# saifahmadgit/go2-sim2real-locomotion-rl

Measured on AMD Instinct MI355X. Metric: env-steps/sec (all envs) Go2 walk 4096 envs; 1/2/4/8-GPU scaling, higher is better.
Workload: dtype f32

## Files before the change

go2_sim2real_locomotion_rl_amd/csrc/go2sim.hip:

```cpp

#include <hip/hip_runtime.h>

#include <cstdint>
#include <cstdio>
#include <cstdlib>
#include <cstring>
#include <new>
#include <vector>

#include "../../include/go2sim.h"
#include "../../include/go2sim_detmath.h"

#define DEV __device__ __forceinline__
#define DEVN __device__ __noinline__

namespace {

constexpr int NL = GO2SIM_NL, ND = GO2SIM_ND, NQ = GO2SIM_NQ, NG = GO2SIM_NG, NJ = GO2SIM_NJ;
constexpr int NPAIR = GO2SIM_NPAIR_MAX, MAXC = GO2SIM_MAX_CONTACTS, MAXB = GO2SIM_MAX_BROAD, MAXR = GO2SIM_MAX_ROWS;
constexpr int JOINT_FIXED = 0, JOINT_REVOLUTE = 1, JOINT_FREE = 4;
constexpr int GEOM_PLANE = 0, GEOM_SPHERE = 1, GEOM_CYLINDER = 3, GEOM_BOX = 5, GEOM_TERRAIN = 7;
constexpr int TERRAIN_CB = 4;
constexpr int MAX_CONTACTS_PER_PAIR = 5;
constexpr int CTRL_FORCE = 0, CTRL_VELOCITY = 1, CTRL_POSITION = 2;
// ... 1381 lines not shown
  }
  if (legs) {
    const int r = m.leg_root;
    if (tl < 6 * LEG_K) {
      const int l = tl / 6, c = tl % 6;
      const float* src = (c < 3) ? s->cdofd_vel : s->cdofd_ang;
      const int cc = (c < 3) ? c : c - 3;
      const V3 g0 = -m.gravity * (1.0f - 0.0f);
      const int ds = m.links[r].dof_start;
      float vr[6], xr[6], vl[LEG_D], xl[LEG_D]; int lk[LEG_D];
#pragma unroll
      for (int i = 0; i < 6; ++i) { vr[i] = s->vel[ds + i]; xr[i] = src[3 * (ds + i) + cc]; }
#pragma unroll
      for (int d = 0; d < LEG_D; ++d) {
        lk[d] = m.leg_links[LEG_D * l + d];
        const int i_d = m.links[lk[d]].dof_start;
        vl[d] = s->vel[i_d]; xl[d] = src[3 * i_d + cc];
      }
      float* dst = (c < 3) ? s->cdd_vel : s->cdd_ang;
      float a = (c < 3) ? ((cc == 0) ? g0.x : ((cc == 1) ? g0.y : g0.z)) : 0.0f;
#pragma unroll
      for (int i = 0; i < 6; ++i) a = a + xr[i] * vr[i];
      if (l == 0) dst[3 * r + cc] = a;
#pragma unroll
      for (int d = 0; d < LEG_D; ++d) { a = a + xl[d] * vl[d]; dst[3 * lk[d] + cc] = a; }
    }
    for (int i_l = tl; i_l < NL; i_l += T) {
      if (m.links[i_l].parent != -1 || i_l == r) continue;
      st3(s->cdd_vel, i_l, -m.gravity * (1.0f - 0.0f)); st3(s->cdd_ang, i_l, v3(0, 0, 0));
    }
    team_sync();
  }
  for (int lev = 0; lev < (legs ? 0 : m.n_levels); ++lev) {
    for (int k = m.level_start[lev] + tl; k < m.level_start[lev + 1]; k += T) {
      int i_l = m.level_links[k];
      const auto& L = m.links[i_l];
      V3 cv, ca;
      if (L.parent == -1) { cv = -m.gravity * (1.0f - 0.0f); ca = v3(0, 0, 0); }
      else { cv = ld3(s->cdd_vel, L.parent); ca = ld3(s->cdd_ang, L.parent); }
      for (int i_d = L.dof_start; i_d < L.dof_end; ++i_d) {
        float v = s->vel[i_d];
        V3 local_cdd_vel = ld3(s->cdofd_vel, i_d) * v;
        V3 local_cdd_ang = ld3(s->cdofd_ang, i_d) * v;
        cv = cv + local_cdd_vel;
        ca = ca + local_cdd_ang;
      }
      st3(s->cdd_vel, i_l, cv); st3(s->cdd_ang, i_l, ca);
    }
    team_sync();
  }
  for (int i_l = tl; i_l < NL; i_l += T) {
    V3 f1_ang, f1_vel, f2_ang, f2_vel, f3_ang, f3_vel;
    M3 I = ld9(s->cinr_I, i_l); V3 cp = ld3(s->cinr_pos, i_l); float cm = s->cinr_mass[i_l];
    V3 cdv = ld3(s->cd_vel, i_l), cda = ld3(s->cd_ang, i_l);
    inertial_mul(cp, I, cm, ld3(s->cdd_vel, i_l), ld3(s->cdd_ang, i_l), f1_ang, f1_vel);
    inertial_mul(cp, I, cm, cdv, cda, f2_ang, f2_vel);
    motion_cross_force(cda, cdv, f2_ang, f2_vel, f3_ang, f3_vel);
    V3 ext_ang = ld3(s->cfrc_ang, i_l), ext_vel = ld3(s->cfrc_vel, i_l);
    st3(s->cfrc_vel, i_l, f1_vel + f3_vel + ext_vel + v3(0, 0, 0));
    st3(s->cfrc_ang, i_l, f1_ang + f3_ang + ext_ang + v3(0, 0, 0));
  }
  team_sync();
  if (legs) {
    for (int c = tl; c < 6; c += T) {
      auto at = [&](int i_l) -> float* { return (c < 3) ? &s->cfrc_vel[3 * i_l + c] : &s->cfrc_ang[3 * i_l + c - 3]; };
      const int r = m.leg_root;
      float x[LEG_K][LEG_D];
#pragma unroll
      for (int l = 0; l < LEG_K; ++l)
#pragma unroll
        for (int d = 0; d < LEG_D; ++d) x[l][d] = *at(m.leg_links[LEG_D * l + d]);
      float a = *at(r);
#pragma unroll
      for (int l = 0; l < LEG_K; ++l) {
#pragma unroll
        for (int d = LEG_D - 2; d >= 0; --d) { x[l][d] = x[l][d] + x[l][d + 1]; *at(m.leg_links[LEG_D * l + d]) = x[l][d]; }
      }
#pragma unroll
      for (int l = 0; l < LEG_K; ++l) a = a + x[l][0];
      *at(r) = a;
    }
    team_sync();
  }
  for (int lev = (legs ? -1 : m.n_levels - 2); lev >= 0; --lev) {
    int n_par = m.level_start[lev + 1] - m.level_start[lev];
    for (int w = tl; w < n_par * 6; w += T) {
      int i_p = m.level_links[m.level_start[lev] + w / 6], comp = w % 6;
      float* dst = (comp < 3) ? &s->cfrc_vel[3 * i_p + comp] : &s->cfrc_ang[3 * i_p + comp - 3];
      float a = *dst;
      for (int c = m.child_start[i_p]; c < m.child_start[i_p + 1]; ++c) {
        int i_l = m.child_list[c];
        a = a + ((comp < 3) ? s->cfrc_vel[3 * i_l + comp] : s->cfrc_ang[3 * i_l + comp - 3]);
      }
      *dst = a;
    }
    team_sync();
  }
  for (int i_d = tl; i_d < ND; i_d += T) {
    int i_l = m.dof_link[i_d];
    float qf_bias = dot(ld3(s->cdof_ang, i_d), ld3(s->cfrc_ang, i_l)) + dot(ld3(s->cdof_vel, i_d), ld3(s->cfrc_vel, i_l));
    float f = s->qf_passive[i_d] - qf_bias + s->qf_applied[i_d];
    s->force[i_d] = f;
    if (env_valid) { astore(e, AO(force), i_d, f); astore(e, AO(qf_smooth), i_d, f); }
  }
  team_sync();
  PH(24)
  bool solved = false;
#if GO2SIM_FAST_ORDER
  if constexpr (T == 32 || T == 64) {
    if (arrow) {
      const int leg = (tl >> 3) & 3, u = tl & 7, ub = u < 6 ? u : 5;
      const int p0 = dm_arrow_dof(m.arrow_mode, leg, 0), p1 = dm_arrow_dof(m.arrow_mode, leg, 1), p2 = dm_arrow_dof(m.arrow_mode, leg, 2);
      float xb[6], x0, x1, x2;
      arrow_solve<T>(AF, s->force[p0], s->force[p1], s->force[p2], s->force[ub], s->Dinv, tl, xb, x0, x1, x2);
      if (tl == 0) {
#pragma unroll
        for (int k = 0; k < 6; ++k) s->out[k] = xb[k];
      }
      if (tl < 32 && u == 0) { s->out[p0] = x0; s->out[p1] = x1; s->out[p2] = x2; }
      solved = true;
    }
  }
#endif
  if (!solved) {
    float y[ND];
#pragma unroll
    for (int i_d_ = 0; i_d_ < ND; ++i_d_) {
      const int i_d = ND - i_d_ - 1;
      float cur = s->force[i_d];
#pragma unroll
      for (int j_d = i_d + 1; j_d < ND; ++j_d) cur = cur - s->L[j_d * ND + i_d] * y[j_d];
      y[i_d] = cur;
    }
#pragma unroll
    for (int i_d = 0; i_d < ND; ++i_d) y[i_d] = y[i_d] * s->Dinv[i_d];
#pragma unroll
    for (int i_d = 0; i_d < ND; ++i_d) {
      float cur = y[i_d];
#pragma unroll
      for (int j_d = 0; j_d < i_d; ++j_d) cur = cur - s->L[i_d * ND + j_d] * y[j_d];
      y[i_d] = cur;
    }
    if (tl == 0) {
#pragma unroll
      for (int i_d = 0; i_d < ND; ++i_d) s->out[i_d] = y[i_d];
    }
  }
  team_sync();
  if (env_valid) for (int i_d = tl; i_d < ND; i_d += T) { float a = s->out[i_d]; astore(e, AO(acc_smooth), i_d, a); astore(e, AO(acc), i_d, a); }
  if (env_valid) for (int idx = tl; idx < NTRI; idx += T) { int i, j; tri_index(m, idx, i, j); astore(e, AO(mass_mat), idx, s->M[i * ND + j]); }
  PH(25)
}

template <int T>
__global__ __launch_bounds__(64) void k_dynamics_team(Pool P, const ModelS* __restrict__ mp) {
  constexpr int EPW = 64 / T;
  __shared__ DynData lds[EPW];
  __shared__ alignas(16) char ms_raw[MODELS_LDS_BYTES];
  const ModelS& ms = *(const ModelS*)ms_raw;
  wg_dma_to_lds<(int)sizeof(ModelS)>(ms_raw, mp);
  {
    const int b0 = xcd_block() * EPW;
    wg_load<EPW, NL * 3>(P, b0, FO(cd_vel), [&](int ev, int k, float v) { lds[ev].cd_vel[k] = v; });
    wg_load<EPW, NL * 3>(P, b0, FO(cd_ang), [&](int ev, int k, float v) { lds[ev].cd_ang[k] = v; });
    wg_load<EPW, ND>(P, b0, FO(vel), [&](int ev, int k, float v) { lds[ev].vel[k] = v; });
  }
  const int tl = threadIdx.x % T, slot = threadIdx.x / T;
  const int b = xcd_block() * EPW + slot;
  const bool env_valid = b < P.B;
  const ModelView m(&ms, mp);
  E e(P, env_valid ? b : P.B - 1);
  DynData* s = &lds[slot];
  PH_BEGIN
  team_stage<NL * 9, T>(tl, [&](int k) { return aload(e, AO(cinr_inertial), k); }, [&](int k, float v) { s->cinr_I[k] = v; s->crb_I[k] = v; });
  team_stage<NL * 3, T>(tl, [&](int k) { return aload(e, AO(cinr_pos), k); }, [&](int k, float v) { s->cinr_pos[k] = v; s->crb_pos[k] = v; });
  team_stage<NL, T>(tl, [&](int k) { return aload(e, AO(cinr_mass), k); }, [&](int k, float v) { s->cinr_mass[k] = v; s->crb_mass[k] = v; });
  team_stage<ND, T>(tl, [&](int d) { return __int_as_float((int)e.ctrl_mode()[d]); }, [&](int d, float v) { s->ctrl_mode[d] = __float_as_int(v); });
  team_stage<ND * 3, T>(tl, [&](int k) { return aload(e, AO(cdof_ang), k); }, [&](int k, float v) { s->cdof_ang[k] = v; });
  team_stage<ND * 3, T>(tl, [&](int k) { return aload(e, AO(cdof_vel), k); }, [&](int k, float v) { s->cdof_vel[k] = v; });
  team_stage<ND * 3, T>(tl, [&](int k) { return aload(e, AO(cdofd_ang), k); }, [&](int k, float v) { s->cdofd_ang[k] = v; });
  team_stage<ND * 3, T>(tl, [&](int k) { return aload(e, AO(cdofd_vel), k); }, [&](int k, float v) { s->cdofd_vel[k] = v; });
  team_stage<ND, T>(tl, [&](int d) { return gload(e, FO(ctrl_force), d); }, [&](int d, float v) { s->qf_applied[d] = v; });
  team_stage<ND, T>(tl, [&](int d) { return gload(e, FO(ctrl_pos), d); }, [&](int d, float v) { s->qf_passive[d] = v; });
  team_stage<ND, T>(tl, [&](int d) { return gload(e, FO(ctrl_vel), d); }, [&](int d, float v) { s->force[d] = v; });
  team_stage<ND, T>(tl, [&](int d) { return gload(e, FO(dof_pos), d); }, [&](int d, float v) { s->out[d] = v; });
  team_stage<NL * 6, T>(tl, [&](int k) { return gload(e, FO(ext), k); },
                        [&](int k, float v) { int i_l = k / 6, c = k % 6; if (c < 3) s->cfrc_ang[3 * i_l + c] = v; else s->cfrc_vel[3 * i_l + c - 3] = v; });
  team_sync();
  PH(20)
  tk_dynamics<T>(m, e, s, tl, env_valid);
}


template <bool OVERLAY, int EPW> struct KinSeparate { KinData k[EPW]; DEV KinData* at(int slot, void*) { return &k[slot]; } };
template <int EPW> struct KinSeparate<true, EPW> { DEV KinData* at(int, void* overlay) { return (KinData*)overlay; } };
constexpr bool KIN_OVERLAY = sizeof(KinData) <= 2 * sizeof(float) * ND * ND;
template <int T>
DEV void integrate_fk_dynamics_body(const Pool& P, const ModelS* __restrict__ mp, int b, DynData* lds_d, char* ms_raw, KinSeparate<KIN_OVERLAY, 64 / T>& lds_k,
                                    bool pre, float pre_vel, float pre_acc) {
  const ModelS& ms = *(const ModelS*)ms_raw;
  wg_dma_to_lds<(int)sizeof(ModelS)>(ms_raw, mp);
  const int tl = threadIdx.x % T, slot = threadIdx.x / T;
  const ModelView m(&ms, mp);
  E e(P, b < P.B ? b : P.B - 1);
  DynData* d = &lds_d[slot];
  static_assert(offsetof(DynData, L) == offsetof(DynData, M) + sizeof(float) * ND * ND, "KinData overlay");
  KinData* s = lds_k.at(slot, d->M);
  PH_BEGIN
  if (pre) { if (tl < ND) { s->vel[tl] = pre_vel; s->vel_next[tl] = pre_acc; } }
  else {
    team_stage<ND, T>(tl, [&](int i) { return gload(e, FO(vel), i); }, [&](int i, float v) { s->vel[i] = v; });
    team_stage<ND, T>(tl, [&](int i) { return aload(e, AO(acc), i); }, [&](int i, float a) { s->vel_next[i] = a; });
  }
  team_stage<NQ, T>(tl, [&](int q) { return gload(e, FO(qpos), q); }, [&](int q, float v) { s->qpos[q] = v; });
  team_stage<ND, T>(tl, [&](int i) { return __int_as_float((int)e.ctrl_mode()[i]); }, [&](int i, float v) { d->ctrl_mode[i] = __float_as_int(v); });
  team_stage<ND, T>(tl, [&](int i) { return gload(e, FO(ctrl_force), i); }, [&](int i, float v) { d->qf_applied[i] = v; });
  team_stage<ND, T>(tl, [&](int i) { return gload(e, FO(ctrl_pos), i); }, [&](int i, float v) { d->qf_passive[i] = v; });
  team_stage<ND, T>(tl, [&](int i) { return gload(e, FO(ctrl_vel), i); }, [&](int i, float v) { d->force[i] = v; });
  team_stage<NL * 6, T>(tl, [&](int k) { return gload(e, FO(ext), k); },
                        [&](int k, float v) { int i_l = k / 6, c = k % 6; if (c < 3) d->cfrc_ang[3 * i_l + c] = v; else d->cfrc_vel[3 * i_l + c - 3] = v; });
  team_for<ND, T>(tl, [&](int i) { s->vel_next[i] = s->vel[i] + s->vel_next[i] * m.substep_dt; });
  if (tl == 0) s->valid = 1;
  tk_stage_links<T>(e, s, tl);
  team_sync();
  if (b >= P.B) return;
  tk_integrate<T>(m, e, s, tl);
  PH(40)
  tk_kinematics<T>(m, e, s, tl, false, d);
  team_for<ND, T>(tl, [&](int i) { d->vel[i] = s->vel[i]; });
  team_sync();
  PH(41)
  tk_dynamics<T>(m, e, d, tl, true);
}
template <int T>
__global__ __launch_bounds__(64) void k_integrate_fk_dynamics_team(Pool P, const ModelS* __restrict__ mp) {
  STAMP(STK_INT_FK_DYN)
  constexpr int EPW = 64 / T;
  __shared__ DynData lds_d[EPW];
  __shared__ alignas(16) char ms_raw[MODELS_LDS_BYTES];
  __shared__ KinSeparate<KIN_OVERLAY, EPW> lds_k;
  integrate_fk_dynamics_body<T>(P, mp, xcd_block() * EPW + (int)threadIdx.x / T, lds_d, ms_raw, lds_k, false, 0.0f, 0.0f);
}

DEV int wrap180(float x) {
  if (!(x >= 0.0f)) return 0;
  int i = (x >= 180.0f) ? (int)(x - 180.0f) : (int)x;
  return (i > 179) ? 179 : i;
}
DEV int clampidx(float x) {
  if (!(x >= 0.0f)) return 0;
  return (x >= 179.0f) ? 179 : (int)x;
}
DEV V3 support_cylinder_local(const Model& m, const Geom& G, V3 d_mesh, int* vid_out = nullptr) {
  const float PI = 3.14159265358979323846f;
  float theta = dm_atan2(d_mesh.y, d_mesh.x);
  float phi = dm_acos(d_mesh.z);
  const float support_res = 180.0f;
  float ii = (theta + PI) / PI / 2.0f * support_res;
  float jj = phi / PI * support_res;
  const int i_lo = wrap180(dm_floor(ii)), i_hi = wrap180(dm_ceil(ii));
  int j_lo = clampidx(dm_floor(jj)); if (j_lo == 0) j_lo = 1;
  int j_hi = clampidx(dm_ceil(jj)); if (j_hi == 179) j_hi = 178;
  const int k_lo = m.theta_to_ring[i_lo], k_hi = m.theta_to_ring[i_hi];
  const float rx_lo = G.rim[k_lo][0], ry_lo = G.rim[k_lo][1], rx_hi = G.rim[k_hi][0], ry_hi = G.rim[k_hi][1];
  const float half = 0.5f * G.data[1];
  float dot_max = -1e20f;
  V3 v = v3(0, 0, 0);
  int vid = 0;
#pragma unroll
  for (int i4 = 0; i4 < 4; ++i4) {
    const bool hi_i = (i4 % 2) != 0, hi_j = (i4 / 2) > 0;
    const int j = hi_j ? j_hi : j_lo, k = hi_i ? k_hi : k_lo;
    V3 pos = v3(hi_i ? rx_hi : rx_lo, hi_i ? ry_hi : ry_lo, (j <= 90) ? half : -half);
    float d = dot(pos, d_mesh);
    if (d > dot_max) { v = pos; dot_max = d; vid = k + ((j <= 90) ? 0 : 32); }
  }
  if (vid_out) *vid_out = vid;
  return v;
}
template <int T> DEV unsigned long long team_ballot(bool p) {
  const unsigned long long b = __ballot(p);
  if constexpr (T == 64) return b;
  else return (b >> (threadIdx.x & (64 - T))) & ((1ull << T) - 1ull);
}
DEV V3 vsel(bool c, V3 a, V3 b) { return v3(c ? a.x : b.x, c ? a.y : b.y, c ? a.z : b.z); }
DEV V3 support_prism(const V3* prism, V3 d) {
  const bool bottom = d.z < 0;
  const V3 p0 = vsel(bottom, prism[0], prism[3]), p1 = vsel(bottom, prism[1], prism[4]), p2 = vsel(bottom, prism[2], prism[5]);
  float best = dot(p0, d);
  V3 v = p0;
  const float dt1 = dot(p1, d);
  const bool b1 = dt1 > best;
  v = vsel(b1, p1, v); best = b1 ? dt1 : best;
  const float dt2 = dot(p2, d);
  v = vsel(dt2 > best, p2, v);
  return v;
}
struct GeomLite { int type; float d0, d1, d2; };
DEV GeomLite geom_lite(const Model& m, int i_g) { const Geom& G = m.geoms[i_g]; GeomLite r = {G.type, G.data[0], G.data[1], G.data[2]}; return r; }
DEV V3 support_driver(const Model& m, V3 direction, int i_g, const GeomLite& gl, V3 pos, const Rot& rot, const V3* prism = nullptr) {
  if (gl.type == GEOM_TERRAIN) return support_prism(prism, direction);
  if (gl.type == GEOM_SPHERE) {
    return pos + direction * gl.d0;
  } else if (gl.type == GEOM_BOX) {
    V3 d_box = rot_apply_inv(rot, direction);
    V3 v_ = v3((d_box.x < 0.0f ? -1.0f : 1.0f) * gl.d0 * 0.5f, (d_box.y < 0.0f ? -1.0f : 1.0f) * gl.d1 * 0.5f,
               (d_box.z < 0.0f ? -1.0f : 1.0f) * gl.d2 * 0.5f);
    return rot_apply(rot, v_) + pos;
  } else if (gl.type == GEOM_CYLINDER) {
    V3 d_mesh = rot_apply_inv(rot, direction);
    V3 v_ = support_cylinder_local(m, m.geoms[i_g], d_mesh);
    return rot_apply(rot, v_) + pos;
  }
  return pos;
}
struct Pair { int i_ga, i_gb; V3 pos_a; Q4 quat_a; V3 pos_b; Q4 quat_b; const V3* prism; GeomLite ga, gb; Rot ra, rb; };
DEV void pair_set_rots(Pair& pr) { pr.ra = make_rot(pr.quat_a); pr.rb = make_rot(pr.quat_b); }
DEV void compute_support(const Model& m, V3 direction, const Pair& pr, V3& v, V3& v1, V3& v2) {
  v1 = support_driver(m, direction, pr.i_ga, pr.ga, pr.pos_a, pr.ra);
  v2 = support_driver(m, -direction, pr.i_gb, pr.gb, pr.pos_b, pr.rb, pr.prism);
  v = v1 - v2;
}


DEV V3 gjk_support_driver(const Model& m, V3 direction, int i_g, const GeomLite& gl, V3 pos, const Rot& rot, int& vid) {
  if (gl.type == GEOM_SPHERE) {
    vid = -1;
    return pos + direction * gl.d0;
  } else if (gl.type == GEOM_BOX) {
    V3 d_box = rot_apply_inv(rot, direction);
    V3 v_ = v3((d_box.x < 0.0f ? -1.0f : 1.0f) * gl.d0 * 0.5f, (d_box.y < 0.0f ? -1.0f : 1.0f) * gl.d1 * 0.5f,
               (d_box.z < 0.0f ? -1.0f : 1.0f) * gl.d2 * 0.5f);
    vid = (v_.x > 0.0f) * 1 + (v_.y > 0.0f) * 2 + (v_.z > 0.0f) * 4 + 64 * i_g;
    return rot_apply(rot, v_) + pos;
  } else if (gl.type == GEOM_CYLINDER) {
    V3 d_mesh = rot_apply_inv(rot, direction);
    int k = 0;
    V3 v_ = support_cylinder_local(m, m.geoms[i_g], d_mesh, &k);
    vid = k + 64 * i_g;
    return rot_apply(rot, v_) + pos;
  }
  vid = -1;
  return pos;
}
#include "go2sim_gjk_dev.h"

DEVN DgResult gjk_query_global(const DgPair& dp, GjkStoreFull* full, float eps) { return dg_contact(dp, *full, eps); }
DEV DgResult gjk_query(const DgPair& dp, GjkStoreLds* slots, unsigned* slot_mask, GjkStoreFull* full, float eps) {
  int slot = -1;
  if (slots) {
    for (int i = 0; i < GJK_SLOTS_MAX && slot < 0; ++i) {
      const unsigned bit = 1u << i;
      if (!(atomicOr(slot_mask, bit) & bit)) slot = i;
    }
  }
  DgResult r; r.is_col = false; r.overflow = true; r.penetration = 0.0f; r.normal = v3(0, 0, 0); r.pos = v3(0, 0, 0);
  if (slot >= 0) {
    r = dg_contact(dp, slots[slot], eps);
    atomicAnd(slot_mask, ~(1u << slot));
  }
  if (r.overflow) r = gjk_query_global(dp, full, eps);
  return r;
}

struct Simplex { V3 v[4], v1[4], v2[4]; };
DEV V3 mpr_portal_dir(const Simplex& s) { return normalized(cross(s.v[2] - s.v[1], s.v[3] - s.v[1])); }
DEV bool mpr_portal_reach_tolerance(const Model& m, const Simplex& s, V3 v, V3 direction) {
  float dv1 = dot(s.v[1], direction), dv2 = dot(s.v[2], direction), dv3 = dot(s.v[3], direction), dv4 = dot(v, direction);
  float dot1 = fmn(fmn(dv4 - dv1, dv4 - dv2), dv4 - dv3);
  return dot1 < m.ccd_tolerance + m.ccd_eps * fmx(1.0f, dot1);
}
DEV void simplex_set(Simplex& s, int i, V3 v, V3 v1, V3 v2) {
  const bool c1 = i == 1, c2 = i == 2, c3 = !(c1 || c2);
  s.v[1] = vsel(c1, v, s.v[1]); s.v1[1] = vsel(c1, v1, s.v1[1]); s.v2[1] = vsel(c1, v2, s.v2[1]);
  s.v[2] = vsel(c2, v, s.v[2]); s.v1[2] = vsel(c2, v1, s.v1[2]); s.v2[2] = vsel(c2, v2, s.v2[2]);
  s.v[3] = vsel(c3, v, s.v[3]); s.v1[3] = vsel(c3, v1, s.v1[3]); s.v2[3] = vsel(c3, v2, s.v2[3]);
}
DEV void mpr_expand_portal(Simplex& s, V3 v, V3 v1, V3 v2) {
  V3 v4v0 = cross(v, s.v[0]);
  float d = dot(s.v[1], v4v0);
  int i_s;
  if (d > 0) { d = dot(s.v[2], v4v0); i_s = (d > 0) ? 1 : 3; }
  else { d = dot(s.v[3], v4v0); i_s = (d > 0) ? 2 : 1; }
  simplex_set(s, i_s, v, v1, v2);
}
DEV bool mpr_first_support_separates(const Model& m, const Pair& pr, V3 center_a, V3 center_b) {
  const float EPSC = m.ccd_eps;
  V3 v0 = center_a - center_b;
  if (dm_abs(v0.x) < EPSC && dm_abs(v0.y) < EPSC && dm_abs(v0.z) < EPSC) v0.x += 10.0f * EPSC;
  const V3 direction = -normalized(v0);
  V3 v, v1, v2;
  compute_support(m, direction, pr, v, v1, v2);
  return dot(v, direction) < EPSC;
}
DEV int mpr_discover_portal(const Model& m, Simplex& s, const Pair& pr, V3 center_a, V3 center_b) {
  const float EPSC = m.ccd_eps;
  s.v1[0] = center_a; s.v2[0] = center_b; s.v[0] = center_a - center_b;
  int simplex_size = 1;
  if (dm_abs(s.v[0].x) < EPSC && dm_abs(s.v[0].y) < EPSC && dm_abs(s.v[0].z) < EPSC) s.v[0].x += 10.0f * EPSC;
  V3 direction = -normalized(s.v[0]);
  V3 v, v1, v2;
  compute_support(m, direction, pr, v, v1, v2);
  s.v1[1] = v1; s.v2[1] = v2; s.v[1] = v;
  simplex_size = 2;
  float d = dot(v, direction);
  int ret = 0;
  if (d < EPSC) {
    ret = -1;
  } else {
    direction = cross(s.v[0], s.v[1]);
    if (dot(direction, direction) < EPSC) {
      if (dm_abs(s.v[1].x) < EPSC && dm_abs(s.v[1].y) < EPSC && dm_abs(s.v[1].z) < EPSC) ret = 1; else ret = 2;
    } else {
      direction = normalized(direction);
      compute_support(m, direction, pr, v, v1, v2);
      d = dot(v, direction);
      if (d < EPSC) {
        ret = -1;
      } else {
        s.v1[2] = v1; s.v2[2] = v2; s.v[2] = v;
        simplex_size = 3;
        V3 va = s.v[1] - s.v[0], vb = s.v[2] - s.v[0];
        direction = normalized(cross(va, vb));
        d = dot(direction, s.v[0]);
        if (d > 0) {
          V3 t;
          t = s.v[1]; s.v[1] = s.v[2]; s.v[2] = t; t = s.v1[1]; s.v1[1] = s.v1[2]; s.v1[2] = t; t = s.v2[1]; s.v2[1] = s.v2[2]; s.v2[2] = t;
          direction = -direction;
        }
        int num_trials = 0;
        while (simplex_size < 4) {
          compute_support(m, direction, pr, v, v1, v2);
          d = dot(v, direction);
          if (d < EPSC) { ret = -1; break; }
          bool cont = false;
          va = cross(s.v[1], v);
// ... 4 lines not shown
            d = dot(va, s.v[0]);
            if (d < -EPSC) { s.v1[1] = v1; s.v2[1] = v2; s.v[1] = v; cont = true; }
          }
          if (cont) {
            va = s.v[1] - s.v[0]; vb = s.v[2] - s.v[0];
            direction = normalized(cross(va, vb));
            num_trials++;
            if (num_trials == 15) { ret = -1; break; }
          } else {
            s.v1[3] = v1; s.v2[3] = v2; s.v[3] = v;
            simplex_size = 4;
          }
        }
      }
    }
  }
  return ret;
}
DEV int mpr_refine_portal(const Model& m, Simplex& s, const Pair& pr) {
  int ret = 1;
  while (true) {
    V3 direction = mpr_portal_dir(s);
    if (dot(s.v[1], direction) > -m.ccd_eps) { ret = 0; break; }
    V3 v, v1, v2;
    compute_support(m, direction, pr, v, v1, v2);
    if (!(dot(v, direction) > -m.ccd_eps) || mpr_portal_reach_tolerance(m, s, v, direction)) { ret = -1; break; }
    mpr_expand_portal(s, v, v1, v2);
  }
  return ret;
}
DEV V3 mpr_find_pos(const Model& m, const Simplex& s) {
  float b0 = 0.0f, b1 = 0.0f, b2 = 0.0f, b3 = 0.0f;
  float sum_ = ((b0 + b1) + b2) + b3;
  if (sum_ < m.ccd_eps) {
    V3 direction = mpr_portal_dir(s);
    b0 = 0.0f;
    b1 = dot(cross(s.v[2], s.v[3]), direction);
    b2 = dot(cross(s.v[3], s.v[1]), direction);
    b3 = dot(cross(s.v[1], s.v[2]), direction);
    sum_ = ((b0 + b1) + b2) + b3;
  }
  V3 p1 = v3(0, 0, 0), p2 = v3(0, 0, 0);
  p1 = p1 + b0 * s.v1[0]; p2 = p2 + b0 * s.v2[0];
  p1 = p1 + b1 * s.v1[1]; p2 = p2 + b1 * s.v2[1];
  p1 = p1 + b2 * s.v1[2]; p2 = p2 + b2 * s.v2[2];
  p1 = p1 + b3 * s.v1[3]; p2 = p2 + b3 * s.v2[3];
  return (0.5f / sum_) * (p1 + p2);
}
DEV void mpr_find_penetration(const Model& m, Simplex& s, const Pair& pr, bool& is_col, V3& normal, float& penetration, V3& pos) {
  int iterations = 0;
  while (true) {
    V3 direction = mpr_portal_dir(s);
    V3 v, v1, v2;
    compute_support(m, direction, pr, v, v1, v2);
    if (mpr_portal_reach_tolerance(m, s, v, direction) || iterations > m.ccd_iterations) {
      penetration = dot(direction, s.v[1]);
      normal = -direction;
      is_col = true;
      pos = mpr_find_pos(m, s);
      break;
    }
    mpr_expand_portal(s, v, v1, v2);
    iterations++;
  }
}
DEV void guess_geoms_center(const Model& m, const Pair& pr, V3 normal_ws, V3& center_a, V3& center_b) {
  const Geom& A = m.geoms[pr.i_ga]; const Geom& Bg = m.geoms[pr.i_gb];
  center_a = transform_by_trans_quat(A.center, pr.pos_a, pr.quat_a);
  center_b = transform_by_trans_quat(Bg.center, pr.pos_b, pr.quat_b);
  if (dm_abs(normal_ws.x) > m.ccd_eps || dm_abs(normal_ws.y) > m.ccd_eps || dm_abs(normal_ws.z) > m.ccd_eps) {
    V3 center_a_local = 0.5f * (A.aabb[7] + A.aabb[0]);
    center_a = transform_by_trans_quat(center_a_local, pr.pos_a, pr.quat_a);
    V3 center_b_local = 0.5f * (Bg.aabb[7] + Bg.aabb[0]);
    center_b = transform_by_trans_quat(center_b_local, pr.pos_b, pr.quat_b);
    V3 delta = center_a - center_b;
    V3 normal = normalized(delta);
    if (norm(cross(normal_ws, normal)) > 0.01f) {
      V3 offset = dot(delta, normal_ws) * normal_ws - delta;
      float offset_norm = norm(offset);
      if (offset_norm > m.eps) {
        V3 dir_offset = offset / offset_norm;
        V3 dla = inv_transform_by_quat(dir_offset, pr.quat_a), dlb = inv_transform_by_quat(dir_offset, pr.quat_b);
        V3 box_size_a = A.aabb[7] - A.aabb[0], box_size_b = Bg.aabb[7] - Bg.aabb[0];
        float length_a = dot(box_size_a, v3(dm_abs(dla.x), dm_abs(dla.y), dm_abs(dla.z)));
        float length_b = dot(box_size_b, v3(dm_abs(dlb.x), dm_abs(dlb.y), dm_abs(dlb.z)));
        float offset_ratio = fmn(offset_norm / (length_a + length_b), 0.5f);
        center_a = center_a + dir_offset * length_a * offset_ratio;
        center_b = center_b - dir_offset * length_b * offset_ratio;
      }
    }
  }
}
DEV void mpr_contact_from_centers(const Model& m, const Pair& pr, V3 center_a, V3 center_b, bool& is_col, V3& normal, float& penetration, V3& pos) {
  Simplex s;
  int res = mpr_discover_portal(m, s, pr, center_a, center_b);
  is_col = false; pos = v3(0, 0, 0); normal = v3(0, 0, 0); penetration = 0.0f;
  if (res == 1) {
    is_col = true; penetration = 0.0f; normal = -normalized(s.v[0]); pos = (s.v1[1] + s.v2[1]) * 0.5f;
  } else if (res == 2) {
    is_col = true; penetration = norm(s.v[1]); normal = -normalized(s.v[1]); pos = (s.v1[1] + s.v2[1]) * 0.5f;
  } else if (res == 0) {
    res = mpr_refine_portal(m, s, pr);
    if (res >= 0) mpr_find_penetration(m, s, pr, is_col, normal, penetration, pos);
  }
}
DEV void mpr_contact(const Model& m, const Pair& pr, V3 normal_ws, bool& is_col, V3& normal, float& penetration, V3& pos) {
  V3 center_a, center_b;
  guess_geoms_center(m, pr, normal_ws, center_a, center_b);
  mpr_contact_from_centers(m, pr, center_a, center_b, is_col, normal, penetration, pos);
}

DEV float compute_tolerance(const Model& m, int i_ga, int i_gb, float tolerance) {
  float size_b = norm(m.geoms[i_gb].aabb[7] - m.geoms[i_gb].aabb[0]);
  if (m.geoms[i_ga].type == GEOM_PLANE) return 0.5f * tolerance * size_b;
  float size_a = norm(m.geoms[i_ga].aabb[7] - m.geoms[i_ga].aabb[0]);
  return 0.5f * tolerance * fmn(size_a, size_b);
}
DEV void contact_orthogonals(const Model& m, const E& e, int i_ga, int i_gb, V3 normal, V3& axis_0, V3& axis_1) {
  V3 size_ga = m.geoms[i_ga].aabb[7], size_gb = m.geoms[i_gb].aabb[7];
  float volume_ga = size_ga.x * size_ga.y * size_ga.z, volume_gb = size_gb.x * size_gb.y * size_gb.z;
  int i_g = (volume_ga < volume_gb && m.geoms[i_ga].type != GEOM_PLANE) ? i_ga : i_gb;
  int i_l = m.geoms[i_g].link;
  M3 rot = quat_to_R(e.i_quat()[i_l], m.eps);
  int axis_idx = 0; float axis_angle_max = 0.0f;
#pragma unroll
  for (int i = 0; i < 3; ++i) {
    float axis_angle = dm_abs(dot(mcol(rot, i), normal));
    if (axis_angle > axis_angle_max) { axis_angle_max = axis_angle; axis_idx = i; }
  }
  axis_idx = (axis_idx + 1) % 3;
  axis_0 = mcol(rot, axis_idx);
  axis_0 = normalized(axis_0 - dot(normal, axis_0) * normal);
  axis_1 = cross(normal, axis_0);
}
DEV void rotate_frame(V3 pos, Q4 quat, V3 contact_pos, Q4 qrot, V3& new_pos, Q4& new_quat) {
  new_quat = transform_quat_by_quat(quat, qrot);
  V3 rel = contact_pos - pos;
  V3 vec = transform_by_quat(rel, qrot);
  vec = vec - rel;
  new_pos = pos - vec;
}

DEV void plane_contact(const Model& m, const Pair& pr, bool& is_col, V3& normal, float& penetration, V3& pos) {
  const V3 plane_dir = transform_by_quat(v3(pr.ga.d0, pr.ga.d1, pr.ga.d2), pr.quat_a);
  normal = -normalized(plane_dir);
  const V3 v1 = support_driver(m, normal, pr.i_gb, pr.gb, pr.pos_b, pr.rb);
  penetration = dot(normal, v1 - pr.pos_a);
  pos = v1 - 0.5f * penetration * normal;
  is_col = penetration > 0.0f;
}
constexpr int GJK_SLOTS = GJK_SLOTS_MAX;
template <int T>
struct CollideData {
  struct Broad {
    alignas(16) float amin[NG * 4], amax[NG * 4];
    float sval[2 * NG], sval_sorted[2 * NG];
    alignas(16) unsigned long long skey[2 * NG];
    int sig[2 * NG], sig_sorted[2 * NG];
    alignas(8) int rank_mm[NG * 2];
    int cand_key[MAXB], cand_pair[MAXB];
  };
  struct TPair { int i_ga, r_min, r_max, c_min, c_max, n_items, item_off; float zmin, tol; V3 pos_a; Q4 quat_a; V3 center_a; };
  struct Terrain {
    TPair tp[NG];
  };
  union alignas(16) {
    Broad bp;
    GjkStoreLds gjk[GJK_SLOTS];
    Terrain tr;
  };
  unsigned short pair_sorted[MAXB];
  float stage[T][5][7];
  int cnt[T];
  unsigned gjk_slot_mask;
  float gjk_res[T][8];
  unsigned ncv[NCV];
};
struct ContactStage { float* st; int n; };

DEV void stage_contact(ContactStage& cs, V3 normal, V3 pos, float pen) {
  float* p = cs.st + 7 * cs.n;
  p[0] = normal.x; p[1] = normal.y; p[2] = normal.z; p[3] = pos.x; p[4] = pos.y; p[5] = pos.z; p[6] = pen;
  cs.n++;
}

DEV void plane_box_contact_staged(const Model& m, const E& e, int i_ga, int i_gb, ContactStage& cs) {
  const V3 ga_pos = e.g_pos()[i_ga], gb_pos = e.g_pos()[i_gb];
  const Q4 ga_quat = e.g_quat()[i_ga], gb_quat = e.g_quat()[i_gb];
  const Geom& A = m.geoms[i_ga]; const Geom& Bg = m.geoms[i_gb];
  const V3 normal = -normalized(transform_by_quat(v3(A.data[0], A.data[1], A.data[2]), ga_quat));
  const V3 d_box = inv_transform_by_quat(normal, gb_quat);
  const V3 v_ = v3((d_box.x < 0.0f ? -1.0f : 1.0f) * Bg.data[0] * 0.5f, (d_box.y < 0.0f ? -1.0f : 1.0f) * Bg.data[1] * 0.5f,
                   (d_box.z < 0.0f ? -1.0f : 1.0f) * Bg.data[2] * 0.5f);
  const V3 v1 = transform_by_trans_quat(v_, gb_pos, gb_quat);
  const float pen0 = dot(normal, v1 - ga_pos);
  if (!(pen0 > 0.0f)) return;
  const V3 contact_pos_0 = v1 - 0.5f * pen0 * normal;
  stage_contact(cs, normal, contact_pos_0, pen0);
  const float tolerance = compute_tolerance(m, i_ga, i_gb, m.mc_tolerance);
  const int n_max = imn(m.n_contacts_per_pair, 5);
  for (int c = 0; c < 8; ++c) {
    if (cs.n >= n_max) break;
    const V3 corner = transform_by_trans_quat(Bg.aabb[c], gb_pos, gb_quat);
    const float pen = dot(normal, corner - ga_pos);
    if (pen > 0.0f) {
      const V3 cpos = corner - 0.5f * pen * normal;
      if (norm(cpos - contact_pos_0) > tolerance) stage_contact(cs, normal, cpos, pen);
    }
  }
}

struct CcState {
  Pair pr; V3 ga_pos_o, gb_pos_o; Q4 ga_quat_o, gb_quat_o;
  int i_pair, type_a, type_b; bool multi_contact, want_gjk; float tolerance;
  bool is_col; float penetration; V3 normal, contact_pos;
};
DEV void cc_mpr_with_retry(const Model& m, CcState& c, int i_detection, unsigned* ncv, const Arr3& normal_cache, bool& guess_available) {
  const float EPS = m.eps;
  bool is_mpr_updated = false;
  V3 normal_ws = ((ncv[c.i_pair >> 5] >> (c.i_pair & 31)) & 1u) ? (V3)normal_cache[c.i_pair] : v3(0, 0, 0);
  guess_available = (dm_abs(normal_ws.x) > EPS) || (dm_abs(normal_ws.y) > EPS) || (dm_abs(normal_ws.z) > EPS);
  for (int i_mpr = 0; i_mpr < 2; ++i_mpr) {
    if (i_mpr == 1) {
      if ((i_detection == 0) && !c.is_col && guess_available) { normal_ws = v3(0, 0, 0); guess_available = false; is_mpr_updated = false; }
    }
    if (!is_mpr_updated) {
      PHD_BEGIN
      mpr_contact(m, c.pr, normal_ws, c.is_col, c.normal, c.penetration, c.contact_pos);
      PHD(36)
      is_mpr_updated = true;
    }
  }
}
DEV bool cc_prefer_gjk(const Model& m, const CcState& c, bool guess_available) {
  if (c.penetration > c.tolerance) return !guess_available || (m.mc_tolerance * c.penetration >= m.mpr_to_gjk_ratio * c.tolerance);
  return false;
}
DEV void cc_detect0(const Model& m, const E& e, int i_ga, int i_gb, unsigned* ncv, CcState& c) {
  c.type_a = m.geoms[i_ga].type; c.type_b = m.geoms[i_gb].type;
  c.multi_contact = (c.type_a != GEOM_SPHERE) && (c.type_b != GEOM_SPHERE);
  c.tolerance = compute_tolerance(m, i_ga, i_gb, m.mc_tolerance);
  c.ga_pos_o = e.g_pos()[i_ga]; c.gb_pos_o = e.g_pos()[i_gb]; c.ga_quat_o = e.g_quat()[i_ga]; c.gb_quat_o = e.g_quat()[i_gb];
  Pair& pr = c.pr;
  pr.i_ga = i_ga; pr.i_gb = i_gb; pr.pos_a = c.ga_pos_o; pr.quat_a = c.ga_quat_o; pr.pos_b = c.gb_pos_o; pr.quat_b = c.gb_quat_o; pr.prism = nullptr; pr.ga = geom_lite(m, i_ga); pr.gb = geom_lite(m, i_gb);
  pair_set_rots(pr);
  c.is_col = false; c.penetration = 0.0f; c.normal = v3(0, 0, 0); c.contact_pos = v3(0, 0, 0);
  c.i_pair = (i_ga > i_gb) ? m.pair_idx[i_gb][i_ga] : m.pair_idx[i_ga][i_gb];
  if (c.type_a == GEOM_PLANE) {
    plane_contact(m, pr, c.is_col, c.normal, c.penetration, c.contact_pos);
    c.want_gjk = false;
    return;
  }
  bool guess_available;
  cc_mpr_with_retry(m, c, 0, ncv, e.normal_cache(), guess_available);
  c.want_gjk = cc_prefer_gjk(m, c, guess_available);
}
DEV void cc_gjk_lane(const Model& m, const E& e, CcState& c, GjkStoreLds* gjk_slots, unsigned* gjk_slot_mask, GjkStoreFull* gjk_full) {
  atomicAdd(&e.gjk_fallback()[0], 1);
  const Pair& pr = c.pr;
  DgPair dp;
  dp.m = &m; dp.i_ga = pr.i_ga; dp.i_gb = pr.i_gb; dp.pos_a = pr.pos_a; dp.quat_a = pr.quat_a; dp.pos_b = pr.pos_b; dp.quat_b = pr.quat_b;
  dp.ga = pr.ga; dp.gb = pr.gb; dp.ra = pr.ra; dp.rb = pr.rb;
  dp.discrete = c.type_a == GEOM_BOX && c.type_b == GEOM_BOX;
  PHD_BEGIN
  const DgResult gr = gjk_query(dp, gjk_slots, gjk_slot_mask, gjk_full, m.eps);
  PHD(34)
  c.is_col = gr.is_col;
  c.penetration = gr.penetration;
  if (c.is_col) { c.contact_pos = gr.pos; c.normal = gr.normal; }
}
DEV void cc_rest(const Model& m, const E& e, CcState& c, ContactStage& cs, GjkStoreLds* gjk_slots, unsigned* gjk_slot_mask, GjkStoreFull* gjk_full, unsigned* ncv) {
  const float EPS = m.eps;
  const int i_ga = c.pr.i_ga, i_gb = c.pr.i_gb, i_pair = c.i_pair;
  const bool multi_contact = c.multi_contact;
  const float tolerance = c.tolerance;
  Pair& pr = c.pr;
  bool is_col_0 = false; V3 normal_0 = v3(0, 0, 0), contact_pos_0 = v3(0, 0, 0);
  bool& is_col = c.is_col; float& penetration = c.penetration; V3& normal = c.normal; V3& contact_pos = c.contact_pos;
  V3 axis_0 = v3(0, 0, 0), axis_1 = v3(0, 0, 0); Q4 qrot = q4(0, 0, 0, 0);
  auto normal_cache = e.normal_cache();
  PHD_BEGIN
  for (int i_detection = 0; i_detection < 5; ++i_detection) {
    if (i_detection == 1) { PHD(44) }
    if (i_detection > 0 && multi_contact && is_col_0) {
      V3 axis = (float)(2 * (i_detection % 2) - 1) * axis_0 + (float)(1 - 2 * ((i_detection / 2) % 2)) * axis_1;
      qrot = rotvec_to_quat(m.mc_perturbation * axis, EPS);
      rotate_frame(c.ga_pos_o, c.ga_quat_o, contact_pos_0, qrot, pr.pos_a, pr.quat_a);
      rotate_frame(c.gb_pos_o, c.gb_quat_o, contact_pos_0, inv_quat(qrot), pr.pos_b, pr.quat_b);
      pair_set_rots(pr);
      if (c.type_a == GEOM_PLANE) {
        plane_contact(m, pr, is_col, normal, penetration, contact_pos);
      } else {
        bool guess_available;
        cc_mpr_with_retry(m, c, i_detection, ncv, normal_cache, guess_available);
        if (cc_prefer_gjk(m, c, guess_available)) cc_gjk_lane(m, e, c, gjk_slots, gjk_slot_mask, gjk_full);
      }
    }
    if (i_detection == 0) {
      is_col_0 = is_col; normal_0 = normal; contact_pos_0 = contact_pos;
      if (is_col_0) {
        stage_contact(cs, normal, contact_pos, penetration);
        if (multi_contact) contact_orthogonals(m, e, i_ga, i_gb, normal, axis_0, axis_1);
        normal_cache[i_pair] = normal; atomicOr(&ncv[i_pair >> 5], 1u << (i_pair & 31));
      } else {
        atomicAnd(&ncv[i_pair >> 5], ~(1u << (i_pair & 31)));
      }
    } else if (multi_contact && is_col) {
      V3 contact_point_a = transform_by_quat((contact_pos - 0.5f * penetration * normal) - contact_pos_0, inv_quat(qrot)) + contact_pos_0;
      V3 contact_point_b = transform_by_quat((contact_pos + 0.5f * penetration * normal) - contact_pos_0, qrot) + contact_pos_0;
      contact_pos = 0.5f * (contact_point_a + contact_point_b);
      V3 tw = cross(normal, normal_0);
      V3 twist_rotvec = v3(clampf(tw.x, -m.mc_perturbation, m.mc_perturbation), clampf(tw.y, -m.mc_perturbation, m.mc_perturbation),
                           clampf(tw.z, -m.mc_perturbation, m.mc_perturbation));
      normal = normal + cross(twist_rotvec, normal);
      penetration = dot(normal, contact_point_b - contact_point_a);
      bool repeated = false;
      for (int i_c = 0; i_c < cs.n; ++i_c)
        if (!repeated) {
          const float* prev = cs.st + 7 * (cs.n - 1 - i_c);
          if (norm(contact_pos - v3(prev[3], prev[4], prev[5])) < tolerance) repeated = true;
        }
      if (!repeated && penetration > -tolerance) {
        penetration = fmx(penetration, 0.0f);
        stage_contact(cs, normal, contact_pos, penetration);
      }
    }
  }
  PHD(46)
}
DEV void convex_convex_contact_staged(const Model& m, const E& e, int i_ga, int i_gb, ContactStage& cs, GjkStoreLds* gjk_slots, unsigned* gjk_slot_mask, GjkStoreFull* gjk_full, unsigned* ncv) {
  CcState c;
  cc_detect0(m, e, i_ga, i_gb, ncv, c);
  if (c.want_gjk) cc_gjk_lane(m, e, c, gjk_slots, gjk_slot_mask, gjk_full);
  cc_rest(m, e, c, cs, gjk_slots, gjk_slot_mask, gjk_full, ncv);
}

DEV bool terrain_pair_out_of_reach(const Model& m, const GeomLite& gl, V3 pos) {
  float R;
  if (gl.type == GEOM_SPHERE) R = gl.d0;
  else if (gl.type == GEOM_BOX) R = 0.5f * dm_sqrt(gl.d0 * gl.d0 + gl.d1 * gl.d1 + gl.d2 * gl.d2);
  else if (gl.type == GEOM_CYLINDER) R = dm_sqrt(gl.d0 * gl.d0 + 0.25f * (gl.d1 * gl.d1));
  else return false;
  R = R * 1.001f + 1e-3f;
  const float* tmm = m.terrain_xyz_maxmin;
  const float sh = m.terrain_hs;
  int r_lo = (int)dm_floor((pos.x - R - tmm[3]) / sh) - 1, r_hi = (int)dm_ceil((pos.x + R - tmm[3]) / sh) + 1;
  int c_lo = (int)dm_floor((pos.y - R - tmm[4]) / sh) - 1, c_hi = (int)dm_ceil((pos.y + R - tmm[4]) / sh) + 1;
  r_lo = imx(0, r_lo); c_lo = imx(0, c_lo); r_hi = imn(m.terrain_rows - 1, r_hi); c_hi = imn(m.terrain_cols - 1, c_hi);
  if (!(r_lo <= r_hi && c_lo <= c_hi)) return false;
  const int I0 = r_lo / TERRAIN_CB, J0 = c_lo / TERRAIN_CB;
  if (r_hi / TERRAIN_CB > I0 + 2 || c_hi / TERRAIN_CB > J0 + 2) return false;
  float mx = -1e30f;
#pragma unroll
  for (int a = 0; a < 3; ++a)
#pragma unroll
    for (int q = 0; q < 3; ++q) mx = fmx(mx, m.terrain_cmax[(size_t)imn(I0 + a, m.terrain_crows - 1) * m.terrain_ccols + imn(J0 + q, m.terrain_ccols - 1)]);
  return mx < pos.z - R;
}
template <class TP>
DEV bool terrain_pair_setup(const Model& m, const E& e, int i_ga, int i_gb, TP& t) {
  V3 ga_pos = e.g_pos()[i_ga], gb_pos = e.g_pos()[i_gb]; Q4 ga_quat = e.g_quat()[i_ga], gb_quat = e.g_quat()[i_gb];
  const float margin = 0.0f;
  transform_pos_quat_by_trans_quat(ga_pos - gb_pos, ga_quat, v3(0, 0, 0), inv_quat(gb_quat), t.pos_a, t.quat_a);
  t.center_a = transform_by_trans_quat(m.geoms[i_ga].center, t.pos_a, t.quat_a);
  t.i_ga = i_ga;
  GeomLite gl = geom_lite(m, i_ga);
  const Rot t_rot = make_rot(t.quat_a);
  float xyz_max_min[6];
#pragma unroll
  for (int i_axis = 0; i_axis < 3; ++i_axis)
#pragma unroll
    for (int i_m = 0; i_m < 2; ++i_m) {
      V3 direction = v3(0, 0, 0);
      vset(direction, i_axis, (i_m == 0) ? 1.0f : -1.0f);
      V3 v1 = support_driver(m, direction, i_ga, gl, t.pos_a, t_rot);
      xyz_max_min[3 * i_m + i_axis] = vget(v1, i_axis);
    }
  const float* tmm = m.terrain_xyz_maxmin;
  bool is_return = false;
#pragma unroll
  for (int i = 0; i < 3; ++i)
    if (tmm[i] < xyz_max_min[i + 3] - margin || tmm[i + 3] > xyz_max_min[i] + margin) is_return = true;
  const float sh = m.terrain_hs;
  int r_min = (int)dm_floor((xyz_max_min[3] - tmm[3]) / sh);
  int r_max = (int)dm_ceil((xyz_max_min[0] - tmm[3]) / sh);
  int c_min = (int)dm_floor((xyz_max_min[4] - tmm[4]) / sh);
  int c_max = (int)dm_ceil((xyz_max_min[1] - tmm[4]) / sh);
  t.r_min = imx(0, r_min); t.c_min = imx(0, c_min);
  t.r_max = imn(m.terrain_rows - 1, r_max); t.c_max = imn(m.terrain_cols - 1, c_max);
  t.zmin = xyz_max_min[5];
  if (is_return) { t.r_max = t.r_min; }
  return !is_return;
}
DEV float terrain_strip_z(const Model& m, int r, int c_min, int k) { return m.terrain_hf[(size_t)(r + (k & 1)) * m.terrain_cols + c_min + (k >> 1)]; }
static_assert(NG - 1 <= 32, "five bits of pair slot: at most 32 geoms besides the heightfield");
inline bool terrain_cells_fit(const Model& m, float hs) {
  for (int i = 0; i < NG; ++i) {
    const double dx = m.geoms[i].aabb[7].x - m.geoms[i].aabb[0].x, dy = m.geoms[i].aabb[7].y - m.geoms[i].aabb[0].y, dz = m.geoms[i].aabb[7].z - m.geoms[i].aabb[0].z;
    const double n = std::sqrt(dx * dx + dy * dy + dz * dz) / (double)hs + 2.0;
    if (i > 0 && 2.0 * n * n >= (double)(1 << 26)) return false;
  }
  return true;
}
DEV int terrain_desc(int p, int local) { return p | (local << 5); }
template <class TP>
DEV void terrain_desc_cell(const TP& t, int local, int& r, int& k) {
  const int nkk = 2 * (t.c_max - t.c_min + 1) - 2;
  r = t.r_min + local / nkk; k = 2 + local % nkk;
}
template <class TP>
DEV void terrain_prism_pair(const Model& m, const TP& t, int i_gb, int r, int k, V3 (&prism)[6], Pair& pr, V3& center_b) {
  const float* tmm = m.terrain_xyz_maxmin;
  const float sh = m.terrain_hs;
#pragma unroll
  for (int j = 0; j < 3; ++j) {
    int kk = k - 2 + j;
    float x = sh * (float)(r + (kk & 1)) + tmm[3], y = sh * (float)(t.c_min + (kk >> 1)) + tmm[4];
    prism[j] = v3(x, y, tmm[5]);
    prism[3 + j] = v3(x, y, terrain_strip_z(m, r, t.c_min, kk) + 0.0f);
  }
  pr.i_ga = t.i_ga; pr.i_gb = i_gb; pr.prism = prism; pr.pos_a = t.pos_a; pr.quat_a = t.quat_a; pr.pos_b = v3(0, 0, 0); pr.quat_b = qident();
  pr.ga = geom_lite(m, t.i_ga); pr.gb = geom_lite(m, i_gb);
  pair_set_rots(pr);
  center_b = v3(0, 0, 0);
  for (int i_p = 0; i_p < 6; ++i_p) center_b = center_b + prism[i_p];
  center_b = center_b / 6.0f;
}
template <class TP>
DEV bool terrain_prism_separated_at_once(const Model& m, const TP& t, int i_gb, int r, int k) {
  V3 prism[6]; Pair pr; V3 center_b;
  terrain_prism_pair(m, t, i_gb, r, k, prism, pr, center_b);
  return mpr_first_support_separates(m, pr, t.center_a, center_b);
}
template <class TP>
DEV bool terrain_prism_contact(const Model& m, const E& e, const TP& t, int i_gb, int r, int k, V3& normal, V3& contact_pos, float& penetration) {
  V3 prism[6]; Pair pr; V3 center_b;
  terrain_prism_pair(m, t, i_gb, r, k, prism, pr, center_b);
  bool is_col;
  mpr_contact_from_centers(m, pr, t.center_a, center_b, is_col, normal, penetration, contact_pos);
  if (is_col) {
    V3 gb_pos = e.g_pos()[i_gb]; Q4 gb_quat = e.g_quat()[i_gb];
    normal = transform_by_quat(normal, gb_quat);
    contact_pos = transform_by_quat(contact_pos, gb_quat);
    contact_pos = contact_pos + gb_pos;
  }
  return is_col;
}

template <int T>
__global__ __launch_bounds__(64) void k_collide_team(Pool P, const Model* __restrict__ mp, GjkStoreFull* __restrict__ gjk_scratch, int* __restrict__ lpt_rec, int lpt_cap, int solver_epw) {
  STAMP(STK_COLLIDE)
  constexpr int EPW = 64 / T;
  __shared__ CollideData<T> lds[EPW];
  const int tl = threadIdx.x % T, slot = threadIdx.x / T;
  const int b = xcd_block() * EPW + slot;
  if (slot >= EPW || b >= P.B) return;
  const Model& m = *mp;
  E e(P, b);
  CollideData<T>* s = &lds[slot];
  const float inf = dm_bits2f(0x7f800000u);
  if (tl == 0) s->gjk_slot_mask = 0u;
  for (int i = tl; i < NCV; i += T) s->ncv[i] = (unsigned)e.ncache_valid()[i];
  PH_BEGIN
  const int nc_old = e.n_contacts()[0];
  const bool first = e.first_time()[0] != 0;
  const int n2 = 2 * NG;
  team_stage<2 * NG, T>(tl, [&](int i) { return __int_as_float(e.sort_ig()[i]); }, [&](int i, float v) { s->bp.sig[i] = __float_as_int(v); });
  constexpr int NPI = (NPAIR + T - 1) / T;
  int packed_[NPI];
  {
    const int n_pairs = m.n_pairs;
#pragma unroll
    for (int it = 0; it < NPI; ++it) { int pidx = it * T + tl; int v = m.pair_list[pidx < NPAIR ? pidx : NPAIR - 1]; packed_[it] = (pidx < n_pairs) ? v : -1; }
  }
#pragma unroll
  for (int g0 = 0; g0 < NG; g0 += T) {
    const int i_g = (g0 + tl < NG) ? g0 + tl : NG - 1;
    V3 lower = v3(inf, inf, inf), upper = v3(-inf, -inf, -inf);
    V3 gp = e.g_pos()[i_g]; Q4 gq = e.g_quat()[i_g];
#pragma unroll
    for (int c = 0; c < 8; ++c) {
      V3 corner = transform_by_trans_quat(m.geoms[i_g].aabb[c], gp, gq);
      lower = vmin(lower, corner); upper = vmax(upper, corner);
    }
    *(float4*)&s->bp.amin[4 * i_g] = make_float4(lower.x, lower.y, lower.z, 0.0f);
    *(float4*)&s->bp.amax[4 * i_g] = make_float4(upper.x, upper.y, upper.z, 0.0f);
  }
  for (int i_c = tl; i_c < nc_old; i_c += T) {
    e.c_link()[i_c] = -1; e.c_link()[MAXC + i_c] = -1; e.c_geom()[i_c] = -1; e.c_geom()[MAXC + i_c] = -1;
    e.c_pen()[i_c] = 0.0f; e.c_pos()[i_c] = v3(0, 0, 0); e.c_normal()[i_c] = v3(0, 0, 0); e.c_force()[i_c] = v3(0, 0, 0);
  }
  team_sync();
  PH(30)
  for (int i = tl; i < n2; i += T) {
    int sg = first ? ((i >> 1) | ((i & 1) ? 0x100 : 0)) : s->bp.sig[i];
    int g = sg & 0xff;
    s->bp.sig[i] = sg;
    const float v = (sg & 0x100) ? s->bp.amax[4 * g] : s->bp.amin[4 * g];
    s->bp.sval[i] = v;
    unsigned u = (unsigned)__float_as_int(v + 0.0f);
    u = (u & 0x80000000u) ? ~u : (u | 0x80000000u);
    s->bp.skey[i] = ((unsigned long long)u << 8) | (unsigned long long)i;
  }
  team_sync();
  {
    constexpr int NK = (2 * NG + T - 1) / T;
    unsigned long long key[NK]; int r[NK];
#pragma unroll
    for (int q = 0; q < NK; ++q) { const int i = tl + q * T; key[q] = s->bp.skey[i < n2 ? i : n2 - 1]; r[q] = 0; }
#pragma unroll
    for (int j = 0; j < 2 * NG; ++j) {
      const unsigned long long kj = s->bp.skey[j];
#pragma unroll
      for (int q = 0; q < NK; ++q) r[q] += (kj < key[q]) ? 1 : 0;
    }
#pragma unroll
    for (int q = 0; q < NK; ++q) {
      const int i = tl + q * T;
      if (i < n2) {
        const float v = s->bp.sval[i];
        const int sg = s->bp.sig[i];
        s->bp.sval_sorted[r[q]] = v; s->bp.sig_sorted[r[q]] = sg;
        s->bp.rank_mm[2 * (sg & 0xff) + ((sg & 0x100) ? 1 : 0)] = r[q];
        e.sort_value()[r[q]] = v; e.sort_ig()[r[q]] = sg;
      }
    }
  }
  if (tl == 0 && first) e.first_time()[0] = 0;
  team_sync();
  PH(31)
  int n_cand = 0;
  unsigned cmask = 0; int key_[NPI];
  unsigned ncv_clear = 0u;
  static_assert(NCV <= T, "one lane per word of the normal-cache mask");
#pragma unroll
  for (int it = 0; it < NPI; ++it) {
    const int pidx = it * T + tl;
    const int packed = packed_[it];
    const int a = (packed < 0) ? 0 : (packed & 0xff), bg = (packed < 0) ? 0 : (packed >> 8);
    const int2 rka = *(const int2*)&s->bp.rank_mm[2 * a], rkb = *(const int2*)&s->bp.rank_mm[2 * bg];
    const float4 amn = *(const float4*)&s->bp.amin[4 * a], amx = *(const float4*)&s->bp.amax[4 * a], bmn = *(const float4*)&s->bp.amin[4 * bg], bmx = *(const float4*)&s->bp.amax[4 * bg];
    const int ra = rka.x, rb = rkb.x;
    const int rs = (ra < rb) ? rb : ra, rf = (ra < rb) ? ra : rb;
    const int rmax_first = (ra < rb) ? rka.y : rkb.y;
    key_[it] = rs * 64 + rf;
    const bool swept = packed >= 0 && rs < rmax_first;
    const bool any1 = (amx.x <= bmn.x) || (amx.y <= bmn.y) || (amx.z <= bmn.z);
    const bool any2 = (amn.x >= bmx.x) || (amn.y >= bmx.y) || (amn.z >= bmx.z);
    if (swept && !(any1 || any2)) cmask |= 1u << it;
    const unsigned long long sep = team_ballot<T>(swept && (any1 || any2));
    (void)pidx;
    if constexpr (T < 32) { if (tl == ((it * T) >> 5)) ncv_clear |= (unsigned)(sep << ((it * T) & 31)); }
    else if constexpr (T == 32) { if (tl == it) ncv_clear |= (unsigned)sep; }
    else { if (tl == 2 * it) ncv_clear |= (unsigned)sep; if (tl == 2 * it + 1) ncv_clear |= (unsigned)(sep >> 32); }
  }
  if (tl < NCV) s->ncv[tl] &= ~ncv_clear;
  {
    const int mine = __popc(cmask);
    s->cnt[tl] = mine;
    team_sync();
    int pos = 0, tot = 0;
    for (int l = 0; l < T; ++l) { int c = s->cnt[l]; pos += (l < tl) ? c : 0; tot += c; }
    team_sync();
#pragma unroll
    for (int it = 0; it < NPI; ++it)
      if (cmask & (1u << it)) { if (pos < MAXB) { s->bp.cand_key[pos] = key_[it]; s->bp.cand_pair[pos] = packed_[it]; } pos++; }
    n_cand = tot;
  }
  if (n_cand > m.max_broad_pairs && tl == 0) atomicOr(&e.err()[0], GO2SIM_ERR_OVERFLOW_CANDIDATE_CONTACTS);
  n_cand = imn(n_cand, MAXB);
  team_sync();
  for (int c = tl; c < n_cand; c += T) {
    int key = s->bp.cand_key[c], r = 0;
    for (int j = 0; j < n_cand; ++j) r += s->bp.cand_key[j] < key;
    s->pair_sorted[r] = (unsigned short)s->bp.cand_pair[c];
  }
  const int n_broad = imn(n_cand, m.max_broad_pairs);
  team_sync();
  for (int c = tl; c < n_broad; c += T) { int pk = s->pair_sorted[c]; e.broad()[2 * c] = pk & 0xff; e.broad()[2 * c + 1] = pk >> 8; }
  PH(32)
  int nc_run = 0;
  const int n_np_iter = (n_broad + T - 1) / T;
  auto append_staged = [&](const ContactStage& cs, int i_ga, int i_gb) {
    s->cnt[tl] = cs.n;
    team_sync();
    int off = 0, tot = 0;
    for (int l = 0; l < T; ++l) { int c = s->cnt[l]; off += (l < tl) ? c : 0; tot += c; }
    for (int k = 0; k < cs.n; ++k) {
      int i_c = nc_run + off + k;
      if (i_c < m.max_contact_pairs) {
        const float* p = cs.st + 7 * k;
        float friction_a = e.geom_friction()[i_ga] * e.friction_ratio()[i_ga];
        float friction_b = e.geom_friction()[i_gb] * e.friction_ratio()[i_gb];
        e.c_geom()[i_c] = i_ga; e.c_geom()[MAXC + i_c] = i_gb;
        e.c_normal()[i_c] = v3(p[0], p[1], p[2]); e.c_pos()[i_c] = v3(p[3], p[4], p[5]); e.c_pen()[i_c] = p[6];
        e.c_friction()[i_c] = fmx(fmx(friction_a, friction_b), 1e-2f);
        auto sol = e.c_sol()[i_c];
        for (int q = 0; q < 7; ++q) sol[q] = 0.5f * (m.geoms[i_ga].sol_params[q] + m.geoms[i_gb].sol_params[q]);
        e.c_link()[i_c] = m.geoms[i_ga].link; e.c_link()[MAXC + i_c] = m.geoms[i_gb].link;
      } else {
        atomicOr(&e.err()[0], GO2SIM_ERR_OVERFLOW_COLLISION_PAIRS);
      }
    }
    nc_run += tot;
    team_sync();
  };
  bool any_plane_box = false;
  for (int it = 0; it < n_np_iter; ++it) {
    int ip = it * T + tl;
    ContactStage cs; cs.st = &s->stage[tl][0][0]; cs.n = 0;
    int i_ga = 0, i_gb = 0;
    bool convex_pair = false, plane_box = false;
    if (ip < n_broad) {
      int pk = s->pair_sorted[ip];
      i_ga = pk & 0xff; i_gb = pk >> 8;
      if (m.geoms[i_ga].type > m.geoms[i_gb].type) { int t = i_ga; i_ga = i_gb; i_gb = t; }
      plane_box = m.geoms[i_ga].type == GEOM_PLANE && m.geoms[i_gb].type == GEOM_BOX;
      convex_pair = m.geoms[i_gb].type != GEOM_TERRAIN && !plane_box;
    }
    any_plane_box |= team_ballot<T>(plane_box) != 0ull;
    if constexpr (T == 16) {
      static_assert(GJK_SLOTS >= 4, "one LDS polytope slot per quad");
      CcState cst;
      cst.want_gjk = false;
      if (convex_pair) cc_detect0(m, e, i_ga, i_gb, s->ncv, cst);
      const bool wants = convex_pair && cst.want_gjk;
      const unsigned want = dgc_ballot<16>(wants);
      const int n_want = __popc(want), quad = tl >> 2, ql = tl & 3;
      for (int r0 = 0; r0 < n_want; r0 += 4) {
        unsigned rest = want;
        for (int k = 0; k < r0 + quad; ++k) rest &= rest - 1u;
        const int L = rest ? __ffs((int)rest) - 1 : -1;
        const int Ls = L < 0 ? tl : L;
        DgPair dp;
        dp.m = mp; dp.i_ga = __shfl(i_ga, Ls, 16); dp.i_gb = __shfl(i_gb, Ls, 16);
        dp.pos_a = v3(__shfl(cst.pr.pos_a.x, Ls, 16), __shfl(cst.pr.pos_a.y, Ls, 16), __shfl(cst.pr.pos_a.z, Ls, 16));
        dp.quat_a = q4(__shfl(cst.pr.quat_a.w, Ls, 16), __shfl(cst.pr.quat_a.x, Ls, 16), __shfl(cst.pr.quat_a.y, Ls, 16), __shfl(cst.pr.quat_a.z, Ls, 16));
        dp.pos_b = v3(__shfl(cst.pr.pos_b.x, Ls, 16), __shfl(cst.pr.pos_b.y, Ls, 16), __shfl(cst.pr.pos_b.z, Ls, 16));
        dp.quat_b = q4(__shfl(cst.pr.quat_b.w, Ls, 16), __shfl(cst.pr.quat_b.x, Ls, 16), __shfl(cst.pr.quat_b.y, Ls, 16), __shfl(cst.pr.quat_b.z, Ls, 16));
        if (L >= 0) {
          dp.ga = geom_lite(m, dp.i_ga); dp.gb = geom_lite(m, dp.i_gb); dp.ra = make_rot(dp.quat_a); dp.rb = make_rot(dp.quat_b);
          dp.discrete = dp.ga.type == GEOM_BOX && dp.gb.type == GEOM_BOX;
          PHD_BEGIN
          DgResult gr = dgc_contact<4>(dp, s->gjk[quad], m.eps, ql);
          if (gr.overflow) gr = dgc_contact<4>(dp, gjk_scratch[(size_t)b * T + L], m.eps, ql);
          PHD(34)
          if (ql == 0) {
            float* o = s->gjk_res[L];
            o[0] = gr.is_col ? 1.0f : 0.0f; o[1] = gr.penetration; o[2] = gr.normal.x; o[3] = gr.normal.y; o[4] = gr.normal.z; o[5] = gr.pos.x; o[6] = gr.pos.y; o[7] = gr.pos.z;
          }
        }
      }
      team_sync();
      if (wants) {
        atomicAdd(&e.gjk_fallback()[0], 1);
        const float* o = s->gjk_res[tl];
        cst.is_col = o[0] != 0.0f;
        cst.penetration = o[1];
        if (cst.is_col) { cst.normal = v3(o[2], o[3], o[4]); cst.contact_pos = v3(o[5], o[6], o[7]); }
      }
      if (convex_pair) cc_rest(m, e, cst, cs, nullptr, &s->gjk_slot_mask, &gjk_scratch[(size_t)b * T + tl], s->ncv);
    } else if (convex_pair) convex_convex_contact_staged(m, e, i_ga, i_gb, cs, s->gjk, &s->gjk_slot_mask, &gjk_scratch[(size_t)b * T + tl], s->ncv);
    append_staged(cs, i_ga, i_gb);
  }
  if (any_plane_box) {
    for (int it = 0; it < n_np_iter; ++it) {
      int ip = it * T + tl;
      ContactStage cs; cs.st = &s->stage[tl][0][0]; cs.n = 0;
      int i_ga = 0, i_gb = 0;
      if (ip < n_broad) {
        int pk = s->pair_sorted[ip];
        i_ga = pk & 0xff; i_gb = pk >> 8;
        if (m.geoms[i_ga].type > m.geoms[i_gb].type) { int t = i_ga; i_ga = i_gb; i_gb = t; }
        if (m.geoms[i_ga].type == GEOM_PLANE && m.geoms[i_gb].type == GEOM_BOX) plane_box_contact_staged(m, e, i_ga, i_gb, cs);
      }
      append_staged(cs, i_ga, i_gb);
    }
  }
  if (m.terrain_enabled) {
    PH(33)
    int n_list = 0, i_terrain = 0;
    for (int ip = 0; ip < n_broad; ++ip) {
      int pk = s->pair_sorted[ip];
      int i_ga = pk & 0xff, i_gb = pk >> 8;
      if (m.geoms[i_ga].type == GEOM_TERRAIN) { int t = i_ga; i_ga = i_gb; i_gb = t; }
      if (m.geoms[i_gb].type != GEOM_TERRAIN) continue;
      if (n_list < NG) { if (tl == 0) s->tr.tp[n_list].i_ga = i_ga; i_terrain = i_gb; n_list++; }
    }
    team_sync();
    int n_tp = 0;
    for (int base = 0; base < n_list; base += T) {
      const int p = base + tl;
      int i_ga = 0; bool keep = false;
      if (p < n_list) {
        i_ga = s->tr.tp[p].i_ga;
        V3 pos_t; Q4 quat_t;
        transform_pos_quat_by_trans_quat((V3)e.g_pos()[i_ga] - (V3)e.g_pos()[i_terrain], e.g_quat()[i_ga], v3(0, 0, 0), inv_quat(e.g_quat()[i_terrain]), pos_t, quat_t);
        keep = m.terrain_cmax == nullptr || !terrain_pair_out_of_reach(m, geom_lite(m, i_ga), pos_t);
      }
      const unsigned long long mk = team_ballot<T>(keep);
      team_sync();
      if (keep) s->tr.tp[n_tp + __popcll(mk & ((1ull << tl) - 1ull))].i_ga = i_ga;
      n_tp += __popcll(mk);
      team_sync();
    }
    for (int p = tl; p < n_tp; p += T) {
      auto& t = s->tr.tp[p];
      terrain_pair_setup(m, e, t.i_ga, i_terrain, t);
      t.n_items = imx(0, t.r_max - t.r_min) * imx(0, 2 * (t.c_max - t.c_min + 1) - 2);
      t.tol = compute_tolerance(m, t.i_ga, i_terrain, m.mc_tolerance);
    }
    team_sync();
    PH(26)
    int* items = (int*)&gjk_scratch[(size_t)b * T];
    constexpr int TU = 4;
    const int items_cap = (int)(sizeof(GjkStoreFull) * T / sizeof(int));
    static_assert(sizeof(GjkStoreFull) / sizeof(int) >= TU, "a chunk of descriptors holds a batch of cells");
    static_assert(sizeof(GjkStoreFull) * 16 / sizeof(int) <= 100000, "test_terrain_gpu.py::test_descriptors_beyond_one_chunk sizes its field for > 1 chunk");
    int n_cells = 0;
    for (int p = 0; p < n_tp; ++p) n_cells += s->tr.tp[p].n_items;
    team_sync();
    { int off = 0; for (int p = 0; p < n_tp; ++p) { int c = s->tr.tp[p].n_items; if (tl == 0) s->tr.tp[p].item_off = off; off += c; } }
    team_sync();
    int cur_p = -1, n_con = 0;
    float tolerance = 0.0f;
    V3 acc[5];
#pragma unroll
    for (int j = 0; j < 5; ++j) acc[j] = v3(0, 0, 0);
    int p_cur = 0, p_end = n_tp > 0 ? s->tr.tp[0].n_items : 0;
    for (int cell_base = 0; cell_base < n_cells;) {
      int n_items = 0;
      for (; cell_base < n_cells && n_items <= items_cap - T * TU; cell_base += T * TU) {
        int desc[TU]; bool el[TU];
#pragma unroll
        for (int u = 0; u < TU; ++u) {
          const int ci = cell_base + u * T + tl;
          el[u] = false; desc[u] = 0;
          if (ci < n_cells) {
            while (ci >= p_end) { ++p_cur; p_end += s->tr.tp[p_cur].n_items; }
            const auto& t = s->tr.tp[p_cur];
            const int local = ci - (p_end - t.n_items);
            int r, k;
            terrain_desc_cell(t, local, r, k);
            const float z0 = terrain_strip_z(m, r, t.c_min, k - 2), z1 = terrain_strip_z(m, r, t.c_min, k - 1), z2 = terrain_strip_z(m, r, t.c_min, k);
            el[u] = (z0 >= t.zmin) | (z1 >= t.zmin) | (z2 >= t.zmin);
            desc[u] = terrain_desc(p_cur, local);
          }
        }
#pragma unroll
        for (int u = 0; u < TU; ++u) {
          const unsigned long long mk = team_ballot<T>(el[u]);
          if (el[u]) items[n_items + __popcll(mk & ((1ull << tl) - 1ull))] = desc[u];
          n_items += __popcll(mk);
        }
      }
      team_sync();
      {
        int n_keep = 0;
        for (int base = 0; base < n_items; base += T) {
          const int q = base + tl;
          int d = 0; bool keep = false;
          if (q < n_items) {
            d = items[q];
            const auto& t = s->tr.tp[d & 31];
            int r, k;
            terrain_desc_cell(t, d >> 5, r, k);
            keep = !terrain_prism_separated_at_once(m, t, i_terrain, r, k);
          }
          const unsigned long long mk = team_ballot<T>(keep);
          if (keep) items[n_keep + __popcll(mk & ((1ull << tl) - 1ull))] = d;
          n_keep += __popcll(mk);
          team_sync();
        }
        n_items = n_keep;
      }
      PH(27)
      for (int base = 0; base < n_items; base += T) {
        const int q = base + tl;
        float* st = &s->stage[tl][0][0];
        int has = 0;
        if (q < n_items) {
          int d = items[q];
          const auto& t = s->tr.tp[d & 31];
          V3 normal, cpos; float pen;
          int r, k;
          terrain_desc_cell(t, d >> 5, r, k);
          if (terrain_prism_contact(m, e, t, i_terrain, r, k, normal, cpos, pen)) {
            has = 1 + (d & 31);
            st[0] = normal.x; st[1] = normal.y; st[2] = normal.z; st[3] = cpos.x; st[4] = cpos.y; st[5] = cpos.z; st[6] = pen;
          }
        }
        s->cnt[tl] = has;
        team_sync();
        PH(28)
        unsigned long long hm = team_ballot<T>(has != 0);
        int n_acc = 0, my_l = -1, my_ic = 0;
        while (hm) {
          const int l = __ffsll((long long)hm) - 1;
          hm &= hm - 1ull;
          const int p = s->cnt[l] - 1;
          if (p != cur_p) { cur_p = p; n_con = 0; tolerance = s->tr.tp[p].tol; }
          if (n_con >= m.n_contacts_per_pair) continue;
          const float* pc = &s->stage[l][0][0];
          const V3 cpos = v3(pc[3], pc[4], pc[5]);
          bool valid = true;
#pragma unroll
          for (int jj = 0; jj < 5; ++jj)
            if (jj < n_con && nc_run - n_con + jj < m.max_contact_pairs && norm(cpos - acc[jj]) < tolerance) valid = false;
          if (!valid) continue;
#pragma unroll
          for (int jj = 0; jj < 5; ++jj) if (jj == n_con) acc[jj] = cpos;
          if (tl == n_acc) { my_l = l; my_ic = nc_run; }
          n_acc++; nc_run++; n_con++;
        }
        if (my_l >= 0) {
          if (my_ic < m.max_contact_pairs) {
            const float* pc = &s->stage[my_l][0][0];
            const int i_ga = s->tr.tp[s->cnt[my_l] - 1].i_ga, i_c = my_ic;
            float friction_a = e.geom_friction()[i_ga] * e.friction_ratio()[i_ga];
            float friction_b = e.geom_friction()[i_terrain] * e.friction_ratio()[i_terrain];
            e.c_geom()[i_c] = i_ga; e.c_geom()[MAXC + i_c] = i_terrain;
            e.c_normal()[i_c] = v3(pc[0], pc[1], pc[2]); e.c_pos()[i_c] = v3(pc[3], pc[4], pc[5]); e.c_pen()[i_c] = pc[6];
            e.c_friction()[i_c] = fmx(fmx(friction_a, friction_b), 1e-2f);
            auto sol = e.c_sol()[i_c];
            for (int qq = 0; qq < 7; ++qq) sol[qq] = 0.5f * (m.geoms[i_ga].sol_params[qq] + m.geoms[i_terrain].sol_params[qq]);
            e.c_link()[i_c] = m.geoms[i_ga].link; e.c_link()[MAXC + i_c] = m.geoms[i_terrain].link;
          } else {
            atomicOr(&e.err()[0], GO2SIM_ERR_OVERFLOW_COLLISION_PAIRS);
          }
        }
        team_sync();
        PH(29)
      }
    }
  }
  if (tl == 0) {
    e.n_broad()[0] = n_broad; e.n_contacts()[0] = imn(nc_run, m.max_contact_pairs);
    s->cnt[0] = imn(nc_run, m.max_contact_pairs);
  }
  team_sync();
  if (lpt_rec && tl == 0 && b % solver_epw == 0) {
    int key = s->cnt[0];
    for (int k = 1; k < solver_epw; ++k) if (b + k < P.B && slot + k < EPW) key = imx(key, lds[slot + k].cnt[0]);
    lpt_file(lpt_rec, lpt_cap, b / solver_epw, P.B, solver_epw, key);
  }
  for (int i = tl; i < NCV; i += T) e.ncache_valid()[i] = (int)s->ncv[i];
  PH(33)
}

struct LsPoint { float alpha, cost, grad, hess; };
DEV int update_bracket(LsPoint& p, const float alphas[3], const float costs[3], const float grads[3], const float hess[3], float& p_next_alpha) {
  int flag = 0;
#pragma unroll
  for (int i = 0; i < 3; ++i) {
    if (p.grad < 0 && grads[i] < 0 && p.grad < grads[i]) { p.alpha = alphas[i]; p.cost = costs[i]; p.grad = grads[i]; p.hess = hess[i]; flag = 1; }
    else if (p.grad > 0 && grads[i] > 0 && p.grad > grads[i]) { p.alpha = alphas[i]; p.cost = costs[i]; p.grad = grads[i]; p.hess = hess[i]; flag = 2; }
  }
  p_next_alpha = p.alpha;
  if (flag > 0) p_next_alpha = p.alpha - p.grad / p.hess;
  return flag;
}

struct BrOut { float alpha, cost, grad, hess, next_alpha; int flag; };
DEVN BrOut update_bracket_v(float pa, float pc, float pg, float ph, float a0, float a1, float a2, float c0, float c1, float c2, float g0, float g1, float g2,
                            float h0, float h1, float h2) {
  LsPoint p = {pa, pc, pg, ph};
  const float alphas[3] = {a0, a1, a2}, costs[3] = {c0, c1, c2}, grads[3] = {g0, g1, g2}, hess[3] = {h0, h1, h2};
  int flag = 0;
#pragma unroll
  for (int i = 0; i < 3; ++i) {
    if (p.grad < 0 && grads[i] < 0 && p.grad < grads[i]) { p.alpha = alphas[i]; p.cost = costs[i]; p.grad = grads[i]; p.hess = hess[i]; flag = 1; }
    else if (p.grad > 0 && grads[i] > 0 && p.grad > grads[i]) { p.alpha = alphas[i]; p.cost = costs[i]; p.grad = grads[i]; p.hess = hess[i]; flag = 2; }
  }
  float next_alpha = p.alpha;
  if (flag > 0) next_alpha = p.alpha - p.grad / p.hess;
  BrOut o = {p.alpha, p.cost, p.grad, p.hess, next_alpha, flag};
  return o;
}

constexpr int RL = 32;
constexpr int RL_TERRAIN = 96;
constexpr int DS = 20;

template <int R>
struct alignas(16) SolverData {
  float J[R * DS];
  float H[ND * DS];
  float M[ND * DS];
  float qacc[DS], Ma[DS], grad[DS], Mgrad[DS], search[DS], mv[DS], force[DS], acc_smooth[DS], qfrc[DS], ntv[DS], vel[DS];
  union {
    struct { float cdof_ang[ND * 3], cdof_vel[ND * 3], root_com[NL * 3]; alignas(16) float rot[ND][4]; };
    float Ablk[21 * 9];
  };
  alignas(16) float aref[R];
  alignas(16) float efc_D[R]; alignas(16) float Jaref[R]; alignas(16) float jv[R]; alignas(16) float efc_force[R];
  alignas(16) float qf0[R]; alignas(16) float qf1[R]; alignas(16) float qf2[R]; alignas(16) float DA[R];
  alignas(16) int active[R]; alignas(16) int prev_active[R];
};

template <int T>
DEV float team_bcast(float x, const int k) {
  if constexpr (T == 64) {
    return __int_as_float(__builtin_amdgcn_readlane(__float_as_int(x), k));
  } else if constexpr (T == 32) {
    const int lo = __builtin_amdgcn_readlane(__float_as_int(x), k), hi = __builtin_amdgcn_readlane(__float_as_int(x), 32 + k);
    return __int_as_float((threadIdx.x & 32) ? hi : lo);
  } else {
    return __shfl(x, k, T);
  }
}
template <int T>
DEV float team_bcast_dyn(float x, int k_uniform) {
  static_assert(T == 32 || T == 64, "teams of 32 or 64 lanes");
  const int k = __builtin_amdgcn_readfirstlane(k_uniform);
  if constexpr (T == 64) {
    return __int_as_float(__builtin_amdgcn_readlane(__float_as_int(x), k));
  } else {
    const int lo = __builtin_amdgcn_readlane(__float_as_int(x), k), hi = __builtin_amdgcn_readlane(__float_as_int(x), 32 + k);
    return __int_as_float((threadIdx.x & 32) ? hi : lo);
  }
}
DEV float dpp_row_shr1(float x) { return __int_as_float(__builtin_amdgcn_update_dpp(0, __float_as_int(x), 0x111, 0xf, 0xf, true)); }
template <int T, int NQ>
DEV void team_serial_sum(const float (&x)[NQ], const float (&base)[NQ], int tl, int nseg, float (&total)[NQ]) {
  float acc[NQ], xx[NQ];
#pragma unroll
  for (int q = 0; q < NQ; ++q) { acc[q] = (tl == 0) ? base[q] + x[q] : x[q]; xx[q] = acc[q]; }
  for (int seg = 0; seg < nseg; ++seg) {
    if (seg > 0) {
#pragma unroll
      for (int q = 0; q < NQ; ++q) {
        const float carry = team_bcast_dyn<T>(acc[q], 16 * seg - 1);
        if (tl == 16 * seg) { acc[q] = carry + x[q]; xx[q] = acc[q]; }
      }
    }
#pragma unroll
    for (int st = 1; st < 16; ++st) {
#pragma unroll
      for (int q = 0; q < NQ; ++q) acc[q] = dpp_row_shr1(acc[q]) + xx[q];
    }
  }
#pragma unroll
  for (int q = 0; q < NQ; ++q) total[q] = team_bcast_dyn<T>(acc[q], 16 * nseg - 1);
}

template <int T, int NQ>
DEV void team_tree_sum(const float (&x)[NQ], float (&total)[NQ]) {
  static_assert(T == 32 || T == 64, "teams of 32 or 64 lanes");
  float a[NQ];
#pragma unroll
  for (int q = 0; q < NQ; ++q) a[q] = x[q];
#pragma unroll
  for (int q = 0; q < NQ; ++q) a[q] = a[q] + dpp_perm<0xB1>(a[q]);
#pragma unroll
  for (int q = 0; q < NQ; ++q) a[q] = a[q] + dpp_perm<0x4E>(a[q]);
#pragma unroll
  for (int q = 0; q < NQ; ++q) a[q] = a[q] + dpp_perm<0x141>(a[q]);
#pragma unroll
  for (int q = 0; q < NQ; ++q) a[q] = a[q] + dpp_perm<0x140>(a[q]);
#pragma unroll
  for (int q = 0; q < NQ; ++q) {
    const auto r = __builtin_amdgcn_permlane16_swap(__float_as_uint(a[q]), __float_as_uint(a[q]), false, false);
    const float pair = __uint_as_float(r[0]) + __uint_as_float(r[1]);
    if constexpr (T == 32) total[q] = pair;
    else { const auto h = __builtin_amdgcn_permlane32_swap(__float_as_uint(pair), __float_as_uint(pair), false, false); total[q] = __uint_as_float(h[0]) + __uint_as_float(h[1]); }
  }
}
template <int T>
DEV float team_tree_sum1(float x) { const float xs[1] = {x}; float t[1]; team_tree_sum<T, 1>(xs, t); return t[0]; }

template <int T, class S, class MT>
DEV void ts_update_constraint(const MT& m, S* s, int tl, int n_con, float& cost, float& prev_cost, float& gauss) {
  prev_cost = cost;
  float row_cost = 0.0f;
  bool first_row = true;
  for (int c = tl; c < n_con; c += T) {
    s->prev_active[c] = s->active[c];
    float Ja = s->Jaref[c];
    int act = Ja < 0.0f;
    s->active[c] = act;
    float D = s->efc_D[c];
    const float DA = D * (float)act;
    s->DA[c] = DA;
    s->efc_force[c] = 0.0f + (-Ja * D * (float)act);
    const float rc = 0.5f * (Ja * Ja * DA);
#if GO2SIM_FAST_ORDER
    row_cost = first_row ? rc : row_cost + rc;
    first_row = false;
#else
    row_cost = rc;
// ... 987 lines not shown
          grad_norm = tot[0];
#endif
        } else {
#pragma unroll
          for (int d = 0; d < ND; ++d) { float g = s->grad[d]; grad_norm = grad_norm + g * g; }
        }
        grad_norm = dm_sqrt(grad_norm);
        bool improved = (grad_norm > tol_scaled) && (improvement > tol_scaled);
        if (!improved) break;
      }
      if (it == m.iterations) break;
      for (int d = tl; d < ND; d += T) s->search[d] = -s->Mgrad[d];
      team_sync();
      float alpha = ts_linesearch<T>(m, s, tl, n_con, gauss);
      PH(6)
      iters++;
      if (dm_abs(alpha) < m.eps) break;
      team_sync();
      for (int d = tl; d < ND; d += T) {
        s->qacc[d] = s->qacc[d] + s->search[d] * alpha;
        s->Ma[d] = s->Ma[d] + s->mv[d] * alpha;
      }
      for (int c = tl; c < n_con; c += T) s->Jaref[c] = s->Jaref[c] + s->jv[c] * alpha;
      team_sync();
      ts_update_constraint<T>(m, s, tl, n_con, cost, prev_cost, gauss);
      PH(7)
      need_full = ts_cholesky_incremental<T>(m, s, tl, n_con);
      team_sync();
      PH(8)
    }
  }
  return iters;
}

template <int T, class S, class MT>
DEV void ts_commit(const MT& m, const E& e, S* s, int tl, int nc, int n_con, int iters) {
  const int d0 = tl < ND ? tl : ND - 1, c0 = tl < nc ? tl : (nc > 0 ? nc - 1 : 0);
  const float qfs0 = aload(e, AO(qf_smooth), d0);
  V3 cn0 = v3(0, 0, 0); float fr0 = 0.0f; int lk0 = 0;
  if (nc > 0) { cn0 = e.c_normal()[c0]; fr0 = e.c_friction()[c0]; lk0 = e.c_link()[c0] | (e.c_link()[MAXC + c0] << 8); }
  int err = 0;
  for (int d = tl; d < ND; d += T) {
    float q = s->qacc[d];
    astore(e, AO(acc), d, q);
    astore(e, AO(force), d, ((d == d0) ? qfs0 : aload(e, AO(qf_smooth), d)) + s->qfrc[d]);
    astore(e, AO(qacc_ws), d, q);
    astore(e, AO(qfrc_constraint), d, s->qfrc[d]);
    if (isnan_(q)) err |= GO2SIM_ERR_INVALID_FORCE_NAN;
  }
  if (err) atomicOr(&e.err()[0], err);
  for (int c = tl; c < n_con; c += T) astore(e, AO(efc_force), c, s->efc_force[c]);
  if (tl == 0) { e.is_warmstart()[0] = 1; e.n_con()[0] = n_con; e.solver_iters()[0] = iters; }
  team_sync();
  float* cf = s->J;
  for (int i_c = tl; i_c < nc; i_c += T) {
    const bool pre = i_c == c0;
    V3 cnormal = pre ? cn0 : (V3)e.c_normal()[i_c]; float friction = pre ? fr0 : (float)e.c_friction()[i_c];
    V3 f = v3(0, 0, 0), d1, d2;
    orthogonals(cnormal, d1, d2);
#pragma unroll
    for (int i_dir = 0; i_dir < 4; ++i_dir) {
      V3 d = (float)(2 * (i_dir % 2) - 1) * ((i_dir < 2) ? d1 : d2);
      V3 n = d * friction - cnormal;
      f = f + n * s->efc_force[i_c * 4 + i_dir];
    }
    e.c_force()[i_c] = f;
    cf[4 * i_c] = f.x; cf[4 * i_c + 1] = f.y; cf[4 * i_c + 2] = f.z;
    ((int*)cf)[4 * i_c + 3] = pre ? lk0 : (e.c_link()[i_c] | (e.c_link()[MAXC + i_c] << 8));
  }
  team_sync();
  for (int i_l = tl; i_l < NL; i_l += T) {
    V3 acc = v3(0, 0, 0);
#pragma unroll 4
    for (int i_c = 0; i_c < nc; ++i_c) {
      int lk = ((const int*)cf)[4 * i_c + 3];
      int la = lk & 0xff, lb = lk >> 8;
      V3 f = v3(cf[4 * i_c], cf[4 * i_c + 1], cf[4 * i_c + 2]);
      if (la == i_l) acc = acc - f;
      if (lb == i_l) acc = acc + f;
    }
    e.contact_force()[i_l] = acc;
  }
}

template <int T>
DEVN void ts_solve_overflow(float* Pf, int* Pi, int PB, float* Pfa, int* Pia, int b, const LinkS* lnk, const unsigned char* tri_i, const unsigned char* tri_j,
                            const Model* __restrict__ gm, SolverData<MAXR>* s, int tl, int nc, int n_con, unsigned lim_mask, int ws_flag) {
  Pool P; P.f = Pf; P.i = Pi; P.B = PB; P.fa = Pfa; P.ia = Pia;
  const E e(P, b);
  const ModelView m(lnk, tri_i, tri_j, gm);
  int iters = ts_solve<T>(m, e, s, tl, nc, n_con, lim_mask, ws_flag);
  ts_commit<T>(m, e, s, tl, nc, n_con, iters);
}

template <int T, int RLN>
DEV void solve_body(const Pool& P, const Model* __restrict__ gm, const ModelS* __restrict__ mp, SolverData<MAXR>* __restrict__ overflow,
                    const int* __restrict__ lpt_rec, int* __restrict__ lpt_next, int lpt_cap, SolverData<RLN>* lds, char* blk_raw, int& b_out, bool& resident_out) {
  constexpr int EPW = 64 / T;
  const LinkS* lnk = (const LinkS*)blk_raw;
  const unsigned char* tri_i = (const unsigned char*)(blk_raw + sizeof(LinkS) * NL);
  const unsigned char* tri_j = tri_i + (NTRI + 1);
  static_assert(T >= NJ, "one lane per joint in the limit test");
  PH_BEGIN
  wg_dma_to_lds<SOLVER_BLOCK_BYTES>(blk_raw, mp->links);
  const int tl = threadIdx.x % T, slot = threadIdx.x / T;
  const int b = lpt_take(lpt_rec, lpt_cap, P.B, EPW, slot);
  if (lpt_next && blockIdx.x == 0) for (int i = threadIdx.x; i < 8 * LPT_CLS; i += 64) lpt_next[i] = 0;
  const bool env_valid = b < P.B;
  b_out = b; resident_out = false;
  E e(P, env_valid ? b : P.B - 1);
  const int nc = e.n_contacts()[0];
  const int ws_flag = e.is_warmstart()[0];
  const JLim jl = mp->jlim[tl < NJ ? tl : NJ - 1];
  const float q_lim = gload(e, FO(qpos), jl.q_start < 0 ? 0 : jl.q_start);
  const bool lim = tl < NJ && jl.q_start >= 0 && fmn(q_lim - jl.lo, jl.hi - q_lim) < 0;
  const unsigned lim_mask = (unsigned)((__ballot(lim) >> (slot * T)) & ((T == 64) ? ~0ull : ((1ull << T) - 1ull)));
  const int n_lim = __popc(lim_mask);
  __syncthreads();
  PH(9)
  const ModelView m(lnk, tri_i, tri_j, gm);
  if (!env_valid) return;
  const int n_con = 4 * nc + n_lim;
  if (n_con <= RLN) {
    SolverData<RLN>* s = &lds[slot];
    resident_out = true;
    int iters = ts_solve<T>(m, e, s, tl, nc, n_con, lim_mask, ws_flag);
    PH(10)
    ts_commit<T>(m, e, s, tl, nc, n_con, iters);
    PH(11)
  } else {
    ts_solve_overflow<T>(P.f, P.i, P.B, P.fa, P.ia, b, lnk, tri_i, tri_j, gm, &overflow[b], tl, nc, n_con, lim_mask, ws_flag);
  }
}
template <int T, int RLN>
__global__ __launch_bounds__(64) __attribute__((amdgpu_waves_per_eu(2, 2))) void k_constraint_solve_team(Pool P, const Model* __restrict__ gm, const ModelS* __restrict__ mp, SolverData<MAXR>* __restrict__ overflow,
                                                                                                         const int* __restrict__ lpt_rec, int* __restrict__ lpt_next, int lpt_cap) {
  STAMP(STK_SOLVE)
  constexpr int EPW = 64 / T;
  __shared__ SolverData<RLN> lds[EPW];
  __shared__ alignas(16) char blk_raw[lds_dma_bytes(SOLVER_BLOCK_BYTES)];
  int b; bool resident;
  solve_body<T, RLN>(P, gm, mp, overflow, lpt_rec, lpt_next, lpt_cap, lds, blk_raw, b, resident);
}

constexpr size_t cmax(size_t a, size_t b) { return a > b ? a : b; }
template <int T, int RLN, bool WITH_DYN>
__global__ __launch_bounds__(64) __attribute__((amdgpu_waves_per_eu(2, 2))) void k_solve_integrate_team(Pool P, const Model* __restrict__ gm, const ModelS* __restrict__ mp,
                                                                                                        SolverData<MAXR>* __restrict__ overflow, const int* __restrict__ lpt_rec,
                                                                                                        int* __restrict__ lpt_next, int lpt_cap) {
  STAMP(STK_SOLVE)
  constexpr int EPW = 64 / T;
  constexpr size_t SOLVE_OFF = (sizeof(SolverData<RLN>) * EPW + 15) / 16 * 16, DYN_OFF = (sizeof(DynData) * EPW + 15) / 16 * 16, KIN_OFF = (sizeof(KinData) * EPW + 15) / 16 * 16;
  constexpr size_t SOLVE_BYTES = SOLVE_OFF + lds_dma_bytes(SOLVER_BLOCK_BYTES);
  constexpr size_t DYN_BYTES = DYN_OFF + MODELS_LDS_BYTES + sizeof(KinSeparate<KIN_OVERLAY, EPW>);
  constexpr size_t KIN_BYTES = KIN_OFF + MODELS_LDS_BYTES;
  __shared__ alignas(16) char raw[cmax(SOLVE_BYTES, WITH_DYN ? DYN_BYTES : KIN_BYTES)];
  const int tl = threadIdx.x % T, slot = threadIdx.x / T;
  int b; bool resident;
  SolverData<RLN>* lds = (SolverData<RLN>*)raw;
  solve_body<T, RLN>(P, gm, mp, overflow, lpt_rec, lpt_next, lpt_cap, lds, raw + SOLVE_OFF, b, resident);
  const bool pre = b < P.B && resident;
  const int dd = tl < ND ? tl : ND - 1;
  const float pre_vel = pre ? lds[slot].vel[dd] : 0.0f, pre_acc = pre ? lds[slot].qacc[dd] : 0.0f;
  __builtin_amdgcn_fence(__ATOMIC_RELEASE, "workgroup");
  __syncthreads();
  __builtin_amdgcn_fence(__ATOMIC_ACQUIRE, "workgroup");
  if constexpr (WITH_DYN) {
    DynData* lds_d = (DynData*)raw;
    char* ms_raw = raw + DYN_OFF;
    auto& lds_k = *(KinSeparate<KIN_OVERLAY, EPW>*)(ms_raw + MODELS_LDS_BYTES);
    integrate_fk_dynamics_body<T>(P, mp, b, lds_d, ms_raw, lds_k, pre, pre_vel, pre_acc);
  } else {
    integrate_fk_body<T>(P, mp, b, (KinData*)raw, raw + KIN_OFF, pre, pre_vel, pre_acc);
  }
}

__global__ __launch_bounds__(64) void k_debug_narrowphase(const Model* __restrict__ mp, int which, int i_ga, int i_gb, V3 pa, Q4 qa, V3 pb, Q4 qb,
                                                          GjkStoreFull* __restrict__ full, float* __restrict__ out8) {
  __shared__ GjkStoreLds slots[GJK_SLOTS_MAX];
  __shared__ GjkStoreTeam team_store;
  __shared__ unsigned mask;
  if (threadIdx.x == 0) mask = 0u;
  __syncthreads();
  const Model& m = *mp;
  bool is_col = false; V3 normal = v3(0, 0, 0), pos = v3(0, 0, 0); float pen = 0.0f;
  if (which >= 3) {
    if (threadIdx.x >= 16) return;
    DgPair dp; dp.m = mp; dp.i_ga = i_ga; dp.i_gb = i_gb; dp.pos_a = pa; dp.quat_a = qa; dp.pos_b = pb; dp.quat_b = qb;
    dp.ga = geom_lite(m, i_ga); dp.gb = geom_lite(m, i_gb); dp.ra = make_rot(qa); dp.rb = make_rot(qb);
    dp.discrete = m.geoms[i_ga].type == GEOM_BOX && m.geoms[i_gb].type == GEOM_BOX;
    DgResult r;
    if (which <= 4) {
      if (threadIdx.x >= 4) return;
      r = (which == 3) ? dgc_contact<4>(dp, slots[0], m.eps, (int)threadIdx.x) : dgc_contact<4>(dp, *full, m.eps, (int)threadIdx.x);
      if (r.overflow) r = dgc_contact<4>(dp, *full, m.eps, (int)threadIdx.x);
    } else {
      r = (which == 5) ? dgc_contact<16>(dp, team_store, m.eps, (int)threadIdx.x) : dgc_contact<16>(dp, *full, m.eps, (int)threadIdx.x);
      if (r.overflow) r = dgc_contact<16>(dp, *full, m.eps, (int)threadIdx.x);
    }
    if (threadIdx.x != 0) return;
    is_col = r.is_col; pen = r.penetration; normal = r.normal; pos = r.pos;
    out8[0] = is_col ? 1.0f : 0.0f; out8[1] = pen; out8[2] = normal.x; out8[3] = normal.y; out8[4] = normal.z; out8[5] = pos.x; out8[6] = pos.y; out8[7] = pos.z;
    return;
  }
  if (threadIdx.x != 0) return;
  if (which == 0) {
    Pair pr; pr.i_ga = i_ga; pr.i_gb = i_gb; pr.pos_a = pa; pr.quat_a = qa; pr.pos_b = pb; pr.quat_b = qb; pr.prism = nullptr; pr.ga = geom_lite(m, i_ga); pr.gb = geom_lite(m, i_gb);
    pair_set_rots(pr);
    mpr_contact(m, pr, v3(0, 0, 0), is_col, normal, pen, pos);
  } else {
    DgPair dp; dp.m = mp; dp.i_ga = i_ga; dp.i_gb = i_gb; dp.pos_a = pa; dp.quat_a = qa; dp.pos_b = pb; dp.quat_b = qb;
    dp.ga = geom_lite(m, i_ga); dp.gb = geom_lite(m, i_gb); dp.ra = make_rot(qa); dp.rb = make_rot(qb);
    dp.discrete = m.geoms[i_ga].type == GEOM_BOX && m.geoms[i_gb].type == GEOM_BOX;
    const DgResult r = (which == 1) ? gjk_query(dp, slots, &mask, full, m.eps) : gjk_query(dp, nullptr, &mask, full, m.eps);
    is_col = r.is_col; pen = r.penetration; normal = r.normal; pos = r.pos;
  }
  out8[0] = is_col ? 1.0f : 0.0f; out8[1] = pen; out8[2] = normal.x; out8[3] = normal.y; out8[4] = normal.z; out8[5] = pos.x; out8[6] = pos.y; out8[7] = pos.z;
}

__global__ __launch_bounds__(WG) void k_clear_ext(Pool P) {
  int b = blockIdx.x * WG + threadIdx.x;
  if (b >= P.B) return;
  E e(P, b);
  auto ext = e.ext();
  for (int i = 0; i < NL * 6; ++i) ext[i] = 0.0f;
}

struct DCfg { double d[GO2SIM_FC_N_HOST]; float f[GO2SIM_FC_COUNT]; int i[GO2SIM_IC_COUNT]; };
struct Acc { double timeouts, tracking, ep[NREW]; int n_reset_now; int done; };
typedef go2sim_env_globals_t Glob;

enum { RNG_ACTION_NOISE = 1, RNG_PUSH = 2, RNG_CMD = 3, RNG_OBS_NOISE = 4, RNG_RESET_DR = 5, RNG_GLOBAL_DR = 6, RNG_RESET_CMD = 7, RNG_RESET_POSE = 8, RNG_TERRAIN_ROW = 9, RNG_TERRAIN_PERM = 10, RNG_RESET_KPKD = 11 };
__host__ __device__ inline dm_u4 rng4(uint64_t seed, uint32_t purpose, uint32_t env, uint32_t step, uint32_t idx) {
#ifdef GO2SIM_RNG_CONST
  dm_u4 o; o.v[0] = o.v[1] = o.v[2] = o.v[3] = step; (void)purpose; (void)env; (void)idx; (void)seed; return o;
#else
  return dm_philox(env, step, purpose, idx, (uint32_t)seed, (uint32_t)(seed >> 32));
#endif
}
__host__ __device__ inline float rand_float(double lower, double upper, uint32_t r) { return (float)(upper - lower) * dm_u01(r) + (float)lower; }
#ifdef GO2SIM_RNG_CONST
DEV int rand_int(int lower, int upper, uint32_t r) { return lower + (int)(dm_rng_const_u(r) * (float)(upper - lower + 1)); }
#else
DEV int rand_int(int lower, int upper, uint32_t r) { return lower + (int)(r % (uint32_t)(upper - lower + 1)); }
#endif
__host__ __device__ inline double clamp01d(double x) { return x < 0.0 ? 0.0 : (x > 1.0 ? 1.0 : x); }
__host__ __device__ inline double lerpd(double a, double b, double t) { t = clamp01d(t); return a + (b - a) * t; }
__host__ __device__ inline double lerp_lo(const DCfg& c, int easy_lo, double t) { return lerpd(c.d[easy_lo], c.d[easy_lo + 2], t); }
__host__ __device__ inline double lerp_hi(const DCfg& c, int easy_lo, double t) { return lerpd(c.d[easy_lo + 1], c.d[easy_lo + 3], t); }
DEV void sample_commands(const DCfg& c, const Glob& g, const dm_u4& r, int b, float& cx, float& cy, float& cz) {
  cx = rand_float(g.cmd_x_lo, g.cmd_x_hi, r.v[0]); cy = rand_float(g.cmd_y_lo, g.cmd_y_hi, r.v[1]); cz = rand_float(g.cmd_yaw_lo, g.cmd_yaw_hi, r.v[2]);
  if (!c.i[GO2SIM_IC_COMPOUND_COMMANDS]) {
    const int choice = rand_int(0, 2, r.v[3]);
    if (choice != 0) cx = 0.0f;
    if (choice != 1) cy = 0.0f;
    if (choice != 2) cz = 0.0f;
  }
  if (b < c.i[GO2SIM_IC_N_STANDING]) { cx = 0.0f; cy = 0.0f; cz = 0.0f; }
}

DEV Q4 tc_quat_mul(Q4 u, Q4 v) {
  float w1 = u.w, x1 = u.x, y1 = u.y, z1 = u.z, w2 = v.w, x2 = v.x, y2 = v.y, z2 = v.z;
  float ww = (z1 + x1) * (x2 + y2), yy = (w1 - y1) * (w2 + z2), zz = (w1 + y1) * (w2 - z2);
  float xx = ww + yy + zz;
  float qq = 0.5f * (xx + (z1 - x1) * (x2 - y2));
  Q4 o = q4(qq - ww + (z1 - y1) * (y2 - z2), qq - xx + (x1 + w1) * (x2 + w2), qq - yy + (w1 - x1) * (y2 + z2), qq - zz + (z1 + y1) * (w2 - x2));
  float n = dm_sqrt(norm_sqr(o));
  return q4(o.w / n, o.x / n, o.y / n, o.z / n);
}
DEV V3 tc_transform_by_quat(V3 v, Q4 q) {
  float q_ww = q.w * q.w, q_wx = q.w * q.x, q_wy = q.w * q.y, q_wz = q.w * q.z;
  float q_xx = q.x * q.x, q_xy = q.x * q.y, q_xz = q.x * q.z, q_yy = q.y * q.y, q_yz = q.y * q.z, q_zz = q.z * q.z;
  float den = q_ww + q_xx + q_yy + q_zz;
  float vx = v.x / den, vy = v.y / den, vz = v.z / den;
  return v3(vx * (q_xx + q_ww - q_yy - q_zz) + vy * (2.0f * q_xy - 2.0f * q_wz) + vz * (2.0f * q_xz + 2.0f * q_wy),
            vx * (2.0f * q_wz + 2.0f * q_xy) + vy * (q_ww - q_xx + q_yy - q_zz) + vz * (2.0f * q_yz - 2.0f * q_wx),
            vx * (2.0f * q_xz - 2.0f * q_wy) + vy * (2.0f * q_wx + 2.0f * q_yz) + vz * (q_ww - q_xx - q_yy + q_zz));
}
DEV V3 tc_quat_to_xyz_rpy_deg(Q4 q, float eps) {
  float q_ww = q.w * q.w, q_wx = q.w * q.x, q_wy = q.w * q.y, q_wz = q.w * q.z;
  float q_xx = q.x * q.x, q_xy = q.x * q.y, q_xz = q.x * q.z, q_yy = q.y * q.y, q_yz = q.y * q.z, q_zz = q.z * q.z;
  float sinp = q_wy - q_xz, sinrcosp = q_wx + q_yz, sinycosp = q_wz + q_xy;
  float cosrcosp = (q_ww - q_xx - q_yy + q_zz) / 2.0f, cosycosp = (q_ww + q_xx - q_yy - q_zz) / 2.0f;
  float cosp = dm_sqrt(cosycosp * cosycosp + sinycosp * sinycosp);
  float x = dm_atan2(sinrcosp, cosrcosp), y = dm_atan2(sinp, cosp), z = dm_atan2(sinycosp, cosycosp);
  if (cosp < eps) { x = 0.0f; z = dm_atan2(q_wz - q_xy, (q_ww - q_xx + q_yy - q_zz) / 2.0f); }
  const float R2D = 57.29577951308232f;
  return v3(x * R2D, y * R2D, z * R2D);
}

__host__ __device__ inline double dr_level(const DCfg& c, double terrain_level) {
  if (!c.i[GO2SIM_IC_DR_SCHEDULE]) return terrain_level;
  double gate = c.d[GO2SIM_FC_DR_TERRAIN_GATE], p1 = c.d[GO2SIM_FC_DR_PHASE1_LEVEL];
  if (terrain_level < gate) return p1;
  double den = 1.0 - gate; if (den < 1e-6) den = 1e-6;
  double progress = clamp01d((terrain_level - gate) / den);
  return lerpd(p1, 1.0, progress);
}
DEV float terrain_height(const Model& m, const DCfg& c, float x, float y) {
  if (!c.i[GO2SIM_IC_USE_TERRAIN] || !m.terrain_enabled) return 0.0f;
  long long col = (long long)((x - c.f[GO2SIM_FC_TERRAIN_ORIGIN_X]) / c.f[GO2SIM_FC_TERRAIN_H_SCALE]);
  long long row = (long long)((y - c.f[GO2SIM_FC_TERRAIN_ORIGIN_Y]) / c.f[GO2SIM_FC_TERRAIN_H_SCALE]);
  col = col < 0 ? 0 : (col > m.terrain_rows - 1 ? m.terrain_rows - 1 : col);
  row = row < 0 ? 0 : (row > m.terrain_cols - 1 ? m.terrain_cols - 1 : row);
  return m.terrain_hf[(size_t)col * m.terrain_cols + row];
}
__host__ __device__ inline void apply_curriculum_level(const DCfg& c, Glob& g) {
  double lvl_terrain = c.i[GO2SIM_IC_CURR_ENABLED] ? g.level : 1.0;
  double lvl = dr_level(c, lvl_terrain);
  g.obs_noise_level_cur = lerpd(0.0, c.i[GO2SIM_IC_HAS_OBS_NOISE] ? c.d[GO2SIM_FC_OBS_NOISE_LEVEL_MAX] : 0.0, lvl);
  g.action_noise_std_cur = lerpd(0.0, c.d[GO2SIM_FC_ACTION_NOISE_STD_MAX], lvl);
  double dt = c.d[GO2SIM_FC_DT];
  if (!c.i[GO2SIM_IC_HAS_PUSH]) {
    g.push_enable = 0; g.push_force_lo = g.push_force_hi = 0.0; g.push_interval = 1000000000;
  } else {
    double push_start = c.d[GO2SIM_FC_PUSH_START];
    if (lvl < push_start) {
      g.push_enable = 0; g.push_force_lo = g.push_force_hi = 0.0;
      g.push_interval = (int)(c.d[GO2SIM_FC_PUSH_INTERVAL_S_EASY] / dt);
    } else {
      double den = 1.0 - push_start; if (den < 1e-6) den = 1e-6;
      double s = clamp01d((lvl - push_start) / den);
      g.push_force_lo = c.d[GO2SIM_FC_PUSH_FORCE_LO] * s;
      g.push_force_hi = c.d[GO2SIM_FC_PUSH_FORCE_HI] * s;
// ... 12 lines not shown
    g.cmd_y_lo = center - half * frac; g.cmd_y_hi = center + half * frac;
    lo = c.d[GO2SIM_FC_CMD_YAW_LO]; hi = c.d[GO2SIM_FC_CMD_YAW_HI]; center = (lo + hi) / 2.0; half = (hi - lo) / 2.0;
    g.cmd_yaw_lo = center - half * frac; g.cmd_yaw_hi = center + half * frac;
  }
}

__host__ __device__ inline bool curriculum_update(const DCfg& c, Glob& g, double timeout_rate, double tracking_per_sec, double fall_rate) {
  double a = c.d[GO2SIM_FC_CURR_EMA_ALPHA];
  if (!g.ema_valid) { g.timeout_rate_ema = timeout_rate; g.tracking_ema = tracking_per_sec; g.fall_rate_ema = fall_rate; g.ema_valid = 1; }
  else {
    g.timeout_rate_ema = (1.0 - a) * g.timeout_rate_ema + a * timeout_rate;
    g.tracking_ema = (1.0 - a) * g.tracking_ema + a * tracking_per_sec;
    g.fall_rate_ema = (1.0 - a) * g.fall_rate_ema + a * fall_rate;
  }
  if (g.cooldown > 0) g.cooldown -= 1;
  bool ready = g.timeout_rate_ema >= c.d[GO2SIM_FC_CURR_READY_TIMEOUT_RATE] && g.tracking_ema >= c.d[GO2SIM_FC_CURR_READY_TRACKING] &&
               g.fall_rate_ema <= c.d[GO2SIM_FC_CURR_READY_FALL_RATE];
  bool hard = g.fall_rate_ema >= c.d[GO2SIM_FC_CURR_HARD_FALL_RATE];
  g.ready_streak = ready ? g.ready_streak + 1 : 0;
  g.hard_streak = hard ? g.hard_streak + 1 : 0;
  double old_level = g.level;
  if (g.hard_streak >= c.i[GO2SIM_IC_CURR_HARD_STREAK]) {
    { double lo = c.d[GO2SIM_FC_CURR_LEVEL_MIN], v = g.level - c.d[GO2SIM_FC_CURR_STEP_DOWN]; g.level = (lo < v) ? v : lo; }
    g.hard_streak = 0; g.ready_streak = 0; g.cooldown = c.i[GO2SIM_IC_CURR_COOLDOWN];
  } else if (g.ready_streak >= c.i[GO2SIM_IC_CURR_READY_STREAK] && g.cooldown == 0) {
    { double hi = c.d[GO2SIM_FC_CURR_LEVEL_MAX], v = g.level + c.d[GO2SIM_FC_CURR_STEP_UP]; g.level = (v < hi) ? v : hi; }
    g.ready_streak = 0; g.cooldown = c.i[GO2SIM_IC_CURR_COOLDOWN];
  }
  g.level = clamp01d(g.level);
  return g.level != old_level;
}

__global__ __launch_bounds__(WG) void k_env_pre(Pool P, const Model* __restrict__ mp, const DCfg cv, const Glob* __restrict__ gp,
                                                const float* __restrict__ actions_in, uint64_t seed, uint32_t step_count, int write_idx) {
  int b = blockIdx.x * WG + threadIdx.x;
  if (b >= P.B) return;
  const DCfg& c = cv;  const Glob& g = *gp;
  E e(P, b);
  const int na = c.i[GO2SIM_IC_NUM_ACTIONS];
  float clip = c.f[GO2SIM_FC_CLIP_ACTIONS];
  auto actions = e.actions(); auto hist = e.action_history(); auto applied = e.applied_actions();
  auto target_dof_pos = e.target_dof_pos(); auto kp_factors = e.kp_factors(); auto kd_factors = e.kd_factors(); auto motor_strength = e.motor_strength();
  auto dof_pos = e.e_dof_pos(); auto dof_vel = e.e_dof_vel(); auto torque_ = e.torque(); auto ctrl_mode = e.ctrl_mode(); auto ctrl_force = e.ctrl_force();
  auto cpf = e.current_push_force(); auto psf = e.push_stored_force(); auto prem = e.push_remaining(); auto ext = e.ext();
  const bool manual_pd = c.i[GO2SIM_IC_MANUAL_PD] != 0, pls = c.i[GO2SIM_IC_PLS_ENABLE] != 0;
  const bool push_on = c.i[GO2SIM_IC_HAS_PUSH] && g.push_enable;
  const int pl = c.i[GO2SIM_IC_PUSH_LINK];
  int delay = e.delay_steps()[0];
  const bool base_env = c.i[GO2SIM_IC_ENV_KIND] == 1;
  const int depth = c.i[GO2SIM_IC_MAX_DELAY] + 1;
  const int read_idx = (((write_idx - delay) % depth) + depth) % depth;
  auto last_a = e.last_actions();
  float a_in[NA], h_[NA];
#pragma unroll
  for (int i = 0; i < NA; ++i) {
    a_in[i] = (i < na) ? actions_in[(size_t)b * na + i] : 0.0f;
    h_[i] = base_env ? last_a[i] : hist[read_idx][i];
  }
  float kpf[NM], kdf[NM], mst[NM], dp[NM], dv[NM];
#pragma unroll
  for (int i = 0; i < NM; ++i) { kpf[i] = kp_factors[i]; kdf[i] = kd_factors[i]; mst[i] = motor_strength[i]; dp[i] = dof_pos[i]; dv[i] = dof_vel[i]; }
  float bkp = c.f[GO2SIM_FC_KP], bkd = c.f[GO2SIM_FC_KD];
  if (manual_pd && !pls && c.i[GO2SIM_IC_HAS_KP_RANGE]) { bkp = e.base_kp()[0]; bkd = e.base_kd()[0]; }
  float psf_[3] = {psf[0], psf[1], psf[2]}; int rem0 = prem[0];
  V3 pl_pos = e.l_pos()[pl], pl_com = e.root_com()[pl];
  float ext_[6];
#pragma unroll
  for (int k = 0; k < 6; ++k) ext_[k] = ext[6 * pl + k];
  float delayed[NA];
#pragma unroll
  for (int i = 0; i < NA; ++i) {
    if (i < na) {
      float a = fmn(fmx(a_in[i], -clip), clip);
      actions[i] = a;
      float d;
      if (base_env) d = (depth > 1) ? h_[i] : a;
      else { hist[write_idx][i] = a; d = (read_idx == write_idx) ? a : h_[i]; }
      delayed[i] = d; applied[i] = d;
    } else {
      delayed[i] = 0.0f;
    }
  }
  float target[NM];
#pragma unroll
  for (int i = 0; i < NM; ++i) target[i] = delayed[i] * c.f[GO2SIM_FC_ACTION_SCALE] + c.f[GO2SIM_FC_DEFAULT_DOF_POS0 + i];
  if (g.action_noise_std_cur > 0.0) {
#pragma unroll
    for (int blk = 0; blk < 3; ++blk) {
      dm_u4 r = rng4(seed, RNG_ACTION_NOISE, b, step_count, blk);
      float n0, n1, n2, n3;
      dm_normal2(r.v[0], r.v[1], &n0, &n1); dm_normal2(r.v[2], r.v[3], &n2, &n3);
      target[4 * blk + 0] = target[4 * blk + 0] + n0 * (float)g.action_noise_std_cur;
      target[4 * blk + 1] = target[4 * blk + 1] + n1 * (float)g.action_noise_std_cur;
      target[4 * blk + 2] = target[4 * blk + 2] + n2 * (float)g.action_noise_std_cur;
      target[4 * blk + 3] = target[4 * blk + 3] + n3 * (float)g.action_noise_std_cur;
    }
  }
  if (!manual_pd) {
    auto ctrl_pos = e.ctrl_pos(); auto ctrl_vel = e.ctrl_vel();
#pragma unroll
    for (int i = 0; i < NM; ++i) {
      target_dof_pos[i] = target[i];
      int d = c.i[GO2SIM_IC_MOTOR_DOF0 + i];
      ctrl_mode[d] = CTRL_POSITION; ctrl_pos[d] = target[i]; ctrl_vel[d] = 0.0f; ctrl_force[d] = 0.0f;
      torque_[i] = 0.0f;
    }
  } else
#pragma unroll
  for (int i = 0; i < NM; ++i) {
    target_dof_pos[i] = target[i];
    float eff_kp, eff_kd;
    if (pls) {
      int leg = i / 3;
      float kp_leg = c.f[GO2SIM_FC_PLS_KP_DEFAULT] + delayed[NM + leg] * c.f[GO2SIM_FC_PLS_KP_ACTION_SCALE];
      kp_leg = fmn(fmx(kp_leg, c.f[GO2SIM_FC_PLS_KP_MIN]), c.f[GO2SIM_FC_PLS_KP_MAX]);
      float kd_j = 0.2f * dm_sqrt(kp_leg);
      eff_kp = kp_leg * kpf[i] * mst[i];
      eff_kd = kd_j * kdf[i];
    } else {
      eff_kp = bkp * kpf[i]; eff_kd = bkd * kdf[i];
    }
    float pos_error = target[i] - dp[i];
    float torque = eff_kp * pos_error - eff_kd * dv[i];
    float lim = c.f[GO2SIM_FC_TORQUE_LIMIT0 + i];
    torque = fmn(fmx(torque, -lim), lim);
    torque_[i] = torque;
    int d = c.i[GO2SIM_IC_MOTOR_DOF0 + i];
    ctrl_mode[d] = CTRL_FORCE; ctrl_force[d] = torque;
  }
  if (!push_on) {
    cpf[0] = 0.0f; cpf[1] = 0.0f; cpf[2] = 0.0f;
  } else {
    if (g.push_counter % g.push_interval == 0) {
      dm_u4 r = rng4(seed, RNG_PUSH, b, step_count, 0);
      psf_[0] = rand_float(g.push_force_lo, g.push_force_hi, r.v[0]);
      psf_[1] = rand_float(g.push_force_lo, g.push_force_hi, r.v[1]);
      psf_[2] = 0.0f;
      psf[0] = psf_[0]; psf[1] = psf_[1]; psf[2] = psf_[2];
      rem0 = rand_int(c.i[GO2SIM_IC_PUSH_DUR_LO], c.i[GO2SIM_IC_PUSH_DUR_HI], r.v[2]);
    }
    int rem = rem0;
    float active = (rem > 0) ? 1.0f : 0.0f;
    V3 force = v3(psf_[0] * active, psf_[1] * active, psf_[2] * active);
    cpf[0] = force.x; cpf[1] = force.y; cpf[2] = force.z;
    prem[0] = imx(rem - 1, 0);
    V3 tq = cross(pl_pos - pl_com, force);
    ext[6 * pl + 0] = ext_[0] - tq.x; ext[6 * pl + 1] = ext_[1] - tq.y; ext[6 * pl + 2] = ext_[2] - tq.z;
    ext[6 * pl + 3] = ext_[3] - force.x; ext[6 * pl + 4] = ext_[4] - force.y; ext[6 * pl + 5] = ext_[5] - force.z;
  }
}

template <int T>
__global__ __launch_bounds__(64) void k_pre_dynamics_team(Pool P, const ModelS* __restrict__ mp, const DCfg cv, const Glob* __restrict__ gp,
                                                          const float* __restrict__ actions_in, uint64_t seed, uint32_t step_count, int write_idx) {
  STAMP(STK_PRE_DYN)
  static_assert(T >= NA, "one lane per action");
  constexpr int EPW = 64 / T;
  __shared__ DynData lds[EPW];
  __shared__ alignas(16) char ms_raw[MODELS_LDS_BYTES];
  const ModelS& ms = *(const ModelS*)ms_raw;
  wg_dma_to_lds<(int)sizeof(ModelS)>(ms_raw, mp);
  {
    const int b0 = xcd_block() * EPW;
    wg_load<EPW, NL * 3>(P, b0, FO(cd_vel), [&](int ev, int k, float v) { lds[ev].cd_vel[k] = v; });
    wg_load<EPW, NL * 3>(P, b0, FO(cd_ang), [&](int ev, int k, float v) { lds[ev].cd_ang[k] = v; });
    wg_load<EPW, ND>(P, b0, FO(vel), [&](int ev, int k, float v) { lds[ev].vel[k] = v; });
  }
  const int tl = threadIdx.x % T, slot = threadIdx.x / T;
  const int b = xcd_block() * EPW + slot;
  const bool env_valid = b < P.B;
  const ModelView m(&ms, mp);
  E e(P, env_valid ? b : P.B - 1);
  DynData* s = &lds[slot];
  const DCfg& c = cv; const Glob& g = *gp;
  PH_BEGIN
  const int na = c.i[GO2SIM_IC_NUM_ACTIONS];
  const int ia = tl < NA ? tl : NA - 1, im = tl < NM ? tl : NM - 1;
  const int eb = env_valid ? b : P.B - 1;
  auto hist = e.action_history();
  const int delay = e.delay_steps()[0];
  const float a_in = (ia < na) ? actions_in[(size_t)eb * na + ia] : 0.0f;
  const bool base_env = c.i[GO2SIM_IC_ENV_KIND] == 1;
  const int depth = c.i[GO2SIM_IC_MAX_DELAY] + 1;
  const int read_idx = (((write_idx - delay) % depth) + depth) % depth;
  const float h_ = base_env ? e.last_actions()[ia] : hist[read_idx][ia];
  const float kpf = e.kp_factors()[im], kdf = e.kd_factors()[im], mst = e.motor_strength()[im], dp = e.e_dof_pos()[im], dv = e.e_dof_vel()[im];
  const bool manual_pd = c.i[GO2SIM_IC_MANUAL_PD] != 0, pls = c.i[GO2SIM_IC_PLS_ENABLE] != 0;
  const bool base_gains = manual_pd && !pls && c.i[GO2SIM_IC_HAS_KP_RANGE];
  const float bkp = base_gains ? e.base_kp()[0] : c.f[GO2SIM_FC_KP], bkd = base_gains ? e.base_kd()[0] : c.f[GO2SIM_FC_KD];
  const bool push_on = c.i[GO2SIM_IC_HAS_PUSH] && g.push_enable;
  const int pl = c.i[GO2SIM_IC_PUSH_LINK];
  auto psf = e.push_stored_force(); auto prem = e.push_remaining(); auto cpf = e.current_push_force(); auto ext = e.ext();
  float psf_[3] = {psf[0], psf[1], psf[2]}; int rem0 = prem[0];
  const V3 pl_pos = e.l_pos()[pl], pl_com = e.root_com()[pl];
  float ext_[6];
#pragma unroll
  for (int k = 0; k < 6; ++k) ext_[k] = ext[6 * pl + k];
  team_stage<NL * 9, T>(tl, [&](int k) { return aload(e, AO(cinr_inertial), k); }, [&](int k, float v) { s->cinr_I[k] = v; s->crb_I[k] = v; });
  team_stage<NL * 3, T>(tl, [&](int k) { return aload(e, AO(cinr_pos), k); }, [&](int k, float v) { s->cinr_pos[k] = v; s->crb_pos[k] = v; });
  team_stage<NL, T>(tl, [&](int k) { return aload(e, AO(cinr_mass), k); }, [&](int k, float v) { s->cinr_mass[k] = v; s->crb_mass[k] = v; });
  team_stage<ND, T>(tl, [&](int d) { return __int_as_float((int)e.ctrl_mode()[d]); }, [&](int d, float v) { s->ctrl_mode[d] = __float_as_int(v); });
  team_stage<ND * 3, T>(tl, [&](int k) { return aload(e, AO(cdof_ang), k); }, [&](int k, float v) { s->cdof_ang[k] = v; });
  team_stage<ND * 3, T>(tl, [&](int k) { return aload(e, AO(cdof_vel), k); }, [&](int k, float v) { s->cdof_vel[k] = v; });
  team_stage<ND * 3, T>(tl, [&](int k) { return aload(e, AO(cdofd_ang), k); }, [&](int k, float v) { s->cdofd_ang[k] = v; });
  team_stage<ND * 3, T>(tl, [&](int k) { return aload(e, AO(cdofd_vel), k); }, [&](int k, float v) { s->cdofd_vel[k] = v; });
  team_stage<ND, T>(tl, [&](int d) { return gload(e, FO(ctrl_force), d); }, [&](int d, float v) { s->qf_applied[d] = v; });
  team_stage<ND, T>(tl, [&](int d) { return gload(e, FO(ctrl_pos), d); }, [&](int d, float v) { s->qf_passive[d] = v; });
  team_stage<ND, T>(tl, [&](int d) { return gload(e, FO(ctrl_vel), d); }, [&](int d, float v) { s->force[d] = v; });
  team_stage<ND, T>(tl, [&](int d) { return gload(e, FO(dof_pos), d); }, [&](int d, float v) { s->out[d] = v; });
  team_stage<NL * 6, T>(tl, [&](int k) { return gload(e, FO(ext), k); },
                        [&](int k, float v) { int i_l = k / 6, cc = k % 6; if (cc < 3) s->cfrc_ang[3 * i_l + cc] = v; else s->cfrc_vel[3 * i_l + cc - 3] = v; });
  team_sync();
  if (env_valid) {
    const float clip = c.f[GO2SIM_FC_CLIP_ACTIONS];
    float delayed = 0.0f;
    if (tl < NA && tl < na) {
      const float a = fmn(fmx(a_in, -clip), clip);
      e.actions()[tl] = a;
      if (base_env) delayed = (depth > 1) ? h_ : a;
      else { hist[write_idx][tl] = a; delayed = (read_idx == write_idx) ? a : h_; }
      e.applied_actions()[tl] = delayed;
    }
    const float delayed_leg = __shfl(delayed, NM + im / 3, T);
    if (tl < NM) {
      float target = delayed * c.f[GO2SIM_FC_ACTION_SCALE] + c.f[GO2SIM_FC_DEFAULT_DOF_POS0 + tl];
      if (g.action_noise_std_cur > 0.0) {
        dm_u4 r = rng4(seed, RNG_ACTION_NOISE, b, step_count, tl / 4);
        float n0, n1;
        if ((tl & 2) == 0) dm_normal2(r.v[0], r.v[1], &n0, &n1); else dm_normal2(r.v[2], r.v[3], &n0, &n1);
        target = target + ((tl & 1) ? n1 : n0) * (float)g.action_noise_std_cur;
      }
      e.target_dof_pos()[tl] = target;
      const int d = c.i[GO2SIM_IC_MOTOR_DOF0 + tl];
      if (!manual_pd) {
        e.ctrl_mode()[d] = CTRL_POSITION; e.ctrl_pos()[d] = target; e.ctrl_vel()[d] = 0.0f; e.ctrl_force()[d] = 0.0f;
        e.torque()[tl] = 0.0f;
        s->ctrl_mode[d] = CTRL_POSITION; s->qf_passive[d] = target; s->force[d] = 0.0f; s->qf_applied[d] = 0.0f;
      } else {
        float eff_kp, eff_kd;
        if (pls) {
          float kp_leg = c.f[GO2SIM_FC_PLS_KP_DEFAULT] + delayed_leg * c.f[GO2SIM_FC_PLS_KP_ACTION_SCALE];
          kp_leg = fmn(fmx(kp_leg, c.f[GO2SIM_FC_PLS_KP_MIN]), c.f[GO2SIM_FC_PLS_KP_MAX]);
          const float kd_j = 0.2f * dm_sqrt(kp_leg);
          eff_kp = kp_leg * kpf * mst;
          eff_kd = kd_j * kdf;
        } else {
          eff_kp = bkp * kpf; eff_kd = bkd * kdf;
        }
        const float pos_error = target - dp;
        float torque = eff_kp * pos_error - eff_kd * dv;
        const float lim = c.f[GO2SIM_FC_TORQUE_LIMIT0 + tl];
        torque = fmn(fmx(torque, -lim), lim);
        e.torque()[tl] = torque;
        e.ctrl_mode()[d] = CTRL_FORCE; e.ctrl_force()[d] = torque;
        s->ctrl_mode[d] = CTRL_FORCE; s->qf_applied[d] = torque;
      }
    }
    if (tl == T - 1) {
      if (!push_on) {
        cpf[0] = 0.0f; cpf[1] = 0.0f; cpf[2] = 0.0f;
      } else {
        if (g.push_counter % g.push_interval == 0) {
          dm_u4 r = rng4(seed, RNG_PUSH, b, step_count, 0);
          psf_[0] = rand_float(g.push_force_lo, g.push_force_hi, r.v[0]);
          psf_[1] = rand_float(g.push_force_lo, g.push_force_hi, r.v[1]);
          psf_[2] = 0.0f;
          psf[0] = psf_[0]; psf[1] = psf_[1]; psf[2] = psf_[2];
          rem0 = rand_int(c.i[GO2SIM_IC_PUSH_DUR_LO], c.i[GO2SIM_IC_PUSH_DUR_HI], r.v[2]);
        }
        const float active = (rem0 > 0) ? 1.0f : 0.0f;
        const V3 force = v3(psf_[0] * active, psf_[1] * active, psf_[2] * active);
        cpf[0] = force.x; cpf[1] = force.y; cpf[2] = force.z;
        prem[0] = imx(rem0 - 1, 0);
        const V3 tq = cross(pl_pos - pl_com, force);
        const float x0 = ext_[0] - tq.x, x1 = ext_[1] - tq.y, x2 = ext_[2] - tq.z, x3 = ext_[3] - force.x, x4 = ext_[4] - force.y, x5 = ext_[5] - force.z;
        ext[6 * pl + 0] = x0; ext[6 * pl + 1] = x1; ext[6 * pl + 2] = x2; ext[6 * pl + 3] = x3; ext[6 * pl + 4] = x4; ext[6 * pl + 5] = x5;
        s->cfrc_ang[3 * pl + 0] = x0; s->cfrc_ang[3 * pl + 1] = x1; s->cfrc_ang[3 * pl + 2] = x2;
        s->cfrc_vel[3 * pl + 0] = x3; s->cfrc_vel[3 * pl + 1] = x4; s->cfrc_vel[3 * pl + 2] = x5;
      }
    }
  }
  team_sync();
  PH(20)
  tk_dynamics<T>(m, e, s, tl, env_valid);
}

struct RewCtx { float link_vel_xy[8], foot_z[4], foot_xy[8]; float vel_world[3]; int was_reset; };
struct RewState {
  float cmd[3], blv[3], bav[3], pg[3], base_pos[3];
  float dof_pos[NM], dof_vel[NM], last_dof_vel[NM], target[NM], ctrl_force[NM];
  float actions[NA], last_actions[NA];
  float fat[4]; int fc[4];
  float last_x;
  float ctrl_pos[NM], ctrl_vel[NM], s_vel[NM], s_dof_pos[NM]; int ctrl_mode[NM];
};
DEV void load_rew_state(const DCfg& c, const E& e, RewState& rs) {
  auto cmd = e.commands(); auto ldv = e.last_dof_vel(); auto t = e.target_dof_pos(); auto cf = e.ctrl_force(); auto a = e.actions(); auto la = e.last_actions();
  auto fat = e.feet_air_time();
#pragma unroll
  for (int i = 0; i < 3; ++i) rs.cmd[i] = cmd[i];
#pragma unroll
  for (int i = 0; i < NM; ++i) { rs.last_dof_vel[i] = ldv[i]; rs.target[i] = t[i]; rs.ctrl_force[i] = cf[c.i[GO2SIM_IC_MOTOR_DOF0 + i]]; }
#pragma unroll
  for (int i = 0; i < NA; ++i) { rs.actions[i] = a[i]; rs.last_actions[i] = la[i]; }
#pragma unroll
  for (int i = 0; i < 4; ++i) rs.fat[i] = fat[i];
  rs.last_x = e.last_base_pos_x()[0];
  if (c.i[GO2SIM_IC_ENV_KIND] == 1) {
    auto ctrl_mode = e.ctrl_mode(); auto cp = e.ctrl_pos(); auto cv = e.ctrl_vel(); auto vel = e.vel(); auto sdp = e.dof_pos();
#pragma unroll
    for (int i = 0; i < NM; ++i) {
      int d = c.i[GO2SIM_IC_MOTOR_DOF0 + i];
      rs.ctrl_mode[i] = ctrl_mode[d]; rs.ctrl_pos[i] = cp[d]; rs.ctrl_vel[i] = cv[d]; rs.s_vel[i] = vel[d]; rs.s_dof_pos[i] = sdp[d];
    }
  }
}
struct RewGates { float still, moving; };
DEV RewGates reward_gates(const RewState& rs) {
  const float c0 = rs.cmd[0], c1 = rs.cmd[1], c2 = rs.cmd[2];
  const float cmd_norm = dm_sqrt(c0 * c0 + c1 * c1 + c2 * c2);
  RewGates g;
  g.still = (cmd_norm < 0.1f) ? 1.0f : 0.0f;
  g.moving = (dm_sqrt(c0 * c0 + c1 * c1) > 0.1f) ? 1.0f : 0.0f;
  return g;
}
DEV float reward_term(const Model& m, const DCfg& c, RewState& rs, int id, const RewCtx& rc, const RewGates& gt) {
  const float dt = c.f[GO2SIM_FC_DT];
  const float* cmd = rs.cmd; const float* blv = rs.blv; const float* bav = rs.bav; const float* dof_pos = rs.dof_pos; const float* dof_vel = rs.dof_vel;
  float c0 = cmd[0], c1 = cmd[1], c2 = cmd[2];
  const float still = gt.still, moving = gt.moving;
  switch (id) {
    case GO2SIM_R_TRACKING_LIN_VEL: { float d0 = c0 - blv[0], d1 = c1 - blv[1]; return dm_exp(-(d0 * d0 + d1 * d1) / c.f[GO2SIM_FC_TRACKING_SIGMA]); }
    case GO2SIM_R_TRACKING_ANG_VEL: { float d = c2 - bav[2]; return dm_exp(-(d * d) / c.f[GO2SIM_FC_TRACKING_SIGMA]); }
    case GO2SIM_R_LIN_VEL_Z: {
      float v = blv[2], dz = c.f[GO2SIM_FC_LIN_VEL_Z_DEADZONE];
      if (dz > 0.0f) { float ex = fmx(dm_abs(v) - dz, 0.0f); return ex * ex; }
      return v * v;
    }
    case GO2SIM_R_ACTION_RATE: {
      float s = 0.0f; const int na = c.i[GO2SIM_IC_NUM_ACTIONS];
#pragma unroll
      for (int i = 0; i < NA; ++i) if (i < na) { float d = rs.last_actions[i] - rs.actions[i]; s = s + d * d; }
      return s;
    }
    case GO2SIM_R_SIMILAR_TO_DEFAULT: {
      float s = 0.0f;
#pragma unroll
      for (int i = 0; i < NM; ++i) s = s + dm_abs(dof_pos[i] - c.f[GO2SIM_FC_DEFAULT_DOF_POS0 + i]);
      return s;
    }
    case GO2SIM_R_BASE_HEIGHT: {
      float hgt = rs.base_pos[2];
      if (c.i[GO2SIM_IC_USE_TERRAIN]) hgt = rs.base_pos[2] - terrain_height(m, c, rs.base_pos[0], rs.base_pos[1]);
      float d = hgt - c.f[GO2SIM_FC_BASE_HEIGHT_TARGET]; return d * d;
    }
    case GO2SIM_R_DOF_ACC: {
      float s = 0.0f;
#pragma unroll
      for (int i = 0; i < NM; ++i) { float a = (dof_vel[i] - rs.last_dof_vel[i]) / dt; s = s + a * a; }
      return s;
    }
    case GO2SIM_R_DOF_VEL: {
      float s = 0.0f;
#pragma unroll
      for (int i = 0; i < NM; ++i) { float v = dof_vel[i]; s = s + v * v; }
      return s;
    }
    case GO2SIM_R_ORIENTATION_PENALTY: { float a = rs.pg[0], b2 = rs.pg[1]; return a * a + b2 * b2; }
    case GO2SIM_R_ANG_VEL_XY: { float a = bav[0], b2 = bav[1]; return a * a + b2 * b2; }
    case GO2SIM_R_STAND_STILL: {
      float s = 0.0f;
#pragma unroll
      for (int i = 0; i < NM; ++i) s = s + dm_abs(dof_pos[i] - c.f[GO2SIM_FC_DEFAULT_DOF_POS0 + i]);
      return s * still;
    }
    case GO2SIM_R_STAND_STILL_VEL: { float a = blv[0], b2 = blv[1], w = bav[2]; float lin = a * a + b2 * b2; float ang = w * w; return (lin + 0.5f * ang) * still; }
    case GO2SIM_R_FEET_STANCE: {
      float sa = 0.0f, sn = 0.0f;
#pragma unroll
      for (int i = 0; i < 4; ++i) { sa = sa + rs.fat[i]; sn = sn + (rs.fc[i] ? 0.0f : 1.0f); }
      return (sa + sn) * still;
    }
    case GO2SIM_R_FEET_AIR_TIME: {
      float first[4], at[4];
#pragma unroll
      for (int i = 0; i < 4; ++i) { float a = rs.fat[i]; int ct = rs.fc[i]; first[i] = (a > 0.0f && ct) ? 1.0f : 0.0f; a = a + dt; a = a * (ct ? 0.0f : 1.0f); rs.fat[i] = a; at[i] = a; }
      float s = 0.0f;
#pragma unroll
      for (int i = 0; i < 4; ++i) s = s + (at[i] - c.f[GO2SIM_FC_FEET_AIR_TIME_TARGET]) * first[i];
      return s * moving;
    }
    case GO2SIM_R_FOOT_SLIP: {
      float slip = 0.0f;
#pragma unroll
      for (int i = 0; i < 4; ++i) { float vx = rc.link_vel_xy[2 * i], vy = rc.link_vel_xy[2 * i + 1]; slip = slip + (rs.fc[i] ? 1.0f : 0.0f) * (vx * vx + vy * vy); }
      return slip;
    }
    case GO2SIM_R_FOOT_CLEARANCE: {
      float pen = 0.0f;
#pragma unroll
      for (int i = 0; i < 4; ++i) {
        float vx = rc.link_vel_xy[2 * i], vy = rc.link_vel_xy[2 * i + 1];
        float vn = dm_sqrt(vx * vx + vy * vy);
        float fz = rc.foot_z[i];
        if (c.i[GO2SIM_IC_USE_TERRAIN]) fz = rc.foot_z[i] - terrain_height(m, c, rc.foot_xy[2 * i], rc.foot_xy[2 * i + 1]);
        float he = c.f[GO2SIM_FC_FEET_HEIGHT_TARGET] - fz; he = he * he;
        pen = pen + (rs.fc[i] ? 0.0f : 1.0f) * he * vn;
      }
      return pen * moving;
    }
    case GO2SIM_R_JOINT_TRACKING: {
      float s = 0.0f;
#pragma unroll
      for (int i = 0; i < NM; ++i) { float d = rs.target[i] - dof_pos[i]; s = s + d * d; }
      return s;
    }
    case GO2SIM_R_ENERGY: case GO2SIM_R_TORQUE_LOAD: {
      float s = 0.0f;
#pragma unroll
      for (int i = 0; i < NM; ++i) {
        int d = c.i[GO2SIM_IC_MOTOR_DOF0 + i];
        float tau = clampf(rs.ctrl_force[i], m.dofs[d].force_range[0], m.dofs[d].force_range[1]);
        s = s + ((id == GO2SIM_R_ENERGY) ? dm_abs(tau * dof_vel[i]) : dm_abs(tau));
      }
      return s;
    }
    case GO2SIM_R_JUMP_IMPULSE: { float gate = (rs.base_pos[2] < 0.50f) ? 1.0f : 0.0f; return gate * fmx(blv[2], 0.0f); }
    case GO2SIM_R_JUMP_APEX: { float q = (rs.base_pos[2] - c.f[GO2SIM_FC_JUMP_APEX_HEIGHT]) / c.f[GO2SIM_FC_JUMP_APEX_SIGMA]; return dm_exp(-(q * q)); }
    case GO2SIM_R_XY_STABILITY: { float vx = rc.vel_world[0], vy = rc.vel_world[1]; return -(vx * vx + vy * vy); }
    case GO2SIM_R_ORIENTATION: return -rs.pg[2];
    case GO2SIM_R_NO_SHAKE: { float a = bav[0], b2 = bav[1], c3 = bav[2]; return -((a * a + b2 * b2) + c3 * c3) / 1.0f; }
    case GO2SIM_R_CROUCH: return (rs.base_pos[2] < 0.25f) ? 1.0f : 0.0f;
    case GO2SIM_R_CROUCH_2: { float z = rs.base_pos[2]; return (z <= 0.30f && z >= 0.20f) ? 1.0f : 0.0f; }
    case GO2SIM_R_GROUND_PENALTY: { float v = (0.15f - rs.base_pos[2]) / 0.1f; v = fmn(fmx(v, 0.0f), 1.0f); return -(v * v); }
    case GO2SIM_R_CROUCH_TARGET: { float q = (rs.base_pos[2] - 0.15f) / 0.03f; return dm_exp(-(q * q)); }
    case GO2SIM_R_NO_FALL: { float dn = fmx(-blv[2] - 0.5f, 0.0f); return -(dn * dn); }
    case GO2SIM_R_Y_STABILITY: { float vy = rc.vel_world[1]; return -(vy * vy); }
// ... 741 lines not shown
      auto bq = e.base_quat(); auto bp = e.base_pos();
      float qw = bq[0], qx = bq[1], qy = bq[2], qz = bq[3];
      float yaw = dm_atan2(2.0f * (qw * qz + qx * qy), 1.0f - 2.0f * (qy * qy + qz * qz));
      float sy, cy;
      dm_sincos(yaw, &sy, &cy);
      float lx = c.f[GO2SIM_FC_SCAN_X0 + j - 56], ly = c.f[GO2SIM_FC_SCAN_Y0 + j - 56];
      float wx = bp[0] + cy * lx - sy * ly;
      float wy = bp[1] + sy * lx + cy * ly;
      v = terrain_height(m, c, wx, wy) - bp[2];
    }
    else v = 0.0f;
    if (write) gstore(e, FO(priv), i, v);
    if (priv_out) priv_out[(size_t)b * npriv + i] = v;
  }
  for (int i = tl; i < na; i += T) gstore(e, FO(last_actions), i, gload(e, FO(actions), i));
  for (int i = tl; i < NM; i += T) gstore(e, FO(last_dof_vel), i, src[PB_DV + i]);
  if (tl == 0) {
    if (rew_out) rew_out[b] = e.rew()[0];
    if (reset_out) reset_out[b] = (uint8_t)was_reset;
    if (timeout_out) timeout_out[b] = e.time_out()[0];
  }
  fk_refresh();
}

__global__ __launch_bounds__(WG) void k_init_state(Pool P, const Model* __restrict__ mp, int keep_dr) {
  int b = blockIdx.x * WG + threadIdx.x;
  if (b >= P.B) return;
  const Model& m = *mp;
  E e(P, b);
  auto qpos = e.qpos();
  for (int i = 0; i < NQ; ++i) qpos[i] = m.qpos0[i];
  if (!keep_dr) {
    auto fr = e.friction_ratio(); auto gf = e.geom_friction();
    for (int i = 0; i < NG; ++i) { fr[i] = 1.0f; gf[i] = m.geoms[i].friction; }
  }
  auto l_pos = e.l_pos(); auto l_quat = e.l_quat();
  for (int i = 0; i < NL; ++i) { l_pos[i] = m.links[i].pos; l_quat[i] = m.links[i].quat; }
  e.first_time()[0] = 1;
}
__global__ __launch_bounds__(WG) void k_scene_reset_clear(Pool P) {
  int b = blockIdx.x * WG + threadIdx.x;
  if (b >= P.B) return;
  E e(P, b);
  auto vel = e.vel(); auto acc = e.acc(); auto qacc_ws = e.qacc_ws();
  for (int d = 0; d < ND; ++d) { vel[d] = 0.0f; acc[d] = 0.0f; qacc_ws[d] = 0.0f; }
  auto ncv = e.ncache_valid();
  for (int p = 0; p < NCV; ++p) ncv[p] = 0;
  int nc = e.n_contacts()[0];
  for (int i_c = 0; i_c < nc; ++i_c) { e.c_link()[i_c] = -1; e.c_link()[MAXC + i_c] = -1; e.c_geom()[i_c] = -1; e.c_geom()[MAXC + i_c] = -1; e.c_pen()[i_c] = 0.0f; e.c_pos()[i_c] = v3(0, 0, 0); e.c_normal()[i_c] = v3(0, 0, 0); e.c_force()[i_c] = v3(0, 0, 0); }
  e.n_contacts()[0] = 0; e.err()[0] = 0; e.is_warmstart()[0] = 0; e.n_con()[0] = 0;
  auto ext = e.ext();
  for (int i = 0; i < NL * 6; ++i) ext[i] = 0.0f;
}
__global__ __launch_bounds__(WG) void k_reset_caches(Pool P, const int* __restrict__ envs_idx, int n_sel) {
  int t = blockIdx.x * WG + threadIdx.x;
  if (t >= n_sel) return;
  int b = envs_idx ? envs_idx[t] : t;
  if (b < 0 || b >= P.B) return;
  E e(P, b);
  e.err()[0] = 0; e.is_warmstart()[0] = 0;
  auto qacc_ws = e.qacc_ws();
  for (int d = 0; d < ND; ++d) qacc_ws[d] = 0.0f;
  auto ncv = e.ncache_valid();
  for (int p = 0; p < NCV; ++p) ncv[p] = 0;
}
__global__ __launch_bounds__(WG) void k_set_friction(Pool P, float mu) {
  int b = blockIdx.x * WG + threadIdx.x;
  if (b >= P.B) return;
  E e(P, b);
  auto gf = e.geom_friction();
  for (int i = 0; i < NG; ++i) gf[i] = mu;
}
__global__ __launch_bounds__(WG) void k_env_init_buffers(Pool P, const DCfg* __restrict__ cp) {
  int b = blockIdx.x * WG + threadIdx.x;
  if (b >= P.B) return;
  const DCfg& c = *cp;
  E e(P, b);
  auto kpf = e.kp_factors(); auto kdf = e.kd_factors(); auto mst = e.motor_strength();
  for (int k = 0; k < NM; ++k) { kpf[k] = 1.0f; kdf[k] = 1.0f; mst[k] = 1.0f; }
  e.base_kp()[0] = c.f[GO2SIM_FC_KP]; e.base_kd()[0] = c.f[GO2SIM_FC_KD];
  e.delay_steps()[0] = 1; e.reset_buf()[0] = 1;
  if (c.i[GO2SIM_IC_MANUAL_PD]) for (int k = 0; k < NM; ++k) e.ctrl_mode()[c.i[GO2SIM_IC_MOTOR_DOF0 + k]] = CTRL_FORCE;
}
__global__ void k_errno_reduce(Pool P, int* out) {
  int v = 0;
  for (int b = blockIdx.x * blockDim.x + threadIdx.x; b < P.B; b += gridDim.x * blockDim.x) v |= P.i[(size_t)IO(err) * P.B + b];
  if (v) atomicOr(out, v);
}
__global__ void k_mass_mat_to_rows(const float* __restrict__ rec, int stride, int off, int B, float* __restrict__ rows) {
  const int t = blockIdx.x * blockDim.x + threadIdx.x;
  if (t >= ND * ND * B) return;
  const int idx = t / B, b = t - idx * B, i = idx / ND, j = idx - i * ND, a = i > j ? i : j, c = i > j ? j : i;
  rows[t] = rec[(size_t)b * stride + off + a * (a + 1) / 2 + c];
}
__global__ void k_rows_to_mass_mat(const float* __restrict__ rows, float* __restrict__ rec, int stride, int off, int B) {
  const int t = blockIdx.x * blockDim.x + threadIdx.x;
  if (t >= NTRI * B) return;
  const int p = t / B, b = t - p * B;
  int i = 0;
  while ((i + 1) * (i + 2) / 2 <= p) ++i;
  const int j = p - i * (i + 1) / 2;
  rec[(size_t)b * stride + off + p] = rows[(size_t)(i * ND + j) * B + b];
}
__global__ void k_aos_to_rows(const int* __restrict__ rec, int stride, int off, int k, int B, int* __restrict__ rows) {
  int t = blockIdx.x * blockDim.x + threadIdx.x;
  if (t >= k * B) return;
  int j = t / B, b = t % B;
  rows[t] = rec[(size_t)b * stride + off + j];
}
__global__ void k_rows_to_aos(const int* __restrict__ rows, int* __restrict__ rec, int stride, int off, int k, int B) {
  int t = blockIdx.x * blockDim.x + threadIdx.x;
  if (t >= k * B) return;
  int j = t / B, b = t % B;
  rec[(size_t)b * stride + off + j] = rows[t];
}
__global__ void k_ncache_mask_rows(Pool P, float* __restrict__ rows) {
  int t = blockIdx.x * blockDim.x + threadIdx.x;
  if (t >= NPAIR * P.B) return;
  int p = t / P.B, b = t % P.B;
  E e(P, b);
  if (!(((unsigned)e.ncache_valid()[p >> 5] >> (p & 31)) & 1u)) { rows[(size_t)(3 * p) * P.B + b] = 0.0f; rows[(size_t)(3 * p + 1) * P.B + b] = 0.0f; rows[(size_t)(3 * p + 2) * P.B + b] = 0.0f; }
}
__global__ void k_ncache_set_valid(Pool P) {
  int t = blockIdx.x * blockDim.x + threadIdx.x;
  if (t >= NCV * P.B) return;
  int w = t / P.B, b = t % P.B;
  E e(P, b);
  const int n = NPAIR - 32 * w;
  e.ncache_valid()[w] = (int)(n >= 32 ? 0xffffffffu : ((1u << n) - 1u));
}
__global__ void k_gather(const void* __restrict__ src, void* __restrict__ dst, int k, int B) {
  int t = blockIdx.x * blockDim.x + threadIdx.x;
  if (t >= k * B) return;
  int b = t / k, j = t % k;
  ((uint32_t*)dst)[t] = ((const uint32_t*)src)[(size_t)j * B + b];
}
__global__ void k_scatter(const void* __restrict__ src, void* __restrict__ dst, int k, int B) {
  int t = blockIdx.x * blockDim.x + threadIdx.x;
  if (t >= k * B) return;
  int b = t / k, j = t % k;
  ((uint32_t*)dst)[(size_t)j * B + b] = ((const uint32_t*)src)[t];
}

}

#define HIPCHK(x) do { hipError_t _e = (x); if (_e != hipSuccess) { fprintf(stderr, "go2sim: HIP error %s at %s:%d\n", hipGetErrorString(_e), __FILE__, __LINE__); return GO2SIM_E_HIP; } } while (0)

enum { T_DYN = 0, T_COLLIDE, T_SOLVE, T_INTEGRATE, T_ENV_PRE, T_ENV_POST, T_MISC, T_TOTAL, T_N };
constexpr int TIMING_RING = 2048;

struct Launch {
  void* func; dim3 grid, block;
  int cat;
  bool join;
  std::vector<void*> args;
};
struct LaunchList {
  std::vector<Launch> v;
  std::vector<void*> owned;
  int pre = -1, post_a = -1, post_b = -1;
  hipGraph_t graph = nullptr; hipGraphExec_t exec = nullptr; std::vector<hipGraphNode_t> nodes;
  LaunchList() = default;
  LaunchList(const LaunchList&) = delete;
  LaunchList& operator=(const LaunchList&) = delete;
  ~LaunchList() { clear(); }
  void drop_graph() {
    if (exec) (void)hipGraphExecDestroy(exec);
    if (graph) (void)hipGraphDestroy(graph);
    exec = nullptr; graph = nullptr; nodes.clear();
  }
  void clear() {
    drop_graph();
    for (void* p : owned) free(p);
    owned.clear(); v.clear(); pre = post_a = post_b = -1;
  }
};

struct go2sim {
  int B = 0, device = 0;
  uint64_t seed = 0;
  Model hm;
  Model* dm = nullptr;
  ModelS* dms = nullptr;
  Pool P = {nullptr, nullptr, 0, nullptr, nullptr};
  DCfg hcfg; DCfg* dcfg = nullptr; bool cfg_set = false;
  Glob* dglob = nullptr; Acc* dacc = nullptr; int* derr = nullptr;
  int* herr_pinned = nullptr; hipEvent_t ev_errno = nullptr; bool errno_poll_pending = false;
  int* didx = nullptr; int didx_cap = 0;
  float* terrain_hf = nullptr;
  float* terrain_cmax = nullptr;
  GjkStoreFull* gjk_scratch = nullptr;
  SolverData<MAXR>* solver_ovf = nullptr;
  int* lpt = nullptr; int lpt_cap = 0; int lpt_parity = 0; bool use_lpt = true;
  LaunchList step;
  bool use_graph = true;
  int graph_fallbacks = 0;
  bool fuse_fk_dyn = true;
  bool fuse_solve_int = true;
  bool par_pre = false;
  int dyn_team = 32;
  int fk_team = 16;
  int collide_team = 16;
  int solver_team = 32;
  int terrain_solver_team = 64;
  uint32_t step_count = 0; int action_write_idx = 0;
  bool timing = false;
  hipEvent_t ev0[TIMING_RING], ev1[TIMING_RING]; int ev_cat[TIMING_RING]; int ev_n = 0; bool ev_created = false;
  float t_ms[T_N] = {0}; int t_cnt[T_N] = {0};
};

static inline dim3 grid_for(int B) { return dim3((B + WG - 1) / WG); }

static void timing_flush(go2sim* h) {
  for (int i = 0; i < h->ev_n; ++i) {
    float ms = 0.0f;
    (void)hipEventSynchronize(h->ev1[i]);
    if (hipEventElapsedTime(&ms, h->ev0[i], h->ev1[i]) == hipSuccess) { h->t_ms[h->ev_cat[i]] += ms; h->t_cnt[h->ev_cat[i]] += 1; }
  }
  h->ev_n = 0;
}
struct ScopedTimer {
  go2sim* h; hipStream_t s; int idx;
  ScopedTimer(go2sim* h_, hipStream_t s_, int cat) : h(h_), s(s_), idx(-1) {
    if (!h->timing) return;
    if (h->ev_n == TIMING_RING) return;
    idx = h->ev_n++;
    h->ev_cat[idx] = cat;
    (void)hipEventRecord(h->ev0[idx], s);
  }
  ~ScopedTimer() { if (idx >= 0) (void)hipEventRecord(h->ev1[idx], s); }
};

static dim3 team_grid(const go2sim* h, int T) { return dim3((h->B + 64 / T - 1) / (64 / T)); }
static auto fk_kernel(int T) { if (T == 16) return k_fk_team<16>; if (T == 32) return k_fk_team<32>; return k_fk_team<64>; }
static auto pre_dynamics_kernel(int T) { return T == 32 ? k_pre_dynamics_team<32> : k_pre_dynamics_team<64>; }
static auto dynamics_kernel(int T) { if (T == 16) return k_dynamics_team<16>; if (T == 32) return k_dynamics_team<32>; return k_dynamics_team<64>; }
static auto collide_kernel(int T) { if (T == 16) return k_collide_team<16>; if (T == 32) return k_collide_team<32>; return k_collide_team<64>; }
static auto solve_kernel(bool terrain, int T, int fuse_mode) {
  if (terrain) return T == 32 ? k_constraint_solve_team<32, RL_TERRAIN> : k_constraint_solve_team<64, RL_TERRAIN>;
  if (T == 16) return k_constraint_solve_team<16, RL>;
  if (fuse_mode) return fuse_mode == 1 ? k_solve_integrate_team<32, RL, true> : k_solve_integrate_team<32, RL, false>;
  return T == 32 ? k_constraint_solve_team<32, RL> : k_constraint_solve_team<64, RL>;
}
static auto integrate_kernel(int T) { if (T == 16) return k_integrate_fk_team<16>; if (T == 32) return k_integrate_fk_team<32>; return k_integrate_fk_team<64>; }
static auto integrate_dynamics_kernel(int T) { return T == 32 ? k_integrate_fk_dynamics_team<32> : k_integrate_fk_dynamics_team<64>; }

static void launch_fk_team(go2sim* h, hipStream_t s, int force_update_fixed, const int* cond) {
  hipLaunchKernelGGL(fk_kernel(h->fk_team), team_grid(h, h->fk_team), dim3(64), 0, s, h->P, h->dms, force_update_fixed, cond);
}

static bool fuse_pre(const go2sim* h) { return h->fuse_fk_dyn && h->dyn_team >= 32; }
static int solver_epw(const go2sim* h) { return 64 / (h->hm.terrain_enabled ? h->terrain_solver_team : h->solver_team); }
static bool lpt_enabled(const go2sim* h) { return h->use_lpt && solver_epw(h) == 1; }
static size_t lpt_record_ints(const go2sim* h) { return (size_t)8 * LPT_CLS * (1 + h->lpt_cap); }
static bool fuse_solve(const go2sim* h) { return h->fuse_solve_int && h->fuse_fk_dyn && !h->hm.terrain_enabled && h->solver_team == 32 && h->dyn_team == 32; }

template <class... P, class... A>
static void add_launch(LaunchList& L, int cat, void (*kernel)(P...), dim3 grid, dim3 block, A... a) {
  static_assert(sizeof...(P) == sizeof...(A), "argument count");
  Launch e{(void*)kernel, grid, block, cat, false, {}};
  auto store = [&](auto typed) { using T = decltype(typed); T* m = (T*)malloc(sizeof(T)); memcpy((void*)m, (const void*)&typed, sizeof(T)); L.owned.push_back((void*)m); e.args.push_back((void*)m); };
  (store(static_cast<P>(a)), ...);
  L.v.push_back(std::move(e));
}
struct StepIO { const float* actions; float *obs, *priv, *rew; uint8_t* reset; float* timeout; };
static void build_launch_list(const go2sim* h, LaunchList& L, int n, const StepIO* io) {
  const dim3 ge = grid_for(h->B), b(WG);
  const bool terrain = h->hm.terrain_enabled != 0;
  auto add_dynamics = [&]() { add_launch(L, T_DYN, dynamics_kernel(h->dyn_team), team_grid(h, h->dyn_team), b, h->P, h->dms); };
  if (io) L.pre = 0;
  if (io && fuse_pre(h)) {
    add_launch(L, T_DYN, pre_dynamics_kernel(h->dyn_team), team_grid(h, h->dyn_team), b, h->P, h->dms, h->hcfg, h->dglob, io->actions, h->seed, h->step_count, h->action_write_idx);
  } else {
    if (io) add_launch(L, T_ENV_PRE, k_env_pre, ge, b, h->P, h->dm, h->hcfg, h->dglob, io->actions, h->seed, h->step_count, h->action_write_idx);
    add_dynamics();
  }
  const bool lpt_on = lpt_enabled(h) && !(io && n % 2);
  const int lpt0 = io ? 0 : h->lpt_parity;
  for (int i = 0; i < n; ++i) {
    const bool more = i + 1 < n;
    int* lpt_cur = lpt_on ? h->lpt + ((lpt0 + i) & 1) * lpt_record_ints(h) : nullptr;
    int* lpt_next = lpt_on ? h->lpt + ((lpt0 + i + 1) & 1) * lpt_record_ints(h) : nullptr;
    add_launch(L, T_COLLIDE, collide_kernel(h->collide_team), team_grid(h, h->collide_team), b, h->P, h->dm, h->gjk_scratch, lpt_cur, h->lpt_cap, solver_epw(h));
    const int Ts = terrain ? h->terrain_solver_team : h->solver_team;
    add_launch(L, T_SOLVE, solve_kernel(terrain, Ts, fuse_solve(h) ? (more ? 1 : 2) : 0), team_grid(h, Ts), b, h->P, h->dm, h->dms, h->solver_ovf, lpt_cur, lpt_next, h->lpt_cap);
    L.v.back().join = io && i == 0 && fuse_pre(h) && h->par_pre;
    if (fuse_solve(h)) continue;
    if (more && h->fuse_fk_dyn) {
      const int Td = h->dyn_team == 64 ? 64 : 32;
      add_launch(L, T_INTEGRATE, integrate_dynamics_kernel(Td), team_grid(h, Td), b, h->P, h->dms);
    } else {
      add_launch(L, T_INTEGRATE, integrate_kernel(h->fk_team), team_grid(h, h->fk_team), b, h->P, h->dms);
      if (more) add_dynamics();
    }
  }
  if (!io) return;
  L.post_a = (int)L.v.size();
  add_launch(L, T_ENV_POST, k_env_post_a, ge, dim3(WG * POST_A_NWAVES), h->P, h->dm, h->hcfg, h->dglob, h->dacc, h->seed, h->step_count);
  if (h->hcfg.i[GO2SIM_IC_USE_TERRAIN]) add_launch(L, T_ENV_POST, k_env_terrain_rows, dim3((h->B + 255) / 256), dim3(256), h->P, h->dcfg, h->dglob, h->seed);
  L.post_b = (int)L.v.size();
  add_launch(L, T_ENV_POST, k_env_post_b_team<16>, dim3((h->B + 3) / 4), dim3(128), h->P, h->dm, h->dms, h->dcfg, h->dglob, h->seed, h->step_count, io->obs, io->priv, io->rew, io->reset, io->timeout);
  if (h->hcfg.i[GO2SIM_IC_ENGINE_BATCH_GAIN]) add_launch(L, T_ENV_POST, k_env_engine_gains, dim3(1), dim3(GAIN_WG), h->P, h->dm, h->dms, h->dcfg, h->dglob);
}
template <class T> static void set_arg(Launch& e, int k, T value) { *(T*)e.args[k] = value; }
static void step_list_patch(go2sim* h, const StepIO& io) {
  Launch &pre = h->step.v[h->step.pre], &pa = h->step.v[h->step.post_a], &pb = h->step.v[h->step.post_b];
  set_arg(pre, 4, io.actions); set_arg(pre, 6, h->step_count); set_arg(pre, 7, h->action_write_idx);
  set_arg(pa, 6, h->step_count);
  set_arg(pb, 6, h->step_count); set_arg(pb, 7, io.obs); set_arg(pb, 8, io.priv); set_arg(pb, 9, io.rew); set_arg(pb, 10, io.reset); set_arg(pb, 11, io.timeout);
}

static void run_plain(go2sim* h, hipStream_t s, const LaunchList& L) {
  for (size_t i = 0; i < L.v.size();) {
    const int cat = L.v[i].cat;
    ScopedTimer t(h, s, cat);
    for (; i < L.v.size() && L.v[i].cat == cat; ++i) (void)hipLaunchKernel(L.v[i].func, L.v[i].grid, L.v[i].block, (void**)L.v[i].args.data(), 0, s);
  }
}
static void run_substeps(go2sim* h, hipStream_t s, int n) {
  LaunchList L;
  build_launch_list(h, L, n, nullptr);
  run_plain(h, s, L);
  h->lpt_parity ^= n & 1;
}

static hipKernelNodeParams node_params(const Launch& e) {
  hipKernelNodeParams kp{};
  kp.func = e.func; kp.gridDim = e.grid; kp.blockDim = e.block; kp.sharedMemBytes = 0; kp.kernelParams = (void**)e.args.data(); kp.extra = nullptr;
  return kp;
}
static bool step_graph_build(LaunchList& L) {
  if (hipGraphCreate(&L.graph, 0) != hipSuccess) return false;
  L.nodes.assign(L.v.size(), nullptr);
  hipGraphNode_t last = nullptr, side = nullptr;
  for (size_t i = 0; i < L.v.size(); ++i) {
    if (i + 1 < L.v.size() && L.v[i + 1].join) { side = last; last = nullptr; }
    hipGraphNode_t deps[2] = {last, L.v[i].join ? side : nullptr};
    const int n_deps = (last ? 1 : 0) + ((last && deps[1]) ? 1 : 0);
    const hipKernelNodeParams kp = node_params(L.v[i]);
    if (hipGraphAddKernelNode(&L.nodes[i], L.graph, n_deps ? deps : nullptr, n_deps, &kp) != hipSuccess) return false;
    last = L.nodes[i];
  }
  return hipGraphInstantiate(&L.exec, L.graph, nullptr, nullptr, 0) == hipSuccess;
}
static bool step_graph_launch(LaunchList& L, hipStream_t s) {
  for (int i : {L.pre, L.post_a, L.post_b}) {
    const hipKernelNodeParams kp = node_params(L.v[i]);
    if (hipGraphExecKernelNodeSetParams(L.exec, L.nodes[i], &kp) != hipSuccess) return false;
  }
  return hipGraphLaunch(L.exec, s) == hipSuccess;
}

extern "C" {

static void handle_release(go2sim* h) {
  h->step.clear();
  if (h->ev_created) for (int i = 0; i < TIMING_RING; ++i) { (void)hipEventDestroy(h->ev0[i]); (void)hipEventDestroy(h->ev1[i]); }
  (void)hipFree(h->P.f); (void)hipFree(h->P.i); (void)hipFree(h->P.fa); (void)hipFree(h->P.ia); (void)hipFree(h->dm); (void)hipFree(h->dcfg);
  (void)hipFree(h->dglob); (void)hipFree(h->dacc); (void)hipFree(h->derr); (void)hipFree(h->solver_ovf); (void)hipFree(h->gjk_scratch); (void)hipFree(h->lpt);
  (void)hipFree(h->terrain_hf); (void)hipFree(h->terrain_cmax); (void)hipFree(h->dms); (void)hipFree(h->didx);
  if (h->herr_pinned) (void)hipHostFree(h->herr_pinned);
  if (h->ev_errno) (void)hipEventDestroy(h->ev_errno);
  delete h;
}

static int env_int(const char* name, int unset) { const char* t = getenv(name); return t ? atoi(t) : unset; }
static void read_knobs(go2sim* h) {
  auto team = [](const char* name, int smallest, int* v) { const int t = env_int(name, *v); if ((t == 16 && smallest == 16) || t == 32 || t == 64) *v = t; };
  team("GO2SIM_DYN_TEAM", 16, &h->dyn_team);
  team("GO2SIM_FK_TEAM", 16, &h->fk_team);
  team("GO2SIM_COLLIDE_TEAM", 16, &h->collide_team);
  team("GO2SIM_SOLVER_TEAM", 16, &h->solver_team);
  team("GO2SIM_TERRAIN_SOLVER_TEAM", 32, &h->terrain_solver_team);
  if (env_int("GO2SIM_NO_GRAPH", 0)) h->use_graph = false;
  if (env_int("GO2SIM_NO_FUSE", 0)) h->fuse_fk_dyn = false;
  if (env_int("GO2SIM_NO_FUSE_SOLVE", 0)) h->fuse_solve_int = false;
  if (env_int("GO2SIM_PAR_PRE", 0)) h->par_pre = true;
  if (env_int("GO2SIM_NO_LPT", 0)) h->use_lpt = false;
}

int go2sim_create(const void* blob, size_t nbytes, int n_envs, int device, uint64_t seed, go2sim_t** out) {
  if (!blob || !out || n_envs <= 0) return GO2SIM_E_BADARG;
  int ndev = 0;
  if (hipGetDeviceCount(&ndev) != hipSuccess || ndev <= 0) { fprintf(stderr, "go2sim: no HIP device available (the product has no CPU fallback)\n"); return GO2SIM_E_NODEVICE; }
  if (device < 0 || device >= ndev) return GO2SIM_E_BADARG;
  go2sim* h = new (std::nothrow) go2sim();
  if (!h) return GO2SIM_E_NOMEM;
  if (!parse_model(blob, nbytes, h->hm)) { delete h; return GO2SIM_E_BADMODEL; }
  h->B = n_envs; h->device = device; h->seed = seed;
  int rc = GO2SIM_E_OK;
#define CK(x) do { hipError_t _e = (x); if (_e != hipSuccess) { fprintf(stderr, "go2sim: HIP error %s at %s:%d\n", hipGetErrorString(_e), __FILE__, __LINE__); rc = GO2SIM_E_HIP; goto fail; } } while (0)
  {
    CK(hipSetDevice(device));
    const size_t nf = (size_t)FO_TOTAL * n_envs, ni = (size_t)IO_TOTAL * n_envs;
    CK(hipMalloc((void**)&h->P.f, nf * sizeof(float)));
    CK(hipMalloc((void**)&h->P.i, ni * sizeof(int)));
    h->P.B = n_envs;
    CK(hipMemset(h->P.f, 0, nf * sizeof(float)));
    CK(hipMemset(h->P.i, 0, ni * sizeof(int)));
    CK(hipMalloc((void**)&h->P.fa, (size_t)ASTRIDE * n_envs * sizeof(float)));
    CK(hipMalloc((void**)&h->P.ia, (size_t)AISTRIDE * n_envs * sizeof(int)));
    CK(hipMemset(h->P.fa, 0, (size_t)ASTRIDE * n_envs * sizeof(float)));
    CK(hipMemset(h->P.ia, 0, (size_t)AISTRIDE * n_envs * sizeof(int)));
    CK(hipMalloc((void**)&h->dm, sizeof(Model)));
    CK(hipMemcpy(h->dm, &h->hm, sizeof(Model), hipMemcpyHostToDevice));
    {
      ModelS hs;
      if (!build_model_s(h->hm, hs)) { rc = GO2SIM_E_BADMODEL; goto fail; }
      CK(hipMalloc((void**)&h->dms, MODELS_LDS_BYTES));
      CK(hipMemset(h->dms, 0, MODELS_LDS_BYTES));
      CK(hipMemcpy(h->dms, &hs, sizeof(ModelS), hipMemcpyHostToDevice));
    }
    CK(hipMalloc((void**)&h->dcfg, sizeof(DCfg)));
    CK(hipMalloc((void**)&h->dglob, sizeof(Glob)));
    CK(hipMalloc((void**)&h->dacc, sizeof(Acc)));
    CK(hipMalloc((void**)&h->derr, 2 * sizeof(int)));
    CK(hipMemset(h->derr, 0, 2 * sizeof(int)));
    CK(hipHostMalloc((void**)&h->herr_pinned, 2 * sizeof(int), hipHostMallocDefault));
    h->herr_pinned[0] = h->herr_pinned[1] = 0;
    CK(hipEventCreateWithFlags(&h->ev_errno, hipEventDisableTiming));
    CK(hipMalloc((void**)&h->solver_ovf, (size_t)n_envs * sizeof(SolverData<MAXR>)));
    read_knobs(h);
    CK(hipMalloc((void**)&h->gjk_scratch, (size_t)n_envs * h->collide_team * sizeof(GjkStoreFull)));
    h->lpt_cap = n_envs / 8 + 72;
    CK(hipMalloc((void**)&h->lpt, 2 * lpt_record_ints(h) * sizeof(int)));
    CK(hipMemset(h->lpt, 0, 2 * lpt_record_ints(h) * sizeof(int)));
    Glob g0; memset(&g0, 0, sizeof(g0)); g0.friction = 1.0f;
    CK(hipMemcpy(h->dglob, &g0, sizeof(Glob), hipMemcpyHostToDevice));
    CK(hipMemset(h->dacc, 0, sizeof(Acc)));
    memset(&h->hcfg, 0, sizeof(DCfg));
    hipLaunchKernelGGL(k_init_state, grid_for(n_envs), dim3(WG), 0, 0, h->P, h->dm, 0);
    launch_fk_team(h, 0, 1, nullptr);
    CK(hipGetLastError());
    CK(hipDeviceSynchronize());
  }
#undef CK
  *out = h;
  return GO2SIM_E_OK;
fail:
  handle_release(h);
  return rc;
}

int go2sim_destroy(go2sim_t* h) {
  if (!h) return GO2SIM_E_BADARG;
  (void)hipSetDevice(h->device);
  (void)hipDeviceSynchronize();
  handle_release(h);
  return GO2SIM_E_OK;
}
int go2sim_n_envs(const go2sim_t* h) { return h ? h->B : GO2SIM_E_BADARG; }

int go2sim_scene_reset(go2sim_t* h, void* stream) {
  if (!h) return GO2SIM_E_BADARG;
  hipStream_t s = (hipStream_t)stream;
  ScopedTimer t(h, s, T_MISC);
  hipLaunchKernelGGL(k_scene_reset_clear, grid_for(h->B), dim3(WG), 0, s, h->P);
  hipLaunchKernelGGL(k_init_state, grid_for(h->B), dim3(WG), 0, s, h->P, h->dm, 1);
  launch_fk_team(h, s, 1, nullptr);
  HIPCHK(hipGetLastError());
  return GO2SIM_E_OK;
}
int go2sim_substep(go2sim_t* h, void* stream) {
  if (!h) return GO2SIM_E_BADARG;
  run_substeps(h, (hipStream_t)stream, 1);
  HIPCHK(hipGetLastError());
  return GO2SIM_E_OK;
}
int go2sim_scene_step(go2sim_t* h, int substeps, void* stream) {
  if (!h || substeps <= 0) return GO2SIM_E_BADARG;
  hipStream_t s = (hipStream_t)stream;
  run_substeps(h, s, substeps);
  { ScopedTimer t(h, s, T_MISC); hipLaunchKernelGGL(k_clear_ext, grid_for(h->B), dim3(WG), 0, s, h->P); }
  HIPCHK(hipGetLastError());
  return GO2SIM_E_OK;
}
int go2sim_forward_kinematics(go2sim_t* h, void* stream) {
  if (!h) return GO2SIM_E_BADARG;
  hipStream_t s = (hipStream_t)stream;
  ScopedTimer t(h, s, T_MISC);
  launch_fk_team(h, s, 1, nullptr);
  HIPCHK(hipGetLastError());
  return GO2SIM_E_OK;
}

static int field_lookup(int field, int* k, int* is_int, int* off, int* is_aos = nullptr) {
  int kk = -1, ii = 0, oo = 0, aa = 0;
  switch (field) {
    case GO2SIM_F_QPOS: kk = NQ; oo = FO(qpos); break;
    case GO2SIM_F_VEL: kk = ND; oo = FO(vel); break;
    case GO2SIM_F_ACC: kk = ND; oo = AO(acc); aa = 1; break;
    case GO2SIM_F_QACC_WS: kk = ND; oo = AO(qacc_ws); aa = 1; break;
    case GO2SIM_F_CTRL_FORCE: kk = ND; oo = FO(ctrl_force); break;
    case GO2SIM_F_EXT_FORCE: kk = NL * 6; oo = FO(ext); break;
    case GO2SIM_F_MASS_SHIFT: kk = NL; oo = FO(mass_shift); break;
    case GO2SIM_F_COM_SHIFT: kk = NL * 3; oo = FO(com_shift); break;
    case GO2SIM_F_FRICTION_RATIO: kk = NG; oo = FO(friction_ratio); break;
    case GO2SIM_F_LINK_POS: kk = NL * 3; oo = FO(l_pos); break;
    case GO2SIM_F_LINK_QUAT: kk = NL * 4; oo = FO(l_quat); break;
    case GO2SIM_F_LINK_CDVEL: kk = NL * 3; oo = FO(cd_vel); break;
    case GO2SIM_F_LINK_CDANG: kk = NL * 3; oo = FO(cd_ang); break;
    case GO2SIM_F_ROOT_COM: kk = 3; oo = FO(root_com) + 3; break;
    case GO2SIM_F_CONTACT_FORCE: kk = NL * 3; oo = FO(contact_force); break;
    case GO2SIM_F_MASS_MAT: kk = ND * ND; oo = AO(mass_mat); aa = 1; break;
    case GO2SIM_F_FORCE: kk = ND; oo = AO(qf_smooth); aa = 1; break;
    case GO2SIM_F_ACC_SMOOTH: kk = ND; oo = AO(acc_smooth); aa = 1; break;
    case GO2SIM_F_CONTACT_POS: kk = MAXC * 3; oo = AO(c_pos); aa = 1; break;
    case GO2SIM_F_CONTACT_NORMAL: kk = MAXC * 3; oo = AO(c_normal); aa = 1; break;
    case GO2SIM_F_CONTACT_PEN: kk = MAXC; oo = AO(c_pen); aa = 1; break;
    case GO2SIM_F_NORMAL_CACHE: kk = NPAIR * 3; oo = AO(normal_cache); aa = 1; break;
    case GO2SIM_F_SORT_VALUE: kk = 2 * NG; oo = AO(sort_value); aa = 1; break;
    case GO2SIM_F_GEOM_FRICTION: kk = NG; oo = FO(geom_friction); break;
    case GO2SIM_F_EFC_FORCE: kk = MAXR; oo = AO(efc_force); aa = 1; break;
    case GO2SIM_F_QFRC_CONSTRAINT: kk = ND; oo = AO(qfrc_constraint); aa = 1; break;
    case GO2SIM_F_CTRL_POS: kk = ND; oo = FO(ctrl_pos); break;
    case GO2SIM_F_CTRL_VEL: kk = ND; oo = FO(ctrl_vel); break;
    case GO2SIM_F_DOF_POS: kk = ND; oo = FO(dof_pos); break;
    case GO2SIM_F_BASE_KP: kk = 1; oo = FO(base_kp); break;
    case GO2SIM_F_BASE_KD: kk = 1; oo = FO(base_kd); break;
    case GO2SIM_I_N_CONTACTS: kk = 1; ii = 1; oo = IO(n_contacts); break;
    case GO2SIM_I_CONTACT_GEOMS: kk = 2 * MAXC; ii = 1; oo = AIO(c_geom); aa = 1; break;
    case GO2SIM_I_N_CONSTRAINTS: kk = 1; ii = 1; oo = IO(n_con); break;
    case GO2SIM_I_ERRNO: kk = 1; ii = 1; oo = IO(err); break;
    case GO2SIM_I_IS_WARMSTART: kk = 1; ii = 1; oo = IO(is_warmstart); break;
    case GO2SIM_I_FIRST_TIME: kk = 1; ii = 1; oo = IO(first_time); break;
    case GO2SIM_I_SORT_IG: kk = 2 * NG; ii = 1; oo = AIO(sort_ig); aa = 1; break;
    case GO2SIM_I_N_BROAD: kk = 1; ii = 1; oo = IO(n_broad); break;
    case GO2SIM_I_SOLVER_ITERS: kk = 1; ii = 1; oo = IO(solver_iters); break;
    case GO2SIM_I_CTRL_MODE: kk = ND; ii = 1; oo = IO(ctrl_mode); break;
    default: return GO2SIM_E_BADARG;
// ... 491 lines not shown
```

Before: 16.81 million.

## Move broadphase from collide kernel into dynamics kernels with LDS overlay

Broadphase (AABB computation, sort-and-sweep ranking, candidate pair selection) now runs at the end of each dynamics-bearing kernel instead of at the start of the collide kernel. It reuses the dynamics LDS through an overlay so the dynamics kernels keep their LDS footprint, and candidate compaction switches to ballot/popcount. The collide kernel now reads the precomputed broad pair list, and per-pair material constants are loaded before the narrowphase. The intent is to shorten the collide kernel, which is a long serial stage, and to drop redundant LDS staging. In exchange the dynamics kernels carry more work and register pressure, and the unused parallel-pre graph branch option is removed.

```diff
diff --git a/go2_sim2real_locomotion_rl_amd/csrc/go2sim.hip b/go2_sim2real_locomotion_rl_amd/csrc/go2sim.hip
--- a/go2_sim2real_locomotion_rl_amd/csrc/go2sim.hip
+++ b/go2_sim2real_locomotion_rl_amd/csrc/go2sim.hip
@@ -1557,11 +1557,154 @@
   PH(25)
 }
 
+template <int T> DEV unsigned long long team_ballot(bool p) {
+  const unsigned long long b = __ballot(p);
+  if constexpr (T == 64) return b;
+  else return (b >> (threadIdx.x & (64 - T))) & ((1ull << T) - 1ull);
+}
 template <int T>
-__global__ __launch_bounds__(64) void k_dynamics_team(Pool P, const ModelS* __restrict__ mp) {
+struct BroadData {
+  alignas(16) float amin[NG * 4], amax[NG * 4];
+  alignas(16) unsigned long long skey[2 * NG];
+  alignas(8) int rank_mm[NG * 2];
+  int cand_key[MAXB], cand_pair[MAXB];
+  unsigned short pair_sorted[MAXB];
+};
+constexpr int BROAD_PAD = 12;
+template <int T> constexpr bool BROAD_OVERLAY = sizeof(BroadData<T>) + BROAD_PAD <= sizeof(DynData);
+template <bool OVERLAY, int T> struct BroadSeparate { BroadData<T> k[64 / T]; DEV BroadData<T>* at(int slot, DynData*) { return &k[slot]; } };
+template <int T> struct BroadSeparate<true, T> {
+  DEV BroadData<T>* at(int slot, DynData* d) {
+    static_assert(sizeof(BroadData<T>) + BROAD_PAD <= sizeof(DynData) && sizeof(DynData) % 4 == 0 && alignof(BroadData<T>) == 16, "BroadData overlay");
+    return (BroadData<T>*)((char*)d + (16 - (slot * (int)sizeof(DynData)) % 16) % 16);
+  }
+};
+static_assert((BROAD_OVERLAY<16> && BROAD_OVERLAY<32> && BROAD_OVERLAY<64>) || NG != 28 || ND != 18, "the Go2 shape keeps the dynamics kernels' LDS size");
+
+template <int T>
+DEV void tk_broadphase(const Model& m, const E& e, BroadData<T>* s, int tl) {
+  const float inf = dm_bits2f(0x7f800000u);
+  PH_BEGIN
+  const int nc_old = e.n_contacts()[0];
+  const bool first = e.first_time()[0] != 0;
+  const unsigned ncv_old = (unsigned)e.ncache_valid()[tl < NCV ? tl : NCV - 1];
+  constexpr int n2 = 2 * NG, NK = (2 * NG + T - 1) / T, NPI = (NPAIR + T - 1) / T, NGR = (NG + T - 1) / T;
+  int sig_[NK];
+#pragma unroll
+  for (int q = 0; q < NK; ++q) { const int i = tl + q * T; sig_[q] = e.sort_ig()[i < n2 ? i : n2 - 1]; }
+  int packed_[NPI];
+  {
+    const int n_pairs = m.n_pairs;
+#pragma unroll
+    for (int it = 0; it < NPI; ++it) { int pidx = it * T + tl; int v = m.pair_list[pidx < NPAIR ? pidx : NPAIR - 1]; packed_[it] = (pidx < n_pairs) ? v : -1; }
+  }
+  V3 lower_[NGR], upper_[NGR];
+#pragma unroll
+  for (int g = 0; g < NGR; ++g) {
+    const int i_g = (g * T + tl < NG) ? g * T + tl : NG - 1;
+    V3 lower = v3(inf, inf, inf), upper = v3(-inf, -inf, -inf);
+    V3 gp = e.g_pos()[i_g]; Q4 gq = e.g_quat()[i_g];
+#pragma unroll
+    for (int c = 0; c < 8; ++c) {
+      V3 corner = transform_by_trans_quat(m.geoms[i_g].aabb[c], gp, gq);
+      lower = vmin(lower, corner); upper = vmax(upper, corner);
+    }
+    lower_[g] = lower; upper_[g] = upper;
+  }
+  team_sync();
+#pragma unroll
+  for (int g = 0; g < NGR; ++g) {
+    const int i_g = (g * T + tl < NG) ? g * T + tl : NG - 1;
+    *(float4*)&s->amin[4 * i_g] = make_float4(lower_[g].x, lower_[g].y, lower_[g].z, 0.0f);
+    *(float4*)&s->amax[4 * i_g] = make_float4(upper_[g].x, upper_[g].y, upper_[g].z, 0.0f);
+  }
+  team_sync();
+  PH(30)
+  int r[NK]; float sorted_v[NK]; int sorted_sg[NK];
+  unsigned long long key[NK];
+#pragma unroll
+  for (int q = 0; q < NK; ++q) {
+    const int i = (tl + q * T < n2) ? tl + q * T : n2 - 1;
+    const int sg = first ? ((i >> 1) | ((i & 1) ? 0x100 : 0)) : sig_[q];
+    const int g = sg & 0xff;
+    const float v = (sg & 0x100) ? s->amax[4 * g] : s->amin[4 * g];
+    unsigned u = (unsigned)__float_as_int(v + 0.0f);
+    u = (u & 0x80000000u) ? ~u : (u | 0x80000000u);
+    key[q] = ((unsigned long long)u << 8) | (unsigned long long)i;
+    s->skey[i] = key[q];
+    sorted_v[q] = v; sorted_sg[q] = sg; r[q] = 0;
+  }
+  team_sync();
+#pragma unroll
+  for (int j = 0; j < 2 * NG; ++j) {
+    const unsigned long long kj = s->skey[j];
+#pragma unroll
+    for (int q = 0; q < NK; ++q) r[q] += (kj < key[q]) ? 1 : 0;
+  }
+#pragma unroll
+  for (int q = 0; q < NK; ++q)
+    if (tl + q * T < n2) s->rank_mm[2 * (sorted_sg[q] & 0xff) + ((sorted_sg[q] & 0x100) ? 1 : 0)] = r[q];
+  team_sync();
+  PH(31)
+  int n_cand = 0;
+  unsigned ncv_clear = 0u;
+  static_assert(NCV <= T, "one lane per word of the normal-cache mask");
+#pragma unroll
+  for (int it = 0; it < NPI; ++it) {
+    const int packed = packed_[it];
+    const int a = (packed < 0) ? 0 : (packed & 0xff), bg = (packed < 0) ? 0 : (packed >> 8);
+    const int2 rka = *(const int2*)&s->rank_mm[2 * a], rkb = *(const int2*)&s->rank_mm[2 * bg];
+    const float4 amn = *(const float4*)&s->amin[4 * a], amx = *(const float4*)&s->amax[4 * a], bmn = *(const float4*)&s->amin[4 * bg], bmx = *(const float4*)&s->amax[4 * bg];
+    const int ra = rka.x, rb = rkb.x;
+    const int rs = (ra < rb) ? rb : ra, rf = (ra < rb) ? ra : rb;
+    const int rmax_first = (ra < rb) ? rka.y : rkb.y;
+    const bool swept = packed >= 0 && rs < rmax_first;
+    const bool any1 = (amx.x <= bmn.x) || (amx.y <= bmn.y) || (amx.z <= bmn.z);
+    const bool any2 = (amn.x >= bmx.x) || (amn.y >= bmx.y) || (amn.z >= bmx.z);
+    const bool cand = swept && !(any1 || any2);
+    const unsigned long long cb = team_ballot<T>(cand);
+    if (cand) {
+      const int pos = n_cand + __popcll(cb & ((1ull << tl) - 1ull));
+      if (pos < MAXB) { s->cand_key[pos] = rs * 64 + rf; s->cand_pair[pos] = packed; }
+    }
+    n_cand += __popcll(cb);
+    const unsigned long long sep = team_ballot<T>(swept && (any1 || any2));
+    if constexpr (T < 32) { if (tl == ((it * T) >> 5)) ncv_clear |= (unsigned)(sep << ((it * T) & 31)); }
+    else if constexpr (T == 32) { if (tl == it) ncv_clear |= (unsigned)sep; }
+    else { if (tl == 2 * it) ncv_clear |= (unsigned)sep; if (tl == 2 * it + 1) ncv_clear |= (unsigned)(sep >> 32); }
+  }
+  const bool overflow = n_cand > m.max_broad_pairs;
+  n_cand = imn(n_cand, MAXB);
+  team_sync();
+  for (int c = tl; c < n_cand; c += T) {
+    const int ck = s->cand_key[c]; int cr = 0;
+    for (int j = 0; j < n_cand; ++j) cr += s->cand_key[j] < ck;
+    s->pair_sorted[cr] = (unsigned short)s->cand_pair[c];
+  }
+  const int n_broad = imn(n_cand, m.max_broad_pairs);
+  team_sync();
+  for (int c = tl; c < n_broad; c += T) { int pk = s->pair_sorted[c]; e.broad()[2 * c] = pk & 0xff; e.broad()[2 * c + 1] = pk >> 8; }
+#pragma unroll
+  for (int q = 0; q < NK; ++q) if (tl + q * T < n2) { e.sort_value()[r[q]] = sorted_v[q]; e.sort_ig()[r[q]] = sorted_sg[q]; }
+  if (tl < NCV && ncv_clear != 0u) e.ncache_valid()[tl] = (int)(ncv_old & ~ncv_clear);
+  if (tl == 0) {
+    e.n_broad()[0] = n_broad;
+    if (first) e.first_time()[0] = 0;
+    if (overflow) atomicOr(&e.err()[0], GO2SIM_ERR_OVERFLOW_CANDIDATE_CONTACTS);
+  }
+  for (int i_c = tl; i_c < nc_old; i_c += T) {
+    e.c_link()[i_c] = -1; e.c_link()[MAXC + i_c] = -1; e.c_geom()[i_c] = -1; e.c_geom()[MAXC + i_c] = -1;
+    e.c_pen()[i_c] = 0.0f; e.c_pos()[i_c] = v3(0, 0, 0); e.c_normal()[i_c] = v3(0, 0, 0); e.c_force()[i_c] = v3(0, 0, 0);
+  }
+  PH(32)
+}
+
+template <int T>
+__global__ __launch_bounds__(64) void k_dynamics_team(Pool P, const ModelS* __restrict__ mp, const Model* __restrict__ gm) {
   constexpr int EPW = 64 / T;
-  __shared__ DynData lds[EPW];
+  __shared__ alignas(16) DynData lds[EPW];
   __shared__ alignas(16) char ms_raw[MODELS_LDS_BYTES];
+  __shared__ BroadSeparate<BROAD_OVERLAY<T>, T> lds_b;
   const ModelS& ms = *(const ModelS*)ms_raw;
   wg_dma_to_lds<(int)sizeof(ModelS)>(ms_raw, mp);
   {
@@ -1594,6 +1737,7 @@
   team_sync();
   PH(20)
   tk_dynamics<T>(m, e, s, tl, env_valid);
+  if (env_valid) tk_broadphase<T>(*gm, e, lds_b.at(slot, s), tl);
 }
 
 
@@ -1601,12 +1745,13 @@
 template <int EPW> struct KinSeparate<true, EPW> { DEV KinData* at(int, void* overlay) { return (KinData*)overlay; } };
 constexpr bool KIN_OVERLAY = sizeof(KinData) <= 2 * sizeof(float) * ND * ND;
 template <int T>
-DEV void integrate_fk_dynamics_body(const Pool& P, const ModelS* __restrict__ mp, int b, DynData* lds_d, char* ms_raw, KinSeparate<KIN_OVERLAY, 64 / T>& lds_k,
-                                    bool pre, float pre_vel, float pre_acc) {
+DEV void integrate_fk_dynamics_body(const Pool& P, const ModelS* __restrict__ mp, const Model* __restrict__ gm, int b, DynData* lds_d, char* ms_raw,
+                                    KinSeparate<KIN_OVERLAY, 64 / T>& lds_k, BroadSeparate<BROAD_OVERLAY<T>, T>& lds_b, bool pre, float pre_vel, float pre_acc) {
   const ModelS& ms = *(const ModelS*)ms_raw;
   wg_dma_to_lds<(int)sizeof(ModelS)>(ms_raw, mp);
   const int tl = threadIdx.x % T, slot = threadIdx.x / T;
   const ModelView m(&ms, mp);
+  asm volatile("" : "+v"(b));
   E e(P, b < P.B ? b : P.B - 1);
   DynData* d = &lds_d[slot];
   static_assert(offsetof(DynData, L) == offsetof(DynData, M) + sizeof(float) * ND * ND, "KinData overlay");
@@ -1636,15 +1781,17 @@
   team_sync();
   PH(41)
   tk_dynamics<T>(m, e, d, tl, true);
+  tk_broadphase<T>(*gm, e, lds_b.at(slot, d), tl);
 }
 template <int T>
-__global__ __launch_bounds__(64) void k_integrate_fk_dynamics_team(Pool P, const ModelS* __restrict__ mp) {
+__global__ __launch_bounds__(64) void k_integrate_fk_dynamics_team(Pool P, const ModelS* __restrict__ mp, const Model* __restrict__ gm) {
   STAMP(STK_INT_FK_DYN)
   constexpr int EPW = 64 / T;
-  __shared__ DynData lds_d[EPW];
+  __shared__ alignas(16) DynData lds_d[EPW];
   __shared__ alignas(16) char ms_raw[MODELS_LDS_BYTES];
   __shared__ KinSeparate<KIN_OVERLAY, EPW> lds_k;
-  integrate_fk_dynamics_body<T>(P, mp, xcd_block() * EPW + (int)threadIdx.x / T, lds_d, ms_raw, lds_k, false, 0.0f, 0.0f);
+  __shared__ BroadSeparate<BROAD_OVERLAY<T>, T> lds_b;
+  integrate_fk_dynamics_body<T>(P, mp, gm, xcd_block() * EPW + (int)threadIdx.x / T, lds_d, ms_raw, lds_k, lds_b, false, 0.0f, 0.0f);
 }
 
 DEV int wrap180(float x) {
@@ -1682,11 +1829,6 @@
   }
   if (vid_out) *vid_out = vid;
   return v;
-}
-template <int T> DEV unsigned long long team_ballot(bool p) {
-  const unsigned long long b = __ballot(p);
-  if constexpr (T == 64) return b;
-  else return (b >> (threadIdx.x & (64 - T))) & ((1ull << T) - 1ull);
 }
 DEV V3 vsel(bool c, V3 a, V3 b) { return v3(c ? a.x : b.x, c ? a.y : b.y, c ? a.z : b.z); }
 DEV V3 support_prism(const V3* prism, V3 d) {
@@ -1997,20 +2139,11 @@
 constexpr int GJK_SLOTS = GJK_SLOTS_MAX;
 template <int T>
 struct CollideData {
-  struct Broad {
-    alignas(16) float amin[NG * 4], amax[NG * 4];
-    float sval[2 * NG], sval_sorted[2 * NG];
-    alignas(16) unsigned long long skey[2 * NG];
-    int sig[2 * NG], sig_sorted[2 * NG];
-    alignas(8) int rank_mm[NG * 2];
-    int cand_key[MAXB], cand_pair[MAXB];
-  };
   struct TPair { int i_ga, r_min, r_max, c_min, c_max, n_items, item_off; float zmin, tol; V3 pos_a; Q4 quat_a; V3 center_a; };
   struct Terrain {
     TPair tp[NG];
   };
   union alignas(16) {
-    Broad bp;
     GjkStoreLds gjk[GJK_SLOTS];
     Terrain tr;
   };
@@ -2303,130 +2436,26 @@
   const Model& m = *mp;
   E e(P, b);
   CollideData<T>* s = &lds[slot];
-  const float inf = dm_bits2f(0x7f800000u);
   if (tl == 0) s->gjk_slot_mask = 0u;
   for (int i = tl; i < NCV; i += T) s->ncv[i] = (unsigned)e.ncache_valid()[i];
   PH_BEGIN
-  const int nc_old = e.n_contacts()[0];
-  const bool first = e.first_time()[0] != 0;
-  const int n2 = 2 * NG;
-  team_stage<2 * NG, T>(tl, [&](int i) { return __int_as_float(e.sort_ig()[i]); }, [&](int i, float v) { s->bp.sig[i] = __float_as_int(v); });
-  constexpr int NPI = (NPAIR + T - 1) / T;
-  int packed_[NPI];
-  {
-    const int n_pairs = m.n_pairs;
-#pragma unroll
-    for (int it = 0; it < NPI; ++it) { int pidx = it * T + tl; int v = m.pair_list[pidx < NPAIR ? pidx : NPAIR - 1]; packed_[it] = (pidx < n_pairs) ? v : -1; }
-  }
-#pragma unroll
-  for (int g0 = 0; g0 < NG; g0 += T) {
-    const int i_g = (g0 + tl < NG) ? g0 + tl : NG - 1;
-    V3 lower = v3(inf, inf, inf), upper = v3(-inf, -inf, -inf);
-    V3 gp = e.g_pos()[i_g]; Q4 gq = e.g_quat()[i_g];
-#pragma unroll
-    for (int c = 0; c < 8; ++c) {
-      V3 corner = transform_by_trans_quat(m.geoms[i_g].aabb[c], gp, gq);
-      lower = vmin(lower, corner); upper = vmax(upper, corner);
-    }
-    *(float4*)&s->bp.amin[4 * i_g] = make_float4(lower.x, lower.y, lower.z, 0.0f);
-    *(float4*)&s->bp.amax[4 * i_g] = make_float4(upper.x, upper.y, upper.z, 0.0f);
-  }
-  for (int i_c = tl; i_c < nc_old; i_c += T) {
-    e.c_link()[i_c] = -1; e.c_link()[MAXC + i_c] = -1; e.c_geom()[i_c] = -1; e.c_geom()[MAXC + i_c] = -1;
-    e.c_pen()[i_c] = 0.0f; e.c_pos()[i_c] = v3(0, 0, 0); e.c_normal()[i_c] = v3(0, 0, 0); e.c_force()[i_c] = v3(0, 0, 0);
-  }
+  const int n_broad = imn(imx(e.n_broad()[0], 0), MAXB);
+  for (int c = tl; c < n_broad; c += T) s->pair_sorted[c] = (unsigned short)(e.broad()[2 * c] | (e.broad()[2 * c + 1] << 8));
   team_sync();
-  PH(30)
-  for (int i = tl; i < n2; i += T) {
-    int sg = first ? ((i >> 1) | ((i & 1) ? 0x100 : 0)) : s->bp.sig[i];
-    int g = sg & 0xff;
-    s->bp.sig[i] = sg;
-    const float v = (sg & 0x100) ? s->bp.amax[4 * g] : s->bp.amin[4 * g];
-    s->bp.sval[i] = v;
-    unsigned u = (unsigned)__float_as_int(v + 0.0f);
-    u = (u & 0x80000000u) ? ~u : (u | 0x80000000u);
-    s->bp.skey[i] = ((unsigned long long)u << 8) | (unsigned long long)i;
-  }
-  team_sync();
-  {
-    constexpr int NK = (2 * NG + T - 1) / T;
-    unsigned long long key[NK]; int r[NK];
-#pragma unroll
-    for (int q = 0; q < NK; ++q) { const int i = tl + q * T; key[q] = s->bp.skey[i < n2 ? i : n2 - 1]; r[q] = 0; }
-#pragma unroll
-    for (int j = 0; j < 2 * NG; ++j) {
-      const unsigned long long kj = s->bp.skey[j];
-#pragma unroll
-      for (int q = 0; q < NK; ++q) r[q] += (kj < key[q]) ? 1 : 0;
-    }
-#pragma unroll
-    for (int q = 0; q < NK; ++q) {
-      const int i = tl + q * T;
-      if (i < n2) {
-        const float v = s->bp.sval[i];
-        const int sg = s->bp.sig[i];
-        s->bp.sval_sorted[r[q]] = v; s->bp.sig_sorted[r[q]] = sg;
-        s->bp.rank_mm[2 * (sg & 0xff) + ((sg & 0x100) ? 1 : 0)] = r[q];
-        e.sort_value()[r[q]] = v; e.sort_ig()[r[q]] = sg;
-      }
-    }
-  }
-  if (tl == 0 && first) e.first_time()[0] = 0;
-  team_sync();
-  PH(31)
-  int n_cand = 0;
-  unsigned cmask = 0; int key_[NPI];
-  unsigned ncv_clear = 0u;
-  static_assert(NCV <= T, "one lane per word of the normal-cache mask");
-#pragma unroll
-  for (int it = 0; it < NPI; ++it) {
-    const int pidx = it * T + tl;
-    const int packed = packed_[it];
-    const int a = (packed < 0) ? 0 : (packed & 0xff), bg = (packed < 0) ? 0 : (packed >> 8);
-    const int2 rka = *(const int2*)&s->bp.rank_mm[2 * a], rkb = *(const int2*)&s->bp.rank_mm[2 * bg];
-    const float4 amn = *(const float4*)&s->bp.amin[4 * a], amx = *(const float4*)&s->bp.amax[4 * a], bmn = *(const float4*)&s->bp.amin[4 * bg], bmx = *(const float4*)&s->bp.amax[4 * bg];
-    const int ra = rka.x, rb = rkb.x;
-    const int rs = (ra < rb) ? rb : ra, rf = (ra < rb) ? ra : rb;
-    const int rmax_first = (ra < rb) ? rka.y : rkb.y;
-    key_[it] = rs * 64 + rf;
-    const bool swept = packed >= 0 && rs < rmax_first;
-    const bool any1 = (amx.x <= bmn.x) || (amx.y <= bmn.y) || (amx.z <= bmn.z);
-    const bool any2 = (amn.x >= bmx.x) || (amn.y >= bmx.y) || (amn.z >= bmx.z);
-    if (swept && !(any1 || any2)) cmask |= 1u << it;
-    const unsigned long long sep = team_ballot<T>(swept && (any1 || any2));
-    (void)pidx;
-    if constexpr (T < 32) { if (tl == ((it * T) >> 5)) ncv_clear |= (unsigned)(sep << ((it * T) & 31)); }
-    else if constexpr (T == 32) { if (tl == it) ncv_clear |= (unsigned)sep; }
-    else { if (tl == 2 * it) ncv_clear |= (unsigned)sep; if (tl == 2 * it + 1) ncv_clear |= (unsigned)(sep >> 32); }
-  }
-  if (tl < NCV) s->ncv[tl] &= ~ncv_clear;
-  {
-    const int mine = __popc(cmask);
-    s->cnt[tl] = mine;
-    team_sync();
-    int pos = 0, tot = 0;
-    for (int l = 0; l < T; ++l) { int c = s->cnt[l]; pos += (l < tl) ? c : 0; tot += c; }
-    team_sync();
-#pragma unroll
-    for (int it = 0; it < NPI; ++it)
-      if (cmask & (1u << it)) { if (pos < MAXB) { s->bp.cand_key[pos] = key_[it]; s->bp.cand_pair[pos] = packed_[it]; } pos++; }
-    n_cand = tot;
-  }
-  if (n_cand > m.max_broad_pairs && tl == 0) atomicOr(&e.err()[0], GO2SIM_ERR_OVERFLOW_CANDIDATE_CONTACTS);
-  n_cand = imn(n_cand, MAXB);
-  team_sync();
-  for (int c = tl; c < n_cand; c += T) {
-    int key = s->bp.cand_key[c], r = 0;
-    for (int j = 0; j < n_cand; ++j) r += s->bp.cand_key[j] < key;
-    s->pair_sorted[r] = (unsigned short)s->bp.cand_pair[c];
-  }
-  const int n_broad = imn(n_cand, m.max_broad_pairs);
-  team_sync();
-  for (int c = tl; c < n_broad; c += T) { int pk = s->pair_sorted[c]; e.broad()[2 * c] = pk & 0xff; e.broad()[2 * c + 1] = pk >> 8; }
-  PH(32)
   int nc_run = 0;
   const int n_np_iter = (n_broad + T - 1) / T;
-  auto append_staged = [&](const ContactStage& cs, int i_ga, int i_gb) {
+  struct PairConst { float friction, sol[7]; int link_a, link_b; };
+  auto load_pair_const = [&](int i_ga, int i_gb) {
+    PairConst pc;
+    float friction_a = e.geom_friction()[i_ga] * e.friction_ratio()[i_ga];
+    float friction_b = e.geom_friction()[i_gb] * e.friction_ratio()[i_gb];
+    pc.friction = fmx(fmx(friction_a, friction_b), 1e-2f);
+#pragma unroll
+    for (int q = 0; q < 7; ++q) pc.sol[q] = 0.5f * (m.geoms[i_ga].sol_params[q] + m.geoms[i_gb].sol_params[q]);
+    pc.link_a = m.geoms[i_ga].link; pc.link_b = m.geoms[i_gb].link;
+    return pc;
+  };
+  auto append_staged = [&](const ContactStage& cs, int i_ga, int i_gb, const PairConst& pc) {
     s->cnt[tl] = cs.n;
     team_sync();
     int off = 0, tot = 0;
@@ -2435,14 +2464,13 @@
       int i_c = nc_run + off + k;
       if (i_c < m.max_contact_pairs) {
         const float* p = cs.st + 7 * k;
-        float friction_a = e.geom_friction()[i_ga] * e.friction_ratio()[i_ga];
-        float friction_b = e.geom_friction()[i_gb] * e.friction_ratio()[i_gb];
         e.c_geom()[i_c] = i_ga; e.c_geom()[MAXC + i_c] = i_gb;
         e.c_normal()[i_c] = v3(p[0], p[1], p[2]); e.c_pos()[i_c] = v3(p[3], p[4], p[5]); e.c_pen()[i_c] = p[6];
-        e.c_friction()[i_c] = fmx(fmx(friction_a, friction_b), 1e-2f);
+        e.c_friction()[i_c] = pc.friction;
         auto sol = e.c_sol()[i_c];
-        for (int q = 0; q < 7; ++q) sol[q] = 0.5f * (m.geoms[i_ga].sol_params[q] + m.geoms[i_gb].sol_params[q]);
-        e.c_link()[i_c] = m.geoms[i_ga].link; e.c_link()[MAXC + i_c] = m.geoms[i_gb].link;
+#pragma unroll
+        for (int q = 0; q < 7; ++q) sol[q] = pc.sol[q];
+        e.c_link()[i_c] = pc.link_a; e.c_link()[MAXC + i_c] = pc.link_b;
       } else {
         atomicOr(&e.err()[0], GO2SIM_ERR_OVERFLOW_COLLISION_PAIRS);
       }
@@ -2464,6 +2492,7 @@
       convex_pair = m.geoms[i_gb].type != GEOM_TERRAIN && !plane_box;
     }
     any_plane_box |= team_ballot<T>(plane_box) != 0ull;
+    const PairConst pc = load_pair_const(i_ga, i_gb);
     if constexpr (T == 16) {
       static_assert(GJK_SLOTS >= 4, "one LDS polytope slot per quad");
       CcState cst;
@@ -2506,7 +2535,7 @@
       }
       if (convex_pair) cc_rest(m, e, cst, cs, nullptr, &s->gjk_slot_mask, &gjk_scratch[(size_t)b * T + tl], s->ncv);
     } else if (convex_pair) convex_convex_contact_staged(m, e, i_ga, i_gb, cs, s->gjk, &s->gjk_slot_mask, &gjk_scratch[(size_t)b * T + tl], s->ncv);
-    append_staged(cs, i_ga, i_gb);
+    append_staged(cs, i_ga, i_gb, pc);
   }
   if (any_plane_box) {
     for (int it = 0; it < n_np_iter; ++it) {
@@ -2519,7 +2548,7 @@
         if (m.geoms[i_ga].type > m.geoms[i_gb].type) { int t = i_ga; i_ga = i_gb; i_gb = t; }
         if (m.geoms[i_ga].type == GEOM_PLANE && m.geoms[i_gb].type == GEOM_BOX) plane_box_contact_staged(m, e, i_ga, i_gb, cs);
       }
-      append_staged(cs, i_ga, i_gb);
+      append_staged(cs, i_ga, i_gb, load_pair_const(i_ga, i_gb));
     }
   }
   if (m.terrain_enabled) {
@@ -2680,7 +2709,7 @@
     }
   }
   if (tl == 0) {
-    e.n_broad()[0] = n_broad; e.n_contacts()[0] = imn(nc_run, m.max_contact_pairs);
+    e.n_contacts()[0] = imn(nc_run, m.max_contact_pairs);
     s->cnt[0] = imn(nc_run, m.max_contact_pairs);
   }
   team_sync();
@@ -3974,7 +4003,8 @@
   constexpr int EPW = 64 / T;
   constexpr size_t SOLVE_OFF = (sizeof(SolverData<RLN>) * EPW + 15) / 16 * 16, DYN_OFF = (sizeof(DynData) * EPW + 15) / 16 * 16, KIN_OFF = (sizeof(KinData) * EPW + 15) / 16 * 16;
   constexpr size_t SOLVE_BYTES = SOLVE_OFF + lds_dma_bytes(SOLVER_BLOCK_BYTES);
-  constexpr size_t DYN_BYTES = DYN_OFF + MODELS_LDS_BYTES + sizeof(KinSeparate<KIN_OVERLAY, EPW>);
+  constexpr size_t KSEP_OFF = (sizeof(KinSeparate<KIN_OVERLAY, EPW>) + 15) / 16 * 16;
+  constexpr size_t DYN_BYTES = DYN_OFF + MODELS_LDS_BYTES + (BROAD_OVERLAY<T> ? sizeof(KinSeparate<KIN_OVERLAY, EPW>) : KSEP_OFF + sizeof(BroadSeparate<false, T>));
   constexpr size_t KIN_BYTES = KIN_OFF + MODELS_LDS_BYTES;
   __shared__ alignas(16) char raw[cmax(SOLVE_BYTES, WITH_DYN ? DYN_BYTES : KIN_BYTES)];
   const int tl = threadIdx.x % T, slot = threadIdx.x / T;
@@ -3991,7 +4021,8 @@
     DynData* lds_d = (DynData*)raw;
     char* ms_raw = raw + DYN_OFF;
     auto& lds_k = *(KinSeparate<KIN_OVERLAY, EPW>*)(ms_raw + MODELS_LDS_BYTES);
-    integrate_fk_dynamics_body<T>(P, mp, b, lds_d, ms_raw, lds_k, pre, pre_vel, pre_acc);
+    auto& lds_b = *(BroadSeparate<BROAD_OVERLAY<T>, T>*)(ms_raw + MODELS_LDS_BYTES + KSEP_OFF);
+    integrate_fk_dynamics_body<T>(P, mp, gm, b, lds_d, ms_raw, lds_k, lds_b, pre, pre_vel, pre_acc);
   } else {
     integrate_fk_body<T>(P, mp, b, (KinData*)raw, raw + KIN_OFF, pre, pre_vel, pre_acc);
   }
@@ -4310,12 +4341,14 @@
 
 template <int T>
 __global__ __launch_bounds__(64) void k_pre_dynamics_team(Pool P, const ModelS* __restrict__ mp, const DCfg cv, const Glob* __restrict__ gp,
-                                                          const float* __restrict__ actions_in, uint64_t seed, uint32_t step_count, int write_idx) {
+                                                          const float* __restrict__ actions_in, uint64_t seed, uint32_t step_count, int write_idx,
+                                                          const Model* __restrict__ gm) {
   STAMP(STK_PRE_DYN)
   static_assert(T >= NA, "one lane per action");
   constexpr int EPW = 64 / T;
-  __shared__ DynData lds[EPW];
+  __shared__ alignas(16) DynData lds[EPW];
   __shared__ alignas(16) char ms_raw[MODELS_LDS_BYTES];
+  __shared__ BroadSeparate<BROAD_OVERLAY<T>, T> lds_b;
   const ModelS& ms = *(const ModelS*)ms_raw;
   wg_dma_to_lds<(int)sizeof(ModelS)>(ms_raw, mp);
   {
@@ -4441,6 +4474,7 @@
   team_sync();
   PH(20)
   tk_dynamics<T>(m, e, s, tl, env_valid);
+  if (env_valid) tk_broadphase<T>(*gm, e, lds_b.at(slot, s), tl);
 }
 
 struct RewCtx { float link_vel_xy[8], foot_z[4], foot_xy[8]; float vel_world[3]; int was_reset; };
@@ -5488,7 +5522,6 @@
 struct Launch {
   void* func; dim3 grid, block;
   int cat;
-  bool join;
   std::vector<void*> args;
 };
 struct LaunchList {
@@ -5533,7 +5566,6 @@
   int graph_fallbacks = 0;
   bool fuse_fk_dyn = true;
   bool fuse_solve_int = true;
-  bool par_pre = false;
   int dyn_team = 32;
   int fk_team = 16;
   int collide_team = 16;
@@ -5594,7 +5626,7 @@
 template <class... P, class... A>
 static void add_launch(LaunchList& L, int cat, void (*kernel)(P...), dim3 grid, dim3 block, A... a) {
   static_assert(sizeof...(P) == sizeof...(A), "argument count");
-  Launch e{(void*)kernel, grid, block, cat, false, {}};
+  Launch e{(void*)kernel, grid, block, cat, {}};
   auto store = [&](auto typed) { using T = decltype(typed); T* m = (T*)malloc(sizeof(T)); memcpy((void*)m, (const void*)&typed, sizeof(T)); L.owned.push_back((void*)m); e.args.push_back((void*)m); };
   (store(static_cast<P>(a)), ...);
   L.v.push_back(std::move(e));
@@ -5603,10 +5635,10 @@
 static void build_launch_list(const go2sim* h, LaunchList& L, int n, const StepIO* io) {
   const dim3 ge = grid_for(h->B), b(WG);
   const bool terrain = h->hm.terrain_enabled != 0;
-  auto add_dynamics = [&]() { add_launch(L, T_DYN, dynamics_kernel(h->dyn_team), team_grid(h, h->dyn_team), b, h->P, h->dms); };
+  auto add_dynamics = [&]() { add_launch(L, T_DYN, dynamics_kernel(h->dyn_team), team_grid(h, h->dyn_team), b, h->P, h->dms, h->dm); };
   if (io) L.pre = 0;
   if (io && fuse_pre(h)) {
-    add_launch(L, T_DYN, pre_dynamics_kernel(h->dyn_team), team_grid(h, h->dyn_team), b, h->P, h->dms, h->hcfg, h->dglob, io->actions, h->seed, h->step_count, h->action_write_idx);
+    add_launch(L, T_DYN, pre_dynamics_kernel(h->dyn_team), team_grid(h, h->dyn_team), b, h->P, h->dms, h->hcfg, h->dglob, io->actions, h->seed, h->step_count, h->action_write_idx, h->dm);
   } else {
     if (io) add_launch(L, T_ENV_PRE, k_env_pre, ge, b, h->P, h->dm, h->hcfg, h->dglob, io->actions, h->seed, h->step_count, h->action_write_idx);
     add_dynamics();
@@ -5620,11 +5652,10 @@
     add_launch(L, T_COLLIDE, collide_kernel(h->collide_team), team_grid(h, h->collide_team), b, h->P, h->dm, h->gjk_scratch, lpt_cur, h->lpt_cap, solver_epw(h));
     const int Ts = terrain ? h->terrain_solver_team : h->solver_team;
     add_launch(L, T_SOLVE, solve_kernel(terrain, Ts, fuse_solve(h) ? (more ? 1 : 2) : 0), team_grid(h, Ts), b, h->P, h->dm, h->dms, h->solver_ovf, lpt_cur, lpt_next, h->lpt_cap);
-    L.v.back().join = io && i == 0 && fuse_pre(h) && h->par_pre;
     if (fuse_solve(h)) continue;
     if (more && h->fuse_fk_dyn) {
       const int Td = h->dyn_team == 64 ? 64 : 32;
-      add_launch(L, T_INTEGRATE, integrate_dynamics_kernel(Td), team_grid(h, Td), b, h->P, h->dms);
+      add_launch(L, T_INTEGRATE, integrate_dynamics_kernel(Td), team_grid(h, Td), b, h->P, h->dms, h->dm);
     } else {
       add_launch(L, T_INTEGRATE, integrate_kernel(h->fk_team), team_grid(h, h->fk_team), b, h->P, h->dms);
       if (more) add_dynamics();
@@ -5668,13 +5699,10 @@
 static bool step_graph_build(LaunchList& L) {
   if (hipGraphCreate(&L.graph, 0) != hipSuccess) return false;
   L.nodes.assign(L.v.size(), nullptr);
-  hipGraphNode_t last = nullptr, side = nullptr;
+  hipGraphNode_t last = nullptr;
   for (size_t i = 0; i < L.v.size(); ++i) {
-    if (i + 1 < L.v.size() && L.v[i + 1].join) { side = last; last = nullptr; }
-    hipGraphNode_t deps[2] = {last, L.v[i].join ? side : nullptr};
-    const int n_deps = (last ? 1 : 0) + ((last && deps[1]) ? 1 : 0);
     const hipKernelNodeParams kp = node_params(L.v[i]);
-    if (hipGraphAddKernelNode(&L.nodes[i], L.graph, n_deps ? deps : nullptr, n_deps, &kp) != hipSuccess) return false;
+    if (hipGraphAddKernelNode(&L.nodes[i], L.graph, last ? &last : nullptr, last ? 1 : 0, &kp) != hipSuccess) return false;
     last = L.nodes[i];
   }
   return hipGraphInstantiate(&L.exec, L.graph, nullptr, nullptr, 0) == hipSuccess;
@@ -5711,7 +5739,6 @@
   if (env_int("GO2SIM_NO_GRAPH", 0)) h->use_graph = false;
   if (env_int("GO2SIM_NO_FUSE", 0)) h->fuse_fk_dyn = false;
   if (env_int("GO2SIM_NO_FUSE_SOLVE", 0)) h->fuse_solve_int = false;
-  if (env_int("GO2SIM_PAR_PRE", 0)) h->par_pre = true;
   if (env_int("GO2SIM_NO_LPT", 0)) h->use_lpt = false;
 }
 
```

After: 17.66 million, median of 6. +5.0%, better.
